# Nextomics/NextPolish2

Hardware: AMD Instinct MI355X
Metric: polished reference Mbp/s (whole node) at 30x HiFi + k21/k31; FASTA identical to oracle (higher is better)
Workload: dtype u8

## Files before the change

### nextpolish2_amd/csrc/np2_common.hpp

```cpp
#pragma once
#include <cstdint>
#include <hip/hip_runtime.h>

#define NP2_HD __host__ __device__ __forceinline__

namespace np2 {

struct AlignBase {
    uint32_t t_pos;
    uint16_t delta;
    uint8_t q;
    NP2_HD bool is_head() const { return q == 15; }
    NP2_HD bool eq(const AlignBase &o) const { return q == o.q && delta == o.delta && t_pos == o.t_pos; }
};
NP2_HD AlignBase ab_head(uint32_t t_pos, uint16_t delta) { return AlignBase{t_pos, delta, 15}; }

NP2_HD uint16_t node_bases(const AlignBase &b1, const AlignBase &b2, const AlignBase &b3) {
    unsigned f = 0;
    if (b2.t_pos == b1.t_pos) f |= 0x4000u;
    if (b2.t_pos == b3.t_pos) f |= 0x1000u;
    return (uint16_t)(f | ((unsigned)b1.q << 8) | ((unsigned)b2.q << 4) | (unsigned)b3.q);
}
NP2_HD void node_decode(uint16_t bases, uint16_t delta, uint32_t p, AlignBase &a, AlignBase &b, AlignBase &c) {
    a.q = (bases >> 8) & 0xF;
    b.q = (bases >> 4) & 0xF;
    c.q = bases & 0xF;
    if ((bases & 0x5000) == 0x5000) {
        a.t_pos = p, a.delta = delta;
        b.t_pos = p, b.delta = (uint16_t)(delta + 1);
        c.t_pos = p, c.delta = (uint16_t)(delta + 2);
    } else if (bases & 0x1000) {
        a.t_pos = p - 1, a.delta = delta;
        b.t_pos = p, b.delta = 0;
        c.t_pos = p, c.delta = 1;
    } else if (bases & 0x4000) {
        a.t_pos = p - 1, a.delta = delta;
        b.t_pos = p - 1, b.delta = (uint16_t)(delta + 1);
        c.t_pos = p, c.delta = 0;
    } else {
        a.t_pos = p - 2, a.delta = delta;
        b.t_pos = p - 1, b.delta = 0;
        c.t_pos = p, c.delta = 0;
    }
}
NP2_HD uint16_t node_delta3(uint16_t bases, uint16_t delta) {
    if ((bases & 0x5000) == 0x5000) return (uint16_t)(delta + 2);
    if (bases & 0x1000) return 1;
    return 0;
}

NP2_HD uint64_t yak_hash64(uint64_t key, uint64_t mask) {
    key = (~key + (key << 21)) & mask;
    key = key ^ key >> 24;
    key = ((key + (key << 3)) + (key << 8)) & mask;
    key = key ^ key >> 14;
    key = ((key + (key << 2)) + (key << 4)) & mask;
    key = key ^ key >> 28;
    key = (key + (key << 31)) & mask;
    return key;
}

NP2_HD uint8_t code_to_ascii(uint8_t c) {
    const uint64_t tab = 0x004D4E2D54474341ULL;
    return (uint8_t)(tab >> (8 * (c & 7)));
}
NP2_HD uint8_t ascii_to_code(uint8_t ch) {
    switch (ch & 0x7F) {
    case 'A': case 'a': return 0;
    case 'C': case 'c': return 1;
    case 'G': case 'g': return 2;
    case 'T': case 't': case 'U': case 'u': return 3;
    case 'N': case 'n': return 5;
    case 'M': case 'm': return 6;
    default: return 4;
    }
}

static constexpr uint64_t INVALID_KMER = ~0ULL;
static constexpr uint32_t LQSEQ_MAX_CAN_COUNT = 60;
static constexpr int64_t SCORE_NEG = INT64_MIN >> 1;

enum : uint8_t { CLS_HQ = 0, CLS_LQ = 1, CLS_RESET = 2 };
static constexpr uint32_t GROW_ERR = 0x1000u;
static constexpr uint32_t LQ_LIST_ERR = 0x800u;

static constexpr uint32_t CKPT_SHIFT = 5;
static constexpr uint32_t CKPT = 1u << CKPT_SHIFT;

NP2_HD uint8_t nib_at(const uint8_t *bytes, uint32_t c) {
    uint8_t t = bytes[c >> 1];
    return (c & 1) ? (t & 15) : (t >> 4);
}


#if defined(__HIPCC__)
__device__ __forceinline__ uint32_t xcd_order(uint32_t b, uint32_t n) {
    if (n < 64) return b;
    const uint32_t q = n >> 3, r = n & 7u, x = b & 7u;
    return x * q + (x < r ? x : r) + (b >> 3);
}
#endif

}
```

### nextpolish2_amd/csrc/np2_ctx.hpp

```cpp
#pragma once
#include "../../include/np2.h"
#include "np2_abi.hpp"
#include "np2_common.hpp"
#include "np2_kernels.hpp"
#include "np2_hostcpu.hpp"

#include <algorithm>
#include <atomic>
#include <chrono>
#include <cstdio>
#include <cstdlib>
#include <cstring>
#include <map>
#include <memory>
#include <exception>
#include <mutex>
#include <stdexcept>
#include <string>
#include <vector>

namespace np2h {

using namespace np2;

// ... 393 lines not shown
    return std::chrono::duration<double, std::milli>(std::chrono::steady_clock::now().time_since_epoch()).count();
}


}

using namespace np2h;

struct np2_contig {
    np2_contig() {
        reads.cached = nib.cached = refnib.cached = ck_off.cached = ckpt.cached = descs.cached = true;
        tile_rd_off.cached = tile_rd.cached = true;
    }
    uint32_t L = 0, R = 0;
    uint64_t nib_bytes = 0, n_cols = 0, n_ckpt = 0;
    DevBuf<np2_read_t> reads;
    DevBuf<uint8_t> nib;
    DevBuf<uint8_t> refnib;
    uint32_t ref_stride = 0;
    DevBuf<uint64_t> ck_off;
    DevBuf<uint32_t> ckpt;
    uint32_t n_chunks = 0;
    DevBuf<ChunkDesc> descs;
    uint32_t n_tiles = 0;
    DevBuf<uint32_t> tile_rd_off, tile_rd;
    uint32_t tile_cap = TILE_CAP;
};

struct np2_ctx {
    int device = 0;
    hipStream_t stream = nullptr;
    hipStream_t stream_out = nullptr;
    hipEvent_t ev_out = nullptr;
    uint8_t *out_host[2] = {nullptr, nullptr};
    size_t out_host_cap[2] = {0, 0};
    int out_slot = 0;
    bool out_pending = false;
    uint64_t out_len = 0;
    std::vector<YakTable> yaks;
    std::string err;
    bool trace = false;
    std::map<std::string, std::vector<uint8_t>> trace_items;
    Timing timing;
    std::vector<std::pair<std::string, std::pair<hipEvent_t, hipEvent_t>>> pending_events;

    PinnedBuf pin_d2h, pin_h2d;
    uint32_t *mbox_host = nullptr, *mbox_dev = nullptr;
    uint32_t mbox_seq = 0;
    bool borrowed_state = false;
    uint8_t *sink_dst = nullptr;
    uint64_t sink_cap = 0;
    uint32_t last_first_pos = 0, last_last_pos = 0;
    const uint8_t *last_dbase = nullptr;
    const uint32_t *last_dpos = nullptr;
    DevBuf<uint32_t> shard_bounds;
    uint64_t last_len = 0;
    bool reuse_identical_pass = true;
    bool h2d_inflight = false;
    bool stage_timing = false;
    DevBuf<uint8_t> tmp;
    DevBuf<uint64_t> keys_raw, keys;
    DevBuf<uint32_t> vals_raw, vals;
    DevBuf<uint32_t> npos, ncount, nminr, nbesti, node_off, run_start, run_end, n0_besti, emit, eoff;
    DevBuf<uint16_t> nbases, ndelta;
    DevBuf<int64_t> nscore;
    DevBuf<int32_t> cov, mval, smin;
    DevBuf<uint8_t> alive, cns_base, cns_cls, lq_kind, lq_nothead;
    DevBuf<uint32_t> cns_pos, lq_next, rflag, rstart, rend, ridx, raw_start, raw_end, headflag, hidx, lq_start,
        lq_end;
    DevBuf<uint32_t> pj, pcount, reg_ncand, reg_bytes, reg_soff, reg_maxlen, blk_sum, blk_coff, blk_soff, kept_read, kept_len, kept_col, cand_off, cand_order, cand_seq_off, kill_ids;
    DevBuf<uint64_t> cand_kmer;
    DevBuf<uint8_t> cand_seq;
    DevBuf<uint16_t> kscore;
    DevBuf<uint32_t> scal;
    DevBuf<uint64_t> lb_status;
    DevBuf<uint32_t> lb_ticket;
    uint32_t lb_ticket_total = 0, lb_epoch = 0;
    bool lb_dirty = false;
    static constexpr size_t LB_MAX_BLOCKS = 1u << 20;
    DevBuf<uint32_t> mlen;
    DevBuf<uint8_t> reg_lable, grp, cns_base2, rech_groups, rech_groups_tmp;
    DevBuf<uint8_t> votepack;
    DevBuf<uint8_t> votepack2;
    DevBuf<uint32_t> rech_headjobs;
    DevBuf<uint32_t> ecount, eval, eval_s, eflag, eidx, seed_cand, keep_n, keep_list, cns_pos2, sp_idx_s,
        sp_idx_e, ap_g, ap_s, ap_e, rech, rech_joboff, job_len,
        job_off32;
    DevBuf<int32_t> ew, ap_delta, ap_shift;
    DevBuf<uint64_t> ekey, ekey_s;
    DevBuf<uint16_t> keep_ks;
    DevBuf<uint32_t> long_list;
    DevBuf<uint64_t> bt_path;
    DevBuf<uint64_t> chunk_st;
    uint32_t chunk_epoch = 0;
    DevBuf<uint32_t> tile_cur, tile_n, tile_scan, tile_scanb, tile_nn, tile_nr, tile_noff, tile_roff;
    uint32_t tile_cap = TILE_CAP;
    uint32_t bucket_cap = 0;
    DevBuf<uint2> nrec;
    DevBuf<uint8_t> votebuf;
    DevBuf<uint32_t> band, band_n, band_off, row_cnt;
    DevBuf<int64_t> run_gain, tile_gain;
    DevBuf<uint8_t> out_snap;
    DevBuf<uint8_t> run_flag;
    uint32_t deep_min = 65536;
    DevBuf<uint32_t> lq_list, hbits;
    DevBuf<uint16_t> tile_pidx;
    bool pidx_valid = false;
    DevBuf<ReadInfo> rinfo;
    DevBuf<uint32_t> lqc, lqoff;
    DevBuf<uint8_t> pflag;
    DevBuf<uint32_t> dp_list;
    DevBuf<uint16_t> pf_slots;
    DevBuf<uint32_t> pf_bad, pf_bad2;
    DevBuf<uint64_t> pf_prof;
    bool front_fused = false;
    struct Hooks {
        bool front_unfused = false, pf_prof = false, edge_sort = false;
        bool test_misspeculate = false, shard_spec_log = false, phase_profile = false, exact_grow = false, no_speculate = false;
        bool has_grow_guess = false;
        uint32_t grow_guess = 0;
        bool has_pf_cap = false, has_pf_cap_big = false, has_pf_halo = false, has_pf_cov_max = false;
        uint32_t pf_cap = 0, pf_cap_big = 0, pf_halo = 0, pf_cov_max = 0;
        void read() {
            auto on = [](const char *n) { return getenv(n) != nullptr; };
            auto u32 = [](const char *n, bool &has, uint32_t &v) {
                if (const char *e = getenv(n)) has = true, v = (uint32_t)atol(e);
            };
            front_unfused = on("NP2_FRONT_UNFUSED"), pf_prof = on("NP2_PF_PROF"), edge_sort = on("NP2_EDGE_SORT");
            test_misspeculate = on("NP2_TEST_MISSPECULATE");
            shard_spec_log = on("NP2_SHARD_SPEC_LOG"), phase_profile = on("NP2_PHASE_PROFILE"), exact_grow = on("NP2_EXACT_GROW");
            no_speculate = on("NP2_NO_SPECULATE");
            u32("NP2_TEST_GROW_GUESS", has_grow_guess, grow_guess);
            u32("NP2_PF_CAP", has_pf_cap, pf_cap), u32("NP2_PF_CAP_BIG", has_pf_cap_big, pf_cap_big);
            u32("NP2_PF_HALO", has_pf_halo, pf_halo), u32("NP2_PF_COV_MAX", has_pf_cov_max, pf_cov_max);
        }
    } hooks;
    bool pf_big = getenv("NP2_PF_BIG") != nullptr;
    uint32_t front_redos = 0;
    DevBuf<uint16_t> kscore_saved;
    DevBuf<uint8_t> sstr;
    DevBuf<uint64_t> soff;
    DevBuf<uint16_t> sscore;
};


namespace np2h {


enum Scal { S_ERR = 0, S_NNODES, S_NRUNS, S_BEST, S_PATHBEGIN, S_NRAW, S_NREG, S_DUP, S_LAST0, S_LAST1, S_GAIN0,
            S_GAIN1, S_DEEP, S_NDPLIST, S_NRECH, S_NGROUPS, S_NLONG, S_NLQ, S_PF, S_M0, S_M1, S_M2, S_M3, S_NC, S_SB, S_GROW,
            S_NBAD, S_PFOUT, S_PFGAIN0, S_PFGAIN1, S_PFEND0, S_PFEND1, S_NBAD2, S_NOKEY, S_COUNT = 34 };
static_assert(S_M1 % 2 == 0 && S_LAST0 % 2 == 0 && S_GAIN0 % 2 == 0 && S_PFGAIN0 % 2 == 0 && S_PFEND0 % 2 == 0,
              "64-bit device counters live in these slot pairs");

static constexpr int NP2_MAX_YAK = 15;
static constexpr uint32_t SCAL_TOTAL = 96;
static_assert(S_COUNT + 2 * (NP2_MAX_YAK + 2) <= SCAL_TOTAL && S_COUNT < 64, "round counters behind the posted block; the mailbox holds 64 words");

inline double thread_cpu_ms() {
    timespec ts;
    clock_gettime(CLOCK_THREAD_CPUTIME_ID, &ts);
    return ts.tv_sec * 1e3 + ts.tv_nsec * 1e-6;
}
struct WallTimer {
    np2_ctx *cx;
    const char *name;
    double t0, c0 = 0;
    WallTimer(np2_ctx *c, const char *n);
    ~WallTimer();
};

struct EventTimer {
    np2_ctx *cx;
    hipEvent_t a = nullptr, b = nullptr;
    bool on;
    EventTimer(np2_ctx *c, const char *name, bool always = false)
        : cx(c), on((always || c->stage_timing) && !tl_recorder()) {
        if (!on) return;
        (void)hipEventCreate(&a);
        (void)hipEventCreate(&b);
        (void)hipEventRecord(a, cx->stream);
        cx->pending_events.push_back({name, {a, b}});
    }
    ~EventTimer() {
        if (on) (void)hipEventRecord(b, cx->stream);
    }
};

inline WallTimer::WallTimer(np2_ctx *c, const char *n) : cx(c), name(n), t0(c->stage_timing ? now_ms() : 0.0), c0(c->stage_timing ? thread_cpu_ms() : 0.0) {}
inline WallTimer::~WallTimer() {
    if (cx->stage_timing) {
        cx->timing.host.push_back({name, (float)(now_ms() - t0)});
        if (strncmp(name, "wall", 4) == 0) cx->timing.host.push_back({std::string("cpu") + (name + 4), (float)(thread_cpu_ms() - c0)});
    }
}

inline void flush_timings(np2_ctx *cx) {
    std::map<std::string, float> acc;
    std::vector<std::string> order;
    for (auto &e : cx->pending_events) {
        float ms = 0;
        (void)hipEventSynchronize(e.second.second);
        (void)hipEventElapsedTime(&ms, e.second.first, e.second.second);
        if (!acc.count(e.first)) order.push_back(e.first);
        acc[e.first] += ms;
        (void)hipEventDestroy(e.second.first);
        (void)hipEventDestroy(e.second.second);
    }
    cx->pending_events.clear();
    for (auto &h : cx->timing.host) {
        if (!acc.count(h.first)) order.push_back(h.first);
        acc[h.first] += h.second;
    }
    cx->timing.host.clear();
    cx->timing.names = order;
    cx->timing.ms.clear();
    cx->timing.joined.clear();
    for (auto &n : order) {
        cx->timing.ms.push_back(acc[n]);
        cx->timing.joined += n;
        cx->timing.joined.push_back('\0');
    }
    cx->timing.joined.push_back('\0');
}
inline auto ctx_sink(np2_ctx *cx, bool timings = false) {
    return [cx, timings](int, const std::string &msg) {
        (void)hipStreamSynchronize(cx->stream);
        if (timings) flush_timings(cx);
        cx->err = msg;
    };
}

inline void recorder_sync(Recorder *r) {
    r->sync_fn(r, true);
    for (auto &g : r->graveyard)
        dev_release_idle(g.first, (g.second >> 63) ? 0 : g.second, (g.second >> 63) ? (g.second & ~(1ull << 63)) : 0);
    r->graveyard.clear();
}
np2_ctx *ctx_create_slot(np2_ctx *parent, hipStream_t s, uint32_t *mbox_host, uint32_t *mbox_dev);
void ctx_slot_set_stream(np2_ctx *cx, hipStream_t s);
// ... 177 lines not shown
```

### nextpolish2_amd/csrc/np2_host.cpp

```cpp
#include "../../include/np2.h"
#include "np2_common.hpp"
#include "np2_kernels.hpp"
#include "np2_ctx.hpp"
#include "np2_phase_host.hpp"

#include <algorithm>
#include <atomic>
#include <thread>
#include <chrono>
#include <cstdio>
#include <cstdlib>
#include <cstring>
#include <map>
#include <mutex>
#include <stdexcept>
#include <string>
#include <unordered_map>
#include <unordered_set>
#include <future>
#include <functional>
#include <vector>

using namespace np2;

// ... 13 lines not shown
    std::vector<uint32_t> pos;
    std::vector<uint8_t> base;
    size_t size() const { return pos.size(); }
};
void trace_cns(np2_ctx *cx, int pass, const std::string &tag, const Cns &c) {
    trace_put(cx, pass, tag + ".pos", c.pos);
    trace_put(cx, pass, tag + ".base", c.base);
}

struct PassCounts {
    uint32_t n_reg = 0, NC = 0, SB = 0, M = 0;
    uint32_t grow = 0;
    bool known = false;
    uint32_t NC_cap = 0;
    uint32_t SB_cap = 0;
    void resolve(const std::vector<uint32_t> &sc) {
        NC = sc[S_NC], SB = sc[S_SB], grow = sc[S_GROW];
        known = true;
    }
};

RegionTables region_tables(np2_ctx *cx, uint32_t n_reg) {
    return RegionTables{cx->cand_off.p, cx->cand_order.p, cx->kscore.p, cx->cand_seq_off.p, cx->cand_seq.p, n_reg};
}

void trace_region_tables(np2_ctx *cx, int pass, const std::string &tag, const PassCounts &pc, bool kept_view) {
    if (!cx->trace) return;
    const uint32_t n_reg = pc.n_reg;
    auto start = d2h(cx, cx->lq_start.p, n_reg), end = d2h(cx, cx->lq_end.p, n_reg);
    auto coff = d2h(cx, cx->cand_off.p, (size_t)n_reg + 1);
    auto order = d2h(cx, cx->cand_order.p, pc.NC);
    auto ks = d2h(cx, cx->kscore.p, pc.NC);
    auto soff = d2h(cx, cx->cand_seq_off.p, (size_t)pc.NC + 1);
    auto pool = d2h(cx, cx->cand_seq.p, pc.SB);
    std::vector<uint8_t> lable(n_reg, 0);
    std::vector<uint32_t> seedc, keepn, keepl;
    std::vector<uint16_t> keepks;
    if (tag != "cand") lable = d2h(cx, cx->reg_lable.p, n_reg);
    if (kept_view) {
        seedc = d2h(cx, cx->seed_cand.p, n_reg);
        keepn = d2h(cx, cx->keep_n.p, n_reg);
        keepl = d2h(cx, cx->keep_list.p, pc.NC);
        keepks = d2h(cx, cx->keep_ks.p, pc.NC);
    }
    std::vector<uint32_t> o_coff(1, 0), o_order, o_soff(1, 0), sudo_off(1, 0);
    std::vector<uint16_t> o_ks;
    std::vector<uint8_t> o_seq, sudo;
    for (uint32_t g = 0; g < n_reg; ++g) {
        if (kept_view) {
            const uint32_t c = seedc[g];
            if (c != 0xFFFFFFFFu) sudo.insert(sudo.end(), pool.begin() + soff[c], pool.begin() + soff[c + 1]);
            for (uint32_t t = 0; t < keepn[g]; ++t) {
                const uint32_t ci = keepl[coff[g] + t];
                o_order.push_back(order[ci]);
                o_ks.push_back(keepks[coff[g] + t]);
                o_seq.insert(o_seq.end(), pool.begin() + soff[ci], pool.begin() + soff[ci + 1]);
                o_soff.push_back((uint32_t)o_seq.size());
            }
        } else {
            for (uint32_t ci = coff[g]; ci < coff[g + 1]; ++ci) {
                o_order.push_back(order[ci]);
                o_ks.push_back(ks[ci]);
                o_seq.insert(o_seq.end(), pool.begin() + soff[ci], pool.begin() + soff[ci + 1]);
                o_soff.push_back((uint32_t)o_seq.size());
            }
        }
        sudo_off.push_back((uint32_t)sudo.size());
        o_coff.push_back((uint32_t)o_order.size());
    }
    trace_put(cx, pass, tag + ".start", start);
    trace_put(cx, pass, tag + ".end", end);
    trace_put(cx, pass, tag + ".lable", lable);
    trace_put(cx, pass, tag + ".sudo_off", sudo_off);
    trace_put(cx, pass, tag + ".sudo", sudo);
    trace_put(cx, pass, tag + ".cand_off", o_coff);
    trace_put(cx, pass, tag + ".order", o_order);
    trace_put(cx, pass, tag + ".kscore", o_ks);
    trace_put(cx, pass, tag + ".seq_off", o_soff);
    trace_put(cx, pass, tag + ".seq", o_seq);
    if (tag == "cand") trace_put(cx, pass, "cand.kmer", d2h(cx, cx->cand_kmer.p, pc.NC));
}

struct GrowRetry : Np2Error {
    GrowRetry() : Np2Error(NP2_E_DEVICE, "internal: guessed growth allowance too small") {}
};
void check_region_err(np2_ctx *cx, uint32_t e) {
    (void)cx;
    if (e & 4u) throw Np2Error(NP2_E_REFPANIC, "reference would panic: seq2 order is equal to 0");
    if (e & 8u) throw Np2Error(NP2_E_REFPANIC, "reference would panic: index out of bounds: lqseq.seqs[max1_p]");
    if (e & 16u) throw Np2Error(NP2_E_REFPANIC, "reference would panic: the first lqseq is not ref.");
    if (e & 32u) throw Np2Error(NP2_E_REFPANIC, "reference would panic: lqseq.seqs[0] after retain_sort_seqs");
    if (e & 64u) throw Np2Error(NP2_E_REFPANIC, "reference would panic: consensus index out of bounds in reupdate");
    if (e & 128u) throw Np2Error(NP2_E_NOMEM, "cartesian product of chained LQ regions is too large");
    if (e & LB_ERR) throw Np2Error(NP2_E_DEVICE, "device-wide scan timed out waiting for a predecessor block");
    if (e & GROW_ERR) throw GrowRetry();
    if (e & LQ_LIST_ERR) throw Np2Error(NP2_E_DEVICE, "internal: more low-quality bases than their list was sized for");
}

struct VoteData {
    uint32_t R = 0;
    bool any = false;
    std::vector<uint64_t> pair_key;
    std::vector<uint32_t> pair_cnt;
    const uint64_t *view_key = nullptr;
    const uint32_t *view_cnt = nullptr;
    uint64_t view_n = 0;
    const uint32_t *off = nullptr;
    const phase::Graph::Edge *edges = nullptr;
    uint32_t n_nokey = 0;
    std::vector<uint32_t> off_own;
    std::vector<phase::Graph::Edge> edges_own;
    bool rows() const { return off != nullptr; }
    const uint64_t *keys() const { return view_key ? view_key : pair_key.data(); }
    const uint32_t *cnts() const { return view_key ? view_cnt : pair_cnt.data(); }
    uint64_t n_pairs() const { return view_key ? view_n : (uint64_t)pair_key.size(); }
    void own() {
        if (rows() && off_own.empty()) {
            off_own.assign(off, off + R + 1);
            edges_own.assign(edges, edges + off[R]);
            off = off_own.data(), edges = edges_own.data();
        }
        if (!view_key) return;
        pair_key.assign(view_key, view_key + view_n);
        pair_cnt.assign(view_cnt, view_cnt + view_n);
        view_key = nullptr, view_cnt = nullptr, view_n = 0;
    }
    std::vector<uint32_t> first_key;
    std::vector<int32_t> ref_w;
    std::vector<uint8_t> ref_seen, bad;
    const uint8_t *d_bad = nullptr;
    bool key_added = false;
};

bool vote_rows_from_pairs(VoteData &vd, bool use_all) {
    const uint32_t R = vd.R;
    const uint64_t *k = vd.keys();
    const uint32_t *cn = vd.cnts();
    const uint64_t np = vd.n_pairs();
    std::vector<uint32_t> n_lo(R, 0), n_up(R, 0);
    uint32_t nokey = 0;
    auto listed = [&](uint64_t i, uint32_t &a, uint32_t &b) {
        a = (uint32_t)(k[i] >> 32), b = (uint32_t)k[i];
        if (a >= R || b >= R || vd.first_key[a] == 0xFFFFFFFFu || vd.first_key[b] == 0xFFFFFFFFu) return false;
        return use_all || !(vd.bad[a] | vd.bad[b]);
    };
    for (uint64_t i = 0; i < np; ++i) {
        uint32_t a = (uint32_t)(k[i] >> 32), b = (uint32_t)k[i];
        if (b <= a || b - a - 1 >= EDGE_BAND || (i && k[i - 1] >= k[i])) return false;
        if (a >= R || b >= R || vd.first_key[a] == 0xFFFFFFFFu || vd.first_key[b] == 0xFFFFFFFFu) ++nokey;
        if (listed(i, a, b)) ++n_lo[b], ++n_up[a];
    }
    vd.off_own.assign((size_t)R + 1, 0);
    std::vector<uint32_t> cur_lo(R), cur_up(R);
    for (uint32_t v = 0; v < R; ++v) {
        cur_lo[v] = vd.off_own[v], cur_up[v] = vd.off_own[v] + n_lo[v];
        vd.off_own[v + 1] = cur_up[v] + n_up[v];
    }
    vd.edges_own.resize(vd.off_own[R]);
    for (uint64_t i = 0; i < np; ++i) {
        uint32_t a, b;
        if (!listed(i, a, b)) continue;
        const int32_t same = (int32_t)(cn[i] & 0xFFFFu), neg = (int32_t)(cn[i] >> 16);
        const float w = (float)(neg >= 3 ? -neg : same - neg);
        vd.edges_own[cur_lo[b]++] = phase::Graph::Edge(a, w);
        vd.edges_own[cur_up[a]++] = phase::Graph::Edge(b, w);
    }
    vd.off = vd.off_own.data(), vd.edges = vd.edges_own.data(), vd.n_nokey = nokey;
    return true;
}

void vote_collect(np2_ctx *cx, np2_contig *c, PassCounts &pc, bool asref, bool use_all, int pass, uint32_t own_lo,
                  uint32_t own_hi, VoteData &vd, bool wide = false, uint64_t key_add = 0) {
    hipStream_t s = cx->stream;
    const uint32_t R = c->R, n_reg = pc.n_reg;
    RegionTables rt = region_tables(cx, n_reg);
    uint32_t NE = 0, NU = 0;
    vd = VoteData();
    vd.R = R;
// ... 184 lines not shown
    const bool prof = getenv("NP2_PHASE_PROFILE") != nullptr;
    double t_mark = t_host0;
    auto mark = [&](const char *what) {
        if (prof) {
            const double t = now_ms();
            fprintf(stderr, "  vote host: %s %.2f ms\n", what, t - t_mark);
            t_mark = t;
        }
    };
    phase::Graph data;
    data.reserve_ids(R);
    mark("key order");
    for (auto &k : keys) data.add_key(k.second);
    mark("key table");
    auto weight = [&](uint64_t i) {
        const int32_t same = (int32_t)(pair_cnt[i] & 0xFFFFu), neg = (int32_t)(pair_cnt[i] >> 16);
        return (float)(neg >= 3 ? -neg : same - neg);
    };
    std::vector<uint32_t> bad;
    for (uint32_t r = 0; r < R; ++r)
        if (vd.bad[r]) bad.push_back(r);
    if (!use_all) data.keys.keep_if([&](uint32_t k, phase::Nil &) { return !vd.bad[k]; });
    mark("retain");
    std::future<phase::OrderSet> communities;
    if (data.keys.size() >= (1u << 15) && phase::host_threads() > 1)
        communities = std::async(std::launch::async, [&data] { return phase::SignedLouvain::first_communities(data.keys); });
    bool ok = false;
    try {
        if (vd.rows()) {
            ok = vd.n_nokey == 0;
            if (ok) data.adopt_rows(vd.off, vd.edges, R);
        } else {
            ok = data.add_edges_sorted(vd.keys(), NU, weight, use_all ? nullptr : vd.bad.data());
        }
    } catch (...) {
        if (communities.valid()) communities.wait();
        throw;
    }
    phase::OrderSet comm_pre;
    if (communities.valid()) comm_pre = communities.get();
    const bool have_pre = !comm_pre.empty();
    if (!ok) throw Np2Error(NP2_E_DEVICE, "internal: edge endpoint without a key");
    if (!use_all)
        for (uint32_t b : bad) data.is_key[b] = 0;
    mark("keys + edges");
    if (cx && cx->trace && pass >= 0) {
        trace_put(cx, pass, "vote.row_off", data.off);
        const phase::Graph::Edge *e0 = data.n_ids() ? data.adj(0).b : nullptr;
        trace_put(cx, pass, "vote.rows", std::vector<phase::Graph::Edge>(e0, e0 + (e0 ? data.n_edges() : 0)));
    }
    std::vector<float> ref_row(R, 0.f);
    std::vector<uint8_t> ref_have(R, 0);
    bool have_ref = false;
    for (uint32_t r = 0; r < R; ++r)
        if (vd.ref_seen[r]) {
            ref_row[r] = (float)vd.ref_w[r];
            ref_have[r] = 1;
            have_ref = true;
        }
    std::vector<uint32_t> losers;
    if (!phase::losing_reads(std::move(data), have_ref, ref_row, ref_have, losers, have_pre ? &comm_pre : nullptr))
        throw Np2Error(NP2_E_REFPANIC,
                       "reference would panic: the weight of two conflicting community is not less than 0");
    mark("louvain + ranking");
    if (cx) cx->timing.host.push_back({"wall_louvain", (float)(now_ms() - t_host0)});
    std::vector<uint8_t> lost(R, 0);
    for (uint32_t b : bad) lost[b] = 1;
    for (uint32_t l : losers)
        if (l < R) lost[l] = 1;
        else throw Np2Error(NP2_E_DEVICE, "internal: loser outside the contig's reads");
    losers.clear();
    for (uint32_t r = 0; r < R; ++r)
        if (lost[r]) losers.push_back(r);
    return losers;
}

struct CnsDev {
    uint32_t *pos;
    uint8_t *base;
    const uint32_t *M_p;
    uint32_t M_cap;
};

CnsDev splice_gpu(np2_ctx *cx, const CnsDev &in, uint32_t n_reg, uint8_t lable, uint32_t grow_bound, bool to_b,
                  uint32_t version) {
    hipStream_t s = cx->stream;
    EventTimer t(cx, "splice");
    cx->sp_idx_s.ensure(n_reg + 2);
    cx->sp_idx_e.ensure(n_reg + 2);
    cx->ap_g.ensure(n_reg + 2);
    cx->ap_s.ensure(n_reg + 2);
    cx->ap_e.ensure(n_reg + 2);
    cx->ap_delta.ensure(n_reg + 2);
    cx->ap_shift.ensure(n_reg + 2);
    cx->mlen.ensure(16);
    const uint32_t out_cap = in.M_cap + grow_bound;
    const size_t cap = (size_t)out_cap + 64;
    uint32_t *opos = to_b ? cx->cns_pos2.ensure(cap) : cx->cns_pos.ensure(cap);
    uint8_t *obase = to_b ? cx->cns_base2.ensure(cap) : cx->cns_base.ensure(cap);
    uint32_t *const stuck_p = cx->scal.p + S_COUNT + 2 * version, *const nap_p = stuck_p + 1;
    launch_splice_find(s, in.pos, in.M_p, cx->lq_start.p, cx->lq_end.p, cx->reg_lable.p, lable, n_reg, cx->sp_idx_s.p,
                       cx->sp_idx_e.p, stuck_p);
    launch_splice_plan(s, next_lookback(cx, region_lb_blocks(n_reg)), cx->reg_lable.p, lable, n_reg, stuck_p,
                       cx->sp_idx_s.p, cx->sp_idx_e.p, cx->seed_cand.p, cx->cand_seq_off.p, cx->ap_g.p, cx->ap_s.p,
                       cx->ap_e.p, cx->ap_delta.p, cx->ap_shift.p, nap_p, in.M_p, cx->mlen.p + version, out_cap,
                       cx->scal.p + S_ERR);
    launch_splice_write(s, in.pos, in.base, in.M_p, in.M_cap, cx->ap_g.p, cx->ap_s.p, cx->ap_e.p, cx->ap_delta.p,
                        cx->ap_shift.p, nap_p, n_reg, cx->lq_start.p, cx->seed_cand.p, cx->cand_seq_off.p,
                        cx->cand_seq.p, opos, obase);
    return CnsDev{opos, obase, cx->mlen.p + version, out_cap};
}

Cns fetch_cns_dev(np2_ctx *cx, const CnsDev &c) {
    Cns r;
    const uint32_t M = d2h(cx, c.M_p, 1)[0];
    r.pos = d2h(cx, c.pos, M);
    r.base = d2h(cx, c.base, M);
    return r;
}

CnsDev recheck_gpu(np2_ctx *cx, const CnsDev &in, const PassCounts &pc, int yak_idx, uint16_t min_kmer_count,
                   bool first_yak, bool to_b, uint32_t version) {
    hipStream_t s = cx->stream;
    const uint32_t n_reg = pc.n_reg, ksize = cx->yaks[yak_idx].k;
    uint32_t n_rech = 0, n_groups = 0, n_jobs = 0;
    uint64_t blob_bound = 0;
    {
        EventTimer t(cx, "recheck");
        cx->rech.ensure(n_reg + 2);
        cx->rech_groups.ensure((size_t)(n_reg + 2) * rech_group_bytes());
        cx->rech_joboff.ensure(n_reg + 2);
        cx->rech_groups_tmp.ensure((size_t)(n_reg + 2) * rech_group_bytes());
        cx->rech_headjobs.ensure(n_reg + 2);
        launch_rech_list(s, next_lookback(cx, region_lb_blocks(n_reg)), cx->reg_lable.p, n_reg, cx->rech.p, cx->scal.p + S_NRECH,
                         (unsigned long long *)(cx->scal.p + S_M1), cx->scal.p + S_ERR);
        launch_rech_groups(s, next_lookback(cx, region_lb_blocks(n_reg)), cx->rech.p, cx->scal.p + S_NRECH, n_reg, in.pos, in.M_p,
                           cx->lq_start.p, cx->lq_end.p, cx->keep_n.p, ksize, cx->reg_maxlen.p, cx->rech_groups_tmp.p,
                           cx->rech_headjobs.p, cx->rech_groups.p,
                           cx->rech_joboff.p, cx->scal.p + S_NGROUPS,
                           cx->scal.p + S_M0, (unsigned long long *)(cx->scal.p + S_M1), cx->scal.p + S_ERR);
        std::vector<uint32_t> sc = fetch_scal(cx);
        blob_bound = (uint64_t)sc[S_M1] | ((uint64_t)sc[S_M2] << 32);
        check_region_err(cx, sc[S_ERR]);
        n_rech = sc[S_NRECH];
        n_groups = sc[S_NGROUPS];
        n_jobs = sc[S_M0];
    }
    if (n_rech) {
        RechPtrs rp{cx->rech_groups.p, cx->rech_joboff.p, cx->rech.p, cx->cand_off.p, cx->keep_list.p,
                    cx->cand_seq_off.p, cx->cand_seq.p, in.base, n_groups};
        if (n_jobs) {
            EventTimer t(cx, "recheck");
            cx->job_len.ensure(n_jobs + 2);
            cx->job_off32.ensure(n_jobs + 2);
            cx->soff.ensure(n_jobs + 2);
            cx->sscore.ensure(n_jobs + 2);
            cx->tmp.ensure(prim_temp_bytes((size_t)n_jobs + 2));
            launch_rech_job_len(s, rp, n_jobs, cx->job_len.p);
            exclusive_total_n(cx, cx->job_len.p, cx->job_off32.p, n_jobs);
            if (blob_bound >= 0xFFFFFFF0ull)
                blob_bound = fetch_scal(cx, cx->scal.p + S_M0, cx->job_off32.p + n_jobs)[S_M0];
            cx->sstr.ensure((size_t)blob_bound + 64);
            launch_rech_job_build(s, rp, n_jobs, cx->job_off32.p, cx->soff.p, cx->sstr.p);
            launch_score_strings(s, cx->yaks[yak_idx].dev(), cx->sstr.p, cx->soff.p, n_jobs, min_kmer_count,
                                 cx->sscore.p, true);
            launch_rech_apply(s, rp, cx->sscore.p, cx->keep_ks.p);
        }
        EventTimer t(cx, "recheck");
        launch_rech_select(s, cx->rech.p, cx->scal.p + S_NRECH, n_rech, cx->cand_off.p, cx->keep_n.p, cx->keep_list.p,
                           cx->keep_ks.p, cx->cand_order.p, first_yak, cx->reg_lable.p, cx->seed_cand.p);
    }
    CnsDev out = splice_gpu(cx, in, n_reg, LB_RECH, pc.grow, to_b, version);
    launch_rech_relabel(s, cx->reg_lable.p, n_reg);
    return out;
}

void gpu_score_strings(np2_ctx *cx, int yak_idx, const std::vector<uint8_t> &blob, const std::vector<uint64_t> &off,
                       uint16_t min_kmer_count, std::vector<uint16_t> &scores) {
    const size_t n = off.size() - 1;
    scores.assign(n, 0);
    if (!n) return;
    cx->sstr.ensure(blob.size() + 16);
    cx->soff.ensure(off.size());
    cx->sscore.ensure(n);
    {
        op_sync(cx);
        uint8_t *pin = (uint8_t *)cx->pin_h2d.ensure(blob.size() + off.size() * 8 + 16);
        const size_t o2 = (blob.size() + 7) & ~(size_t)7;
        memcpy(pin, blob.data(), blob.size());
        memcpy(pin + o2, off.data(), off.size() * 8);
        op_h2d(cx, cx->sstr.p, pin, blob.size());
        op_h2d(cx, cx->soff.p, pin + o2, off.size() * 8);
        cx->h2d_inflight = true;
    }
    {
        EventTimer t(cx, "score_strings");
        launch_score_strings(cx->stream, cx->yaks[yak_idx].dev(), cx->sstr.p, cx->soff.p, n, min_kmer_count,
                             cx->sscore.p, false);
    }
    scores = d2h(cx, cx->sscore.p, n);
}

struct PassOut {
    bool has_regions = false;
    Cns cns;
};

void run_diff(np2_ctx *cx, np2_contig *c, uint32_t &T) {
    hipStream_t s = cx->stream;
    const uint32_t L = c->L, R = c->R, NCH = c->n_chunks;
    const uint32_t n_tiles = (L + TILE - 1) >> TILE_SHIFT;
    const uint32_t bcap = std::min(cx->tile_cap, c->tile_cap);
    const uint64_t buckets = (uint64_t)n_tiles * bcap;
    uint64_t ovf_cap = std::max<uint64_t>(c->n_cols / 256 + 65536, 1u << 18);
    cx->tmp.ensure(prim_temp_bytes(std::max<size_t>((size_t)NCH + 2, (size_t)L + 2)));
    cx->tile_n.ensure(n_tiles + 2);
    cx->tile_scan.ensure(n_tiles + 2);
    cx->tile_scanb.ensure(n_tiles + 2);
    cx->tile_nn.ensure(n_tiles + 2);
    cx->tile_nr.ensure(n_tiles + 2);
    cx->tile_noff.ensure(n_tiles + 2);
    cx->tile_roff.ensure(n_tiles + 2);
    cx->tile_gain.ensure(n_tiles + 2);
    if (cx->tile_cur.cap < (size_t)n_tiles + 2) {
        cx->tile_cur.ensure(n_tiles + 2);
        zero32(cx, cx->tile_cur.p, cx->tile_cur.cap);
    }
    if (cx->chunk_st.cap < (size_t)NCH + 2) {
        cx->chunk_st.ensure(NCH + 2);
// ... 500 lines not shown
    uint64_t key_add = 0;
    PassCounts pc;
    bool final_pass() const { return pass + 1 == o.iter_count; }
};

void run_begin(PolishRun &r) {
    np2_ctx *cx = r.cx;
    if (r.o.iter_count < 1) throw Np2Error(NP2_E_ARG, "iter_count must be >= 1");
    HIPCHK(hipSetDevice(cx->device));
    cx->trace_items.clear();
    cx->last_dbase = nullptr;
    cx->last_dpos = nullptr;
    cx->scal.ensure(SCAL_TOTAL);
    cx->alive.ensure(r.c->R + 2);
    {
        WallTimer w(cx, "wall_diff");
        run_diff(cx, r.c, r.T);
    }
    launch_init_alive(cx->stream, r.c->reads.p, r.c->R, cx->alive.p);
    r.pass = 0;
    r.reuse = false;
}

void run_pass_front(PolishRun &r) {
    np2_ctx *cx = r.cx;
    np2_contig *c = r.c;
    if (!r.reuse) {
        {
            WallTimer w(cx, "wall_cns_lq");
            if (!r.front_issued) pass_front_issue(cx, c, r.T, (int)r.pass);
            r.front_issued = false;
            consensus_and_regions_finish(cx, c, r.T, (int)r.pass, r.M, r.n_reg, !r.wide_votes);
        }
        if (cx->trace) {
            trace_cns(cx, (int)r.pass, "cns_raw", fetch_cns(cx, r.M));
            trace_put(cx, (int)r.pass, "lq.start", d2h(cx, cx->lq_start.p, r.n_reg));
            trace_put(cx, (int)r.pass, "lq.end", d2h(cx, cx->lq_end.p, r.n_reg));
        }
    }
    if (r.n_reg == 0) return;
    if (!r.reuse) {
        r.pc = PassCounts();
        r.pc.M = r.M;
        WallTimer w(cx, "wall_extract");
        extract_candidates(cx, c, r.n_reg, r.o.min_kmer_count, (int)r.pass, r.pc);
    } else if (r.pc.NC_cap) {
        op_copy_d2d(cx, cx->kscore.p, cx->kscore_saved.p, (size_t)(r.pc.known ? r.pc.NC : r.pc.NC_cap) * 2);
    }
}

void run_vote_pass(PolishRun &r, VoteData &vd, const std::function<void()> *after_front = nullptr) {
    np2_ctx *cx = r.cx;
    vd = VoteData();
    vd.R = r.c->R;
    run_pass_front(r);
    if (after_front) (*after_front)();
    if (r.n_reg == 0) return;
    WallTimer w(cx, "wall_vote");
    const bool may_reuse = cx->reuse_identical_pass && !cx->trace;
    if (may_reuse && r.pc.NC_cap) {
        cx->kscore_saved.ensure((size_t)r.pc.NC_cap + 2);
        op_copy_d2d(cx, cx->kscore_saved.p, cx->kscore.p, (size_t)(r.pc.known ? r.pc.NC : r.pc.NC_cap) * 2);
    }
    vote_collect(cx, r.c, r.pc, r.o.model_ref != 0, r.o.use_all_reads != 0, (int)r.pass, r.own_lo, r.own_hi, vd, r.wide_votes, r.key_add);
    if (r.pc.known) r.grow_prev = r.pc.grow;
}

void run_apply_losers(PolishRun &r, const std::vector<uint32_t> &losers) {
    np2_ctx *cx = r.cx;
    if (r.n_reg) trace_put(cx, (int)r.pass, "invalid_ids", losers);
    for (uint32_t id : losers) REFPANIC_IF(id >= r.c->R, "index out of bounds: alignseqs[id]");
    const bool may_reuse = cx->reuse_identical_pass && !cx->trace;
    r.reuse = false;
    if (!losers.empty()) {
        cx->kill_ids.ensure(losers.size());
        h2d_staged(cx, cx->kill_ids.p, losers.data(), losers.size() * 4);
        launch_kill_reads(cx->stream, cx->kill_ids.p, (uint32_t)losers.size(), cx->alive.p);
    } else if (may_reuse) {
        r.reuse = true;
    }
    ++r.pass;
}

void run_final_pass(PolishRun &r, ResultOut &result, bool exact_grow = false) {
    np2_ctx *cx = r.cx;
    np2_contig *c = r.c;
    hipStream_t s = cx->stream;
    const uint32_t n_reg_prev = r.n_reg;
    (void)n_reg_prev;
    run_pass_front(r);
    const uint32_t n_reg = r.n_reg;
    if (n_reg == 0) {
        fetch_result(cx, cx->cns_pos.p, cx->cns_base.p, cx->eoff.p + c->L, r.M, result);
        return;
    }
    PassCounts &pc = r.pc;
    WallTimer w(cx, "wall_final");
    RegionTables rt = region_tables(cx, n_reg);
    cx->reg_lable.ensure(n_reg + 2);
    cx->seed_cand.ensure(n_reg + 2);
    cx->keep_n.ensure(n_reg + 2);
    const bool no_guess = cx->hooks.exact_grow;
    bool guessed = false;
    if (!pc.known) {
        if (r.grow_prev != 0xFFFFFFFFu && !exact_grow && !no_guess && !cx->trace && (uint64_t)r.grow_prev * 2 + 4096 < 0x7FFFFFFFull) {
            pc.grow = r.grow_prev * 2 + 4096;
            if (cx->hooks.has_grow_guess) pc.grow = cx->hooks.grow_guess;
            guessed = true;
        } else {
            pc.resolve(fetch_scal(cx));
        }
    }
    try {
        cx->keep_list.ensure((size_t)pc.NC_cap + 2);
        cx->keep_ks.ensure((size_t)pc.NC_cap + 2);
        {
            EventTimer t(cx, "seed");
            launch_seed(s, rt, r.o.max_indel_len, cx->reg_lable.p, cx->seed_cand.p, cx->keep_n.p, cx->keep_list.p,
                        cx->keep_ks.p, cx->scal.p + S_ERR);
        }
        if (cx->trace) check_region_err(cx, d2h(cx, cx->scal.p + S_ERR, 1)[0]);
        trace_region_tables(cx, (int)r.pass, "seed", pc, true);
        CnsDev cur{cx->cns_pos.p, cx->cns_base.p, cx->eoff.p + c->L, r.M};
        bool to_b = true;
        uint32_t version = 0;
        cur = splice_gpu(cx, cur, n_reg, LB_SUCC, pc.grow, to_b, version++);
        to_b = !to_b;
        if (cx->trace) trace_cns(cx, (int)r.pass, "cns_succ", fetch_cns_dev(cx, cur));
        for (size_t y = 0; y < cx->yaks.size(); ++y) {
            cur = recheck_gpu(cx, cur, pc, (int)y, r.o.min_kmer_count, y == 0, to_b, version++);
            to_b = !to_b;
            trace_region_tables(cx, (int)r.pass, "rech" + std::to_string(y), pc, true);
            if (cx->trace) trace_cns(cx, (int)r.pass, "cns_rech" + std::to_string(y), fetch_cns_dev(cx, cur));
        }
        fetch_result(cx, cur.pos, cur.base, cur.M_p, cur.M_cap, result, guessed ? r.M + r.grow_prev : r.M + pc.grow);
    } catch (const GrowRetry &) {
        if (!guessed) throw;
        result.release();
        op_fill(cx, cx->scal.p + S_ERR, 0, 4);
        r.reuse = false;
        run_final_pass(r, result, true);
    }
}

void polish_impl(np2_ctx *cx, np2_contig *c, const np2_opts_t *o, ResultOut &result) {
    PolishRun r;
    r.cx = cx, r.c = c, r.o = *o;
    run_begin(r);
    const bool no_spec = cx->hooks.no_speculate;
    const bool use_all = o->use_all_reads != 0;
    struct Decision {
        std::vector<uint32_t> losers;
        double ms = 0;
    };
    struct Pending {
        std::future<Decision> fut;
        std::shared_ptr<VoteData> vd;
        size_t n_bad = 0;
        bool active = false;
    } pend;
    auto settle = [&]() -> bool {
        if (!pend.active) return true;
        pend.active = false;
        Decision d = pend.fut.get();
        cx->timing.host.push_back({"wall_louvain", (float)d.ms});
        std::vector<uint32_t> extra;
        for (uint32_t id : d.losers) {
            REFPANIC_IF(id >= c->R, "index out of bounds: alignseqs[id]");
            if (!pend.vd->bad[id]) extra.push_back(id);
        }
        if (extra.empty() && d.losers.size() == pend.n_bad && !cx->hooks.test_misspeculate) return true;
        if (!extra.empty()) {
            cx->kill_ids.ensure(extra.size() + 1);
            h2d_staged(cx, cx->kill_ids.p, extra.data(), extra.size() * 4);
            launch_kill_reads(cx->stream, cx->kill_ids.p, (uint32_t)extra.size(), cx->alive.p);
        }
        r.reuse = false;
        r.front_issued = false;
        return false;
    };
    const std::function<void()> settle_then_redo = [&]() {
        if (!settle()) run_pass_front(r);
    };
    while (!r.final_pass()) {
        auto vd = std::make_shared<VoteData>();
        run_vote_pass(r, *vd, &settle_then_redo);
        size_t n_bad = 0;
        if (vd->any && vd->d_bad && !use_all && !cx->trace && !no_spec)
            for (uint8_t b : vd->bad) n_bad += b;
        if (n_bad == 0) {
            run_apply_losers(r, vote_decide(cx, *vd, use_all, (int)r.pass));
            continue;
        }
        launch_kill_flagged(cx->stream, vd->d_bad, c->R, cx->alive.p);
        ++r.pass;
        r.reuse = false;
        if (cx->hooks.pf_prof) vd->own();
        pass_front_issue(cx, c, r.T, (int)r.pass);
        r.front_issued = true;
        op_submit(cx);
        pend.vd = vd;
        pend.n_bad = n_bad;
        pend.active = true;
        auto decide = [vd, use_all]() {
            Decision d;
            const double t0 = now_ms();
            d.losers = vote_decide(nullptr, *vd, use_all);
            d.ms = now_ms() - t0;
            return d;
        };
        if (tl_recorder() == nullptr) {
            vd->own();
            pend.fut = std::async(std::launch::async, decide);
        } else {
            std::promise<Decision> p;
            pend.fut = p.get_future();
            try {
                p.set_value(decide());
            } catch (...) {
                p.set_exception(std::current_exception());
            }
            (void)settle();
        }
    }
// ... 1021 lines not shown
```

### nextpolish2_amd/csrc/np2_kernels.hip

```cpp
#include "np2_common.hpp"
#include "np2_kernels.hpp"
#include "np2_blockscan.hpp"
#include "np2_nib128.hpp"
#include "../../include/np2.h"

namespace np2 {

__device__ __forceinline__ uint8_t ref_code(const uint8_t *__restrict__ refnib, uint32_t p) {
    return (refnib[p >> 1] >> (4 * (p & 1))) & 7;
}

__device__ __forceinline__ void k_encode_ref(const uint32_t np2_bid, const uint32_t np2_nb, const uint8_t *__restrict__ read0, uint32_t L, uint8_t *__restrict__ refnib,
                             uint32_t nbytes_total, uint32_t stride, uint32_t *__restrict__ err) {
    uint32_t i = np2_bid * blockDim.x + threadIdx.x;
    if (i >= nbytes_total) return;
    uint32_t c0 = 2 * i, c1 = 2 * i + 1;
    uint8_t b = c0 < L ? read0[i] : 0;
    uint8_t hi = c0 < L ? (b >> 4) : 0, lo = c1 < L ? (b & 15) : 0;
    if ((c0 < L && c0 != 0 && (hi & 8)) || (c1 < L && (lo & 8))) atomicOr(err, 1u);
    if (c0 < L && (hi & 7) == 7) atomicOr(err, 1u);
    if (c1 < L && (lo & 7) == 7) atomicOr(err, 1u);
    refnib[i] = (uint8_t)((hi & 7) | ((lo & 7) << 4));
    const uint8_t nx = c1 + 1 < L ? (uint8_t)((read0[i + 1] >> 4) & 7) : (uint8_t)0;
    refnib[stride + i] = (uint8_t)(((hi & 7) << 4) | (lo & 7));
// ... 1177 lines not shown
        while (atomicCAS((unsigned long long *)&tb[s], (unsigned long long)YAK_EMPTY, (unsigned long long)w) != YAK_EMPTY)
            s = (s + 1) & capm;
        ob[s] = (uint32_t)i;
    }
}

__device__ __forceinline__ void k_lookup(const uint32_t np2_bid, const uint32_t np2_nb, YakDev y, const uint64_t *__restrict__ hashes, uint64_t n, uint16_t min_count,
                         uint16_t *__restrict__ out) {
    uint64_t i = (uint64_t)np2_bid * blockDim.x + threadIdx.x;
    if (i < n) out[i] = yak_get(y, hashes[i], min_count);
}

__device__ __forceinline__ uint16_t wave_score_string_any(const YakDev &y, const uint8_t *__restrict__ s, uint32_t len,
                                                          uint16_t min_count) {
    const uint32_t lane = threadIdx.x & 63;
    const uint32_t k = y.k;
    const uint64_t mask = (1ULL << (2 * (uint64_t)k)) - 1, shift = 2 * ((uint64_t)k - 1);
    uint32_t mn = 0xFFFFFFFFu;
    if (len >= k) {
        for (uint32_t st = lane; st + k <= len; st += 64) {
            uint64_t fw = 0, rv = 0;
            bool ok = true;
            for (uint32_t j = 0; j < k; ++j) {
                const uint64_t c = ascii_to_code(s[st + j]);
                if (c >= 4) {
                    ok = false;
                    break;
                }
                fw = ((fw << 2) | c) & mask;
                rv = (rv >> 2) | ((3ULL ^ c) << shift);
            }
            if (ok) mn = min(mn, (uint32_t)yak_get(y, yak_hash64(fw < rv ? fw : rv, mask), min_count));
        }
    }
    for (int o = 32; o > 0; o >>= 1) mn = min(mn, (uint32_t)__shfl_xor(mn, o));
    return mn == 0xFFFFFFFFu ? (uint16_t)0 : (uint16_t)mn;
}
__device__ __forceinline__ uint16_t wave_score_string(const YakDev &y, const uint8_t *__restrict__ s, uint32_t len,
                                                      uint16_t min_count) {
    const uint32_t lane = threadIdx.x & 63;
    const uint32_t k = y.k;
    const uint64_t mask = (1ULL << (2 * (uint64_t)k)) - 1;
    uint32_t mn = 0xFFFFFFFFu;
    if (len >= k) {
        for (uint32_t st = lane; st + k <= len; st += 64) {
            uint64_t codes = 0, bad = 0;
#pragma unroll
            for (uint32_t wd = 0; wd < 4; ++wd) {
                uint64_t x;
                __builtin_memcpy(&x, s + st + 8 * wd, 8);
                uint64_t c = ((x >> 1) ^ (x >> 2)) & 0x0303030303030303ULL;
                c = (c | (c >> 6)) & 0x000F000F000F000FULL;
                c = (c | (c >> 12)) & 0x000000FF000000FFULL;
                c = (c | (c >> 24)) & 0xFFFFULL;
                codes |= c << (16 * wd);
                uint64_t b = (x >> 3) & 0x0101010101010101ULL;
                b = (b | (b >> 7)) & 0x0003000300030003ULL;
                b = (b | (b >> 14)) & 0x0000000F0000000FULL;
                b = (b | (b >> 28)) & 0xFFULL;
                bad |= b << (8 * wd);
            }
            if ((bad & ((1ULL << k) - 1ULL)) == 0) {
                codes &= mask;
                uint64_t rb = __builtin_bitreverse64(codes);
                rb = ((rb >> 1) & 0x5555555555555555ULL) | ((rb & 0x5555555555555555ULL) << 1);
                const uint64_t fw = rb >> (64 - 2 * k), rv = ~codes & mask;
                mn = min(mn, (uint32_t)yak_get(y, yak_hash64(fw < rv ? fw : rv, mask), min_count));
            }
        }
    }
    for (int o = 32; o > 0; o >>= 1) mn = min(mn, (uint32_t)__shfl_xor(mn, o));
    return mn == 0xFFFFFFFFu ? (uint16_t)0 : (uint16_t)mn;
}

__device__ __forceinline__ void k_score_strings(const uint32_t np2_bid, const uint32_t np2_nb, YakDev y, const uint8_t *__restrict__ strs, const uint64_t *__restrict__ off,
                                uint64_t n, uint16_t min_count, uint16_t *__restrict__ out, uint32_t own_strings) {
    const uint64_t w = ((uint64_t)np2_bid * (blockDim.x >> 6)) + (uint32_t)__builtin_amdgcn_readfirstlane((int)(threadIdx.x >> 6));
    if (w >= n) return;
    const uint16_t sc = own_strings ? wave_score_string(y, strs + off[w], (uint32_t)(off[w + 1] - off[w]), min_count)
                                    : wave_score_string_any(y, strs + off[w], (uint32_t)(off[w + 1] - off[w]), min_count);
    if ((threadIdx.x & 63) == 0) out[w] = sc;
}

__device__ __forceinline__ void k_cand_score(const uint32_t np2_bid, const uint32_t np2_nb, YakDev y, const uint32_t *__restrict__ cand_seq_off, const uint64_t *__restrict__ cand_kmer,
                             const uint32_t *__restrict__ n_cand_p, uint16_t min_count,
                             uint16_t *__restrict__ kscore, uint32_t *__restrict__ long_list,
                             uint32_t *__restrict__ n_long) {
    const uint32_t c = np2_bid * blockDim.x + threadIdx.x;
    const bool live = c < *n_cand_p;
    const uint32_t len = live ? cand_seq_off[c + 1] - cand_seq_off[c] : 0u;
    const bool is_long = live && len > y.k;
    const uint64_t m = __ballot(is_long);
    if (m) {
        const uint32_t lane = threadIdx.x & 63, lead = (uint32_t)__builtin_ctzll(m);
        uint32_t base = 0;
        if (lane == lead) base = atomicAdd(n_long, (uint32_t)__builtin_popcountll(m));
        base = __shfl(base, lead);
        if (is_long) long_list[base + (uint32_t)__builtin_popcountll(m & ((1ULL << lane) - 1ULL))] = c;
    }
    if (!live) return;
    uint16_t sc = 0;
    if (!is_long) {
        const uint64_t km = cand_kmer[c];
        if (km != INVALID_KMER) sc = yak_get(y, km, min_count);
    }
    kscore[c] = sc;
}
__device__ __forceinline__ void k_cand_score_long(const uint32_t np2_bid, const uint32_t np2_nb, YakDev y, const uint32_t *__restrict__ cand_seq_off,
                                  const uint8_t *__restrict__ cand_seq, const uint32_t *__restrict__ long_list,
                                  const uint32_t *__restrict__ n_long, uint16_t min_count,
                                  uint16_t *__restrict__ kscore) {
    const uint32_t nl = *n_long;
    for (uint32_t w = (uint32_t)__builtin_amdgcn_readfirstlane((int)((np2_bid * blockDim.x + threadIdx.x) >> 6)); w < nl; w += (np2_nb * blockDim.x) >> 6) {
        const uint32_t c = long_list[w];
        const uint16_t sc = wave_score_string(y, cand_seq + cand_seq_off[c], cand_seq_off[c + 1] - cand_seq_off[c],
                                              min_count);
        if ((threadIdx.x & 63) == 0) kscore[c] = sc;
    }
}

}

namespace np2 {
static inline dim3 grid1(uint64_t n, uint32_t bs = 256) { return dim3((unsigned)((n + bs - 1) / bs)); }

void launch_encode_ref(hipStream_t s, const uint8_t *read0, uint32_t L, uint8_t *refnib, uint32_t nbytes,
                       uint32_t stride, uint32_t *err) {
    NP2_LAUNCH(k_encode_ref, grid1(nbytes), 256, s, read0, L, refnib, nbytes, stride, err);
}
void launch_post(hipStream_t s, uint32_t *scal, uint32_t n_scal, uint32_t *mbox, uint32_t seq, uint32_t *d0,
                 const uint32_t *s0, uint32_t *d1, const uint32_t *s1, uint32_t *d2, const uint32_t *s2, uint32_t *d3,
                 const uint32_t *s3, const uint32_t *ends_of, uint32_t *ends_dst) {
    NP2_LAUNCH(k_post, dim3(1), 64, s, scal, n_scal, mbox, seq, d0, s0, d1, s1, d2, s2, d3, s3, ends_of, ends_dst);
}
void launch_fill(hipStream_t s, uint8_t *p, uint64_t bytes, uint8_t byte) {
    if (bytes) NP2_LAUNCH(k_fill, grid1((bytes + 15) / 16), 256, s, p, bytes, 0x01010101u * byte);
}
void launch_copy(hipStream_t s, uint8_t *dst, const uint8_t *src, uint64_t bytes) {
    if (bytes) NP2_LAUNCH(k_copy, grid1((bytes + 15) / 16), 256, s, dst, src, bytes);
}
void launch_copy_len(hipStream_t s, uint8_t *dst, const uint8_t *src, const uint32_t *n_dev, uint32_t elem, uint64_t cap_bytes) {
    if (cap_bytes) NP2_LAUNCH(k_copy_len, grid1((cap_bytes + 15) / 16), 256, s, dst, src, n_dev, elem, cap_bytes);
}
void launch_copy_counted(hipStream_t s, uint32_t *dst, const uint32_t *src, const uint32_t *n_dev, uint32_t cap, uint32_t words_per) {
    if (cap) NP2_LAUNCH(k_copy_counted, dim3(std::max<uint32_t>(1, std::min<uint32_t>((cap + 1023) / 1024, 2048))), 256, s, dst, src, n_dev, cap, words_per);
}
void launch_init_alive(hipStream_t s, const np2_read_t *reads, uint32_t R, uint8_t *alive) {
    NP2_LAUNCH(k_init_alive, grid1(R), 256, s, reads, R, alive);
}
void launch_kill_flagged(hipStream_t s, const uint8_t *flag, uint32_t n, uint8_t *alive) {
    if (n) NP2_LAUNCH(k_kill_flagged, grid1(n), 256, s, flag, n, alive);
}
void launch_kill_reads(hipStream_t s, const uint32_t *ids, uint32_t n, uint8_t *alive) {
    if (n) NP2_LAUNCH(k_kill_reads, grid1(n), 256, s, ids, n, alive);
}
void launch_revive_reads(hipStream_t s, const uint32_t *ids, uint32_t n, uint8_t *alive) {
    if (n) NP2_LAUNCH(k_revive_reads, grid1(n), 256, s, ids, n, alive);
}
static Graph mk_graph(const GraphPtrs &gp) { return Graph{gp.refnib, gp.node_off, gp.nd, gp.cov, gp.L, gp.nrec, gp.deep}; }

void launch_dp_short(hipStream_t s, const GraphPtrs &gp, const void *refw, const uint32_t *run_start,
                     const uint32_t *n_runs, uint32_t max_runs, uint32_t *run_end, int64_t *run_gain, uint32_t *emit,
                     uint32_t *path_begin, uint64_t *path, uint32_t *dp_list, uint32_t *n_dp_list) {
    if (max_runs)
        NP2_LAUNCH(k_dp_bt_short, dim3(std::min<uint32_t>((max_runs + 63) / 64, DP_GRID_CAP)), 64, s, run_start, n_runs, mk_graph(gp), (const uint32_t *)refw, run_end, run_gain, emit, path_begin, path, dp_list, n_dp_list);
}
// ... 3 lines not shown
                    const uint32_t *dp_list, const uint32_t *n_dp_list) {
    if (!max_runs) return;
    NP2_LAUNCH(k_dp_bt_oct, dim3(std::min<uint32_t>((max_runs + 7) / 8, 2048u)), 64, s, run_start, mk_graph(gp), nrec, nscore, nbesti, n0_besti, run_end, last_n0_score, run_gain, emit, path_begin, path, run_flag, dp_list, n_dp_list);
    NP2_LAUNCH(k_dp_bt_long, dim3(std::min<uint32_t>((max_runs + DP_BLOCK - 1) / DP_BLOCK, 512u)), DP_BLOCK, s, run_start, mk_graph(gp), nrec, nscore, nbesti, n0_besti, run_end, last_n0_score, run_gain, emit, path_begin, path, run_flag, dp_list, n_dp_list);
}
void launch_dp_finish(hipStream_t s, const GraphPtrs &gp, const uint32_t *run_start, const uint32_t *n_runs,
                      const int64_t *nscore, const uint32_t *nbesti, const uint32_t *n0_besti, const int64_t *last_n0_score,
                      unsigned long long *total_gain, uint32_t *blocks_done, uint32_t *best_idx, const int64_t *run_gain,
                      const long long *tile_gain, uint32_t n_tiles, uint32_t *emit, uint32_t *path_begin, uint64_t *path) {
    NP2_LAUNCH(k_dp_finish, dim3(64), 256, s, run_gain, n_runs, tile_gain, n_tiles, total_gain, blocks_done, mk_graph(gp), nscore, last_n0_score, run_start, nbesti, n0_besti, best_idx, emit, path_begin, path);
}
static inline dim3 run_grid(uint32_t bound) { return dim3(std::max<uint32_t>(1, std::min<uint32_t>((bound + 256) / 256, 4096))); }
void launch_bt_write(hipStream_t s, const GraphPtrs &gp, const uint32_t *run_start, const uint32_t *n_runs,
                     uint32_t run_bound, const uint32_t *emit, const uint32_t *eoff, const uint64_t *path,
                     uint32_t *cns_pos, uint8_t *cns_base, uint8_t *cns_cls, uint8_t *lq_nothead, uint32_t *lqc) {
    NP2_LAUNCH(k_cns_write, grid1(gp.L), 256, s, gp.refnib, gp.pflag, emit, eoff, gp.L, cns_pos, cns_base, cns_cls, lq_nothead);
    NP2_LAUNCH(k_cns_runs, run_grid(4 * (uint64_t)run_bound > 0xFFFFFFF0ull ? 0xFFFFFFF0u : 4 * run_bound), 256, s, run_start, n_runs, run_bound, gp.node_off, emit, eoff, path, cns_pos, cns_base, cns_cls, lq_nothead, lqc);
}
void launch_lq_list(hipStream_t s, const GraphPtrs &gp, const uint32_t *run_start, const uint32_t *n_runs,
                    uint32_t run_bound, const uint32_t *emit, const uint32_t *eoff, const uint64_t *path,
                    const uint32_t *lqoff, uint32_t cap, uint32_t *lq_list, uint32_t *err) {
    NP2_LAUNCH(k_lq_list, run_grid(run_bound), 256, s, run_start, n_runs, run_bound, gp.node_off, emit, eoff, path, lqoff, cap, lq_list, err);
}
void launch_default_tail(hipStream_t s, const GraphPtrs &gp, const uint32_t *best_idx, const uint32_t *M_p, uint8_t *cns_base,
                         uint8_t *cns_cls, uint32_t *lq_list, uint32_t *n_lq, uint32_t cap, uint32_t *err) {
    NP2_LAUNCH(k_default_tail, 1, 64, s, best_idx, gp.node_off, gp.pflag, gp.L, M_p, cns_base, cns_cls, lq_list, n_lq, cap, err);
}
static inline dim3 lq_grid(uint32_t cap) { return dim3(std::max<uint32_t>(1, std::min<uint32_t>((cap + 2047) / 2048, 2048))); }
void launch_lq_scan(hipStream_t s, const uint32_t *cns_pos, const uint8_t *cns_base, const uint8_t *cns_cls,
                    const uint32_t *M_p, const uint32_t *lq_list, const uint32_t *n_lq, uint32_t lq_cap, uint8_t *lq_kind,
                    uint32_t *lq_next, uint8_t *lq_nothead, uint32_t *hbits, uint32_t n_hwords, uint32_t *rstart, uint32_t *rend) {
    NP2_LAUNCH(k_lq_scan, lq_grid(std::max(lq_cap, n_hwords / 4)), 256, s, cns_pos, cns_base, cns_cls, M_p, lq_list, n_lq, lq_cap, lq_kind, lq_next, lq_nothead, hbits, n_hwords);
    NP2_LAUNCH(k_lq_region, lq_grid(lq_cap), 256, s, cns_pos, cns_base, M_p, lq_list, n_lq, lq_cap, lq_kind, lq_next, lq_nothead, hbits, rstart, rend);
}
void launch_lq_bits_count(hipStream_t s, const uint32_t *hbits, uint32_t n_words, uint32_t *wcnt) {
    NP2_LAUNCH(k_lq_bits_count, grid1((uint64_t)n_words + 1), 256, s, hbits, n_words, wcnt);
}
void launch_scatter_regions(hipStream_t s, const uint32_t *hbits, uint32_t n_words, const uint32_t *woff,
                            const uint32_t *rstart, const uint32_t *rend, uint32_t *raw_start, uint32_t *raw_end,
                            uint32_t *n_raw) {
    NP2_LAUNCH(k_scatter_regions, grid1(std::max<uint32_t>(n_words, 1)), 256, s, hbits, n_words, woff, rstart, rend, raw_start, raw_end, n_raw);
}
void launch_lq_merge_flag(hipStream_t s, const uint32_t *raw_start, const uint32_t *raw_end, const uint32_t *n_raw,
                          uint32_t *headflag) {
    NP2_LAUNCH(k_lq_merge_flag, dim3(256), 256, s, raw_start, raw_end, n_raw, headflag);
}
void launch_lq_merge_scan(hipStream_t s, const uint32_t *raw_start, const uint32_t *raw_end, const uint32_t *n_raw, uint32_t n_host,
                          uint32_t *headflag, uint32_t *hidx) {
    NP2_LAUNCH(k_lq_merge_scan, dim3(1), 1024, s, raw_start, raw_end, n_raw, n_host, headflag, hidx);
}
void launch_lq_merge_write(hipStream_t s, const uint32_t *raw_start, const uint32_t *raw_end, const uint32_t *n_raw,
                           const uint32_t *headflag, const uint32_t *hidx, uint32_t *lq_start, uint32_t *lq_end,
                           uint32_t *n_reg) {
    NP2_LAUNCH(k_lq_merge_write, dim3(256), 256, s, raw_start, raw_end, n_raw, headflag, hidx, lq_start, lq_end, n_reg);
}
void launch_read_m(hipStream_t s, const np2_read_t *reads, uint32_t R, const uint8_t *alive, const uint32_t *lq_start,
                   uint32_t n_reg, int32_t *mval) {
    NP2_LAUNCH(k_read_m, grid1(R), 256, s, reads, R, alive, lq_start, n_reg, mval);
}
void launch_pair_count(hipStream_t s, const np2_read_t *reads, uint32_t R, const uint8_t *alive,
                       const uint32_t *lq_start, const uint32_t *lq_end, uint32_t n_reg, const int32_t *smin,
                       uint32_t *pj, uint32_t *pcount, const uint64_t *ck_off, ReadInfo *rinfo) {
    NP2_LAUNCH(k_pair_count, grid1(R), 256, s, reads, R, alive, lq_start, lq_end, n_reg, smin, pj, pcount, ck_off, rinfo);
}
void launch_yak_insert(hipStream_t s, const uint64_t *words, const uint64_t *bucket_off, uint32_t n_buckets,
                       uint64_t max_bucket, uint64_t *table, uint32_t cap_log2, uint32_t *dup_flag, uint32_t gap) {
    uint32_t gx = (uint32_t)((max_bucket + 255) / 256);
    if (gx == 0) gx = 1;
    if (gx > 64) gx = 64;
    hipLaunchKernelGGL(k_yak_insert, dim3(gx, n_buckets), dim3(256), 0, s, words, bucket_off, n_buckets, table,
                       cap_log2, dup_flag, gap);
}
void launch_yak_insert_dup(hipStream_t s, const uint64_t *words, const uint64_t *bucket_off, uint32_t n_buckets,
                           uint64_t max_bucket, uint64_t *table, uint32_t cap_log2, uint32_t *ord, uint32_t gap) {
    uint32_t gx = (uint32_t)((max_bucket + 255) / 256);
    gx = std::min<uint32_t>(64, std::max<uint32_t>(1, gx));
    hipLaunchKernelGGL(k_yak_insert_dup, dim3(gx, n_buckets), dim3(256), 0, s, words, bucket_off, n_buckets, table,
                       cap_log2, ord, gap);
}
void launch_lookup(hipStream_t s, const YakDev &y, const uint64_t *hashes, uint64_t n, uint16_t min_count,
                   uint16_t *out) {
    if (n) NP2_LAUNCH(k_lookup, grid1(n), 256, s, y, hashes, n, min_count, out);
}
void launch_score_strings(hipStream_t s, const YakDev &y, const uint8_t *strs, const uint64_t *off, uint64_t n,
                          uint16_t min_count, uint16_t *out, bool own_strings) {
    if (n) NP2_LAUNCH(k_score_strings, grid1(n * 64), 256, s, y, strs, off, n, min_count, out, own_strings ? 1u : 0u);
}
void launch_cand_score(hipStream_t s, const YakDev &y, const uint32_t *cand_seq_off, const uint8_t *cand_seq,
                       const uint64_t *cand_kmer, const uint32_t *n_cand_p, uint32_t cand_cap, uint16_t min_count,
                       uint16_t *kscore, uint32_t *long_list, uint32_t *n_long) {
    if (!cand_cap) return;
    NP2_LAUNCH(k_cand_score, grid1(cand_cap), 256, s, y, cand_seq_off, cand_kmer, n_cand_p, min_count, kscore, long_list, n_long);
    NP2_LAUNCH(k_cand_score_long, dim3(std::max<uint32_t>(16, std::min<uint32_t>(1024, cand_cap / 4096))), 256, s, y, cand_seq_off, cand_seq, long_list, n_long, min_count, kscore);
}
}
```

### nextpolish2_amd/csrc/np2_kernels.hpp

```cpp
#pragma once
#include <cstddef>
#include <cstdint>
#include <hip/hip_runtime.h>
#include "../../include/np2.h"
#include "np2_lookback.hpp"
#include "np2_launch.hpp"

namespace np2 {

static constexpr uint32_t TILE_SHIFT = 10;
static constexpr uint32_t TILE = 1u << TILE_SHIFT;
static constexpr uint32_t TILE_CAP = 4096;

static constexpr uint32_t DENSE_COLS = 4096;
struct ChunkDesc {
    uint64_t nib_off;
    uint64_t ckbase;
    uint32_t read, ts;
    uint32_t c0, ncols;
    uint32_t first_chunk;
    uint32_t aln_t_e, nck;
    uint32_t pad0;
    uint32_t pad[4];
};
// ... 66 lines not shown
        for (;;) {
            const uint64_t w = tb[s];
            if (w == YAK_EMPTY) return c;
            if ((w >> 10) == key && (uint16_t)(w & 1023) >= min_count && (int64_t)ob[s] > at) at = ob[s], c = (uint16_t)(w & 1023);
            s = (s + 1) & capm;
        }
    }
    for (;;) {
        const uint64_t w = tb[s];
        if (w == YAK_EMPTY) return 0;
        if ((w >> 10) == key) {
            const uint16_t c = (uint16_t)(w & 1023);
            return c >= min_count ? c : 0;
        }
        s = (s + 1) & capm;
    }
}
#endif

void launch_encode_ref(hipStream_t s, const uint8_t *read0, uint32_t L, uint8_t *refnib, uint32_t nbytes, uint32_t stride, uint32_t *err);
void launch_chunk_counts(hipStream_t s, const ChunkDesc *descs, uint32_t n_chunks, const uint8_t *nib, uint64_t *chunk_st, uint32_t epoch);
void launch_diff_reads(hipStream_t s, const ChunkDesc *descs, uint32_t n_chunks, const uint8_t *nib, const uint64_t *refw,
                       const uint8_t *refnib, const uint8_t *refeo, uint32_t eo_stride, uint32_t L, uint64_t *keys, uint32_t *vals, uint32_t *tile_cur,
                       uint32_t n_tiles, uint32_t bucket_cap, uint64_t ovf_base, uint32_t ovf_cap, uint32_t *ovf_cnt,
                       uint32_t *ckpt, uint64_t *chunk_st, uint32_t epoch, uint32_t *err);
void launch_post(hipStream_t s, uint32_t *scal, uint32_t n_scal, uint32_t *mbox, uint32_t seq, uint32_t *d0 = nullptr,
                 const uint32_t *s0 = nullptr, uint32_t *d1 = nullptr, const uint32_t *s1 = nullptr, uint32_t *d2 = nullptr,
                 const uint32_t *s2 = nullptr, uint32_t *d3 = nullptr, const uint32_t *s3 = nullptr,
                 const uint32_t *ends_of = nullptr, uint32_t *ends_dst = nullptr);
void launch_fill(hipStream_t s, uint8_t *p, uint64_t bytes, uint8_t byte);
void launch_copy(hipStream_t s, uint8_t *dst, const uint8_t *src, uint64_t bytes);
void launch_copy_len(hipStream_t s, uint8_t *dst, const uint8_t *src, const uint32_t *n_dev, uint32_t elem, uint64_t cap_bytes);
void launch_copy_counted(hipStream_t s, uint32_t *dst, const uint32_t *src, const uint32_t *n_dev, uint32_t cap, uint32_t words_per = 1);
void launch_init_alive(hipStream_t s, const np2_read_t *reads, uint32_t R, uint8_t *alive);
void launch_kill_reads(hipStream_t s, const uint32_t *ids, uint32_t n, uint8_t *alive);
void launch_revive_reads(hipStream_t s, const uint32_t *ids, uint32_t n, uint8_t *alive);
void launch_kill_flagged(hipStream_t s, const uint8_t *flag, uint32_t n, uint8_t *alive);
void launch_dp_short(hipStream_t s, const GraphPtrs &gp, const void *refw, const uint32_t *run_start,
                     const uint32_t *n_runs, uint32_t max_runs, uint32_t *run_end, int64_t *run_gain, uint32_t *emit,
                     uint32_t *path_begin, uint64_t *path, uint32_t *dp_list, uint32_t *n_dp_list);
void launch_dp_long(hipStream_t s, const GraphPtrs &gp, const uint32_t *run_start, uint32_t max_runs, const uint2 *nrec,
                    int64_t *nscore, uint32_t *nbesti, uint32_t *n0_besti, uint32_t *run_end, int64_t *last_n0_score,
                    int64_t *run_gain, uint32_t *emit, uint32_t *path_begin, uint64_t *path, uint8_t *run_flag,
                    const uint32_t *dp_list, const uint32_t *n_dp_list);
void launch_dp_finish(hipStream_t s, const GraphPtrs &gp, const uint32_t *run_start, const uint32_t *n_runs,
                      const int64_t *nscore, const uint32_t *nbesti, const uint32_t *n0_besti, const int64_t *last_n0_score,
                      unsigned long long *total_gain, uint32_t *blocks_done, uint32_t *best_idx, const int64_t *run_gain,
                      const long long *tile_gain, uint32_t n_tiles, uint32_t *emit, uint32_t *path_begin, uint64_t *path);
void launch_bt_write(hipStream_t s, const GraphPtrs &gp, const uint32_t *run_start, const uint32_t *n_runs,
                     uint32_t run_bound, const uint32_t *emit, const uint32_t *eoff, const uint64_t *path,
                     uint32_t *cns_pos, uint8_t *cns_base, uint8_t *cns_cls, uint8_t *lq_nothead, uint32_t *lqc);
void launch_lq_list(hipStream_t s, const GraphPtrs &gp, const uint32_t *run_start, const uint32_t *n_runs,
                    uint32_t run_bound, const uint32_t *emit, const uint32_t *eoff, const uint64_t *path,
                    const uint32_t *lqoff, uint32_t cap, uint32_t *lq_list, uint32_t *err);
void launch_default_tail(hipStream_t s, const GraphPtrs &gp, const uint32_t *best_idx, const uint32_t *M_p, uint8_t *cns_base,
                         uint8_t *cns_cls, uint32_t *lq_list, uint32_t *n_lq, uint32_t cap, uint32_t *err);
void launch_lq_scan(hipStream_t s, const uint32_t *cns_pos, const uint8_t *cns_base, const uint8_t *cns_cls,
                    const uint32_t *M_p, const uint32_t *lq_list, const uint32_t *n_lq, uint32_t lq_cap, uint8_t *lq_kind,
                    uint32_t *lq_next, uint8_t *lq_nothead, uint32_t *hbits, uint32_t n_hwords, uint32_t *rstart, uint32_t *rend);
void launch_lq_merge_scan_lb(hipStream_t s, const Lookback &lb, const uint32_t *raw_start, const uint32_t *raw_end, const uint32_t *n_raw,
                             uint32_t n_host, uint32_t *headflag, uint32_t *hidx, uint32_t *err);
uint32_t lq_merge_lb_blocks();
void launch_lq_merge_scan(hipStream_t s, const uint32_t *raw_start, const uint32_t *raw_end, const uint32_t *n_raw, uint32_t n_host,
                          uint32_t *headflag, uint32_t *hidx);
void launch_scan_lb_popc(hipStream_t s, const Lookback &lb, const uint32_t *bits, uint32_t *out, uint32_t n_words, uint32_t *err);
void launch_lq_bits_count(hipStream_t s, const uint32_t *hbits, uint32_t n_words, uint32_t *wcnt);
void launch_scatter_regions(hipStream_t s, const uint32_t *hbits, uint32_t n_words, const uint32_t *woff,
                            const uint32_t *rstart, const uint32_t *rend, uint32_t *raw_start, uint32_t *raw_end,
                            uint32_t *n_raw);
void launch_lq_merge_flag(hipStream_t s, const uint32_t *raw_start, const uint32_t *raw_end, const uint32_t *n_raw,
                          uint32_t *headflag);
void launch_lq_merge_write(hipStream_t s, const uint32_t *raw_start, const uint32_t *raw_end, const uint32_t *n_raw,
                           const uint32_t *headflag, const uint32_t *hidx, uint32_t *lq_start, uint32_t *lq_end,
                           uint32_t *n_reg);
void launch_read_m(hipStream_t s, const np2_read_t *reads, uint32_t R, const uint8_t *alive, const uint32_t *lq_start,
                   uint32_t n_reg, int32_t *mval);
void launch_yak_insert(hipStream_t s, const uint64_t *words, const uint64_t *bucket_off, uint32_t n_buckets,
                       uint64_t max_bucket, uint64_t *table, uint32_t cap_log2, uint32_t *dup_flag, uint32_t gap = 0);
void launch_yak_insert_dup(hipStream_t s, const uint64_t *words, const uint64_t *bucket_off, uint32_t n_buckets,
                           uint64_t max_bucket, uint64_t *table, uint32_t cap_log2, uint32_t *ord, uint32_t gap = 0);
void launch_lookup(hipStream_t s, const YakDev &y, const uint64_t *hashes, uint64_t n, uint16_t min_count, uint16_t *out);
void launch_score_strings(hipStream_t s, const YakDev &y, const uint8_t *strs, const uint64_t *off, uint64_t n,
                          uint16_t min_count, uint16_t *out, bool own_strings);
void launch_cand_score(hipStream_t s, const YakDev &y, const uint32_t *cand_seq_off, const uint8_t *cand_seq,
                       const uint64_t *cand_kmer, const uint32_t *n_cand_p, uint32_t cand_cap, uint16_t min_count,
                       uint16_t *kscore, uint32_t *long_list, uint32_t *n_long);


void launch_pair_count(hipStream_t s, const np2_read_t *reads, uint32_t R, const uint8_t *alive,
                       const uint32_t *lq_start, const uint32_t *lq_end, uint32_t n_reg, const int32_t *smin,
                       uint32_t *pj, uint32_t *pcount, const uint64_t *ck_off, ReadInfo *rinfo);
void launch_scan_lb_excl(hipStream_t s, const Lookback &lb, const uint32_t *in, uint32_t *out, uint32_t n, bool write_end,
                          uint32_t *err);
uint32_t scan_lb_blocks(uint64_t n);
void launch_scan_small_excl(hipStream_t s, const uint32_t *in, uint32_t *out, uint32_t n, const uint32_t *n_dev,
                            uint32_t *total_out, bool write_end);
void launch_scan_small_incl(hipStream_t s, const int32_t *in, int32_t *out, uint32_t n, const uint32_t *n_dev);
void launch_scan_small_min(hipStream_t s, const int32_t *in, int32_t *out, uint32_t n, const uint32_t *n_dev);
void launch_region_measure(hipStream_t s, const CandPtrs &c, uint32_t n_reg, uint32_t *kept_read, uint32_t *kept_len,
                           uint32_t *kept_col, uint32_t *reg_ncand, uint32_t *reg_bytes, uint32_t *reg_maxlen,
                           uint32_t *blk_sum);
uint32_t cand_offsets_blocks(uint32_t n_reg);
void launch_cand_offsets(hipStream_t s, const uint32_t *blk_sum, uint32_t n_reg, uint32_t *blk_coff, uint32_t *blk_soff,
                         uint32_t *cand_off, uint32_t *reg_soff, uint32_t *n_cand, uint32_t *n_bytes, uint32_t *grow,
                         const Lookback *lb = nullptr, uint32_t *err = nullptr);
void launch_region_write(hipStream_t s, const CandPtrs &c, uint32_t n_reg, const uint32_t *kept_read,
                         const uint32_t *kept_len, const uint32_t *kept_col, const uint32_t *reg_ncand,
                         const uint32_t *reg_bytes, const uint32_t *blk_coff, const uint32_t *blk_soff, uint32_t *cand_off,
                         uint32_t *reg_soff, uint32_t cand_cap, uint32_t seq_cap, uint32_t *cand_order, uint64_t *cand_kmer,
                         uint32_t *cand_seq_off, uint8_t *cand_seq);

uint32_t tile_scan_blocks(uint32_t n_tiles);
void launch_tile_layout(hipStream_t s, uint32_t *tile_cur, uint32_t n_tiles, uint32_t bucket_cap, uint32_t *tile_n,
                        uint32_t *tile_scan, uint32_t *tile_scanb, const uint32_t *ovf_cnt, uint32_t *out,
                        const Lookback *lb = nullptr, uint32_t *err = nullptr);
void launch_tile_sort(hipStream_t s, uint16_t *pidx, const np2_read_t *reads, const uint8_t *nib, const uint32_t *tile_n,
                      uint32_t n_tiles, uint32_t bucket_cap, uint32_t max_tile, uint64_t *keys, uint32_t *vals,
                      uint32_t *err);
void launch_gather_buckets(hipStream_t s, const np2_read_t *reads, const uint8_t *nib, const uint32_t *tile_n,
                           const uint32_t *tile_scanb, uint32_t n_tiles, uint32_t bucket_cap, const uint64_t *bkeys,
                           const uint32_t *bvals, uint64_t *keys, uint32_t *vals);
void launch_gather_spill(hipStream_t s, const np2_read_t *reads, const uint8_t *nib, const uint64_t *okeys,
                         const uint32_t *ovals, uint32_t n, uint64_t *keys, uint32_t *vals);
void launch_tile_count(hipStream_t s, const uint64_t *keys, const uint32_t *vals, const uint32_t *tile_n,
                       const uint32_t *tile_scan, uint32_t bucket_cap, uint32_t n_tiles, const uint8_t *alive,
                       uint32_t *tile_nn, uint32_t *tile_nr);
void launch_tile_offsets(hipStream_t s, const uint32_t *tile_nn, const uint32_t *tile_nr, uint32_t n_tiles,
                         uint32_t *tile_noff, uint32_t *tile_roff, uint32_t *n_nodes, uint32_t *n_runs, uint32_t *reset,
                         uint32_t n_reset, const Lookback *lb = nullptr, uint32_t *err = nullptr,
                         const long long *tile_gain = nullptr, unsigned long long *gain_total = nullptr);
void launch_tile_write(hipStream_t s, const uint64_t *keys, const uint32_t *vals, const uint32_t *tile_n,
                       const uint32_t *tile_scan, uint32_t bucket_cap, const uint32_t *tile_noff, const uint32_t *tile_roff,
                       uint32_t n_tiles, const uint8_t *alive, uint32_t L, NodeArrays nd, uint2 *nrec, uint32_t *node_off,
                       uint32_t *run_start, const np2_read_t *reads, const uint32_t *tile_rd_off, const uint32_t *tile_rd,
                       int32_t *cov, const uint8_t *refnib, uint32_t *emit, long long *tile_gain, uint32_t *deep_flag, uint32_t deep_min,
                       uint8_t *pflag);

static constexpr uint32_t PF_CAP = 960;
static constexpr uint32_t PF_HALO = 64;
static constexpr uint32_t PF_CAP_MID = 2048;
static constexpr uint32_t PF_CAP_BIG = 3584;
static constexpr uint32_t PF_COV_MAX = 8192;
static constexpr uint32_t PF_REDO = 1u;
static constexpr uint32_t PF_NEED_BIG = 2u;
struct PfTile {
    const uint64_t *keys;
    const uint32_t *vals;
    const uint32_t *tile_n, *tile_scan;
    const uint16_t *pidx;
    const uint8_t *alive;
    const np2_read_t *reads;
    const uint32_t *tile_rd_off, *tile_rd;
    const uint8_t *refnib;
    uint16_t *slots;
    uint32_t *tile_cnt, *tile_lq;
    long long *tile_gain;
    uint32_t *flags, *n_bad, *bad_list, *n_bad2, *bad_list2;
    long long *end_rel;
    unsigned long long *gain_total;
    unsigned long long *prof;
    uint32_t L, n_tiles, bucket_cap;
    uint32_t cap_lim, cap_lim_big, halo_lim, cov_max;
    uint32_t big_enabled;
};
uint64_t pf_slot_entries(uint32_t n_tiles, uint64_t T);
void launch_pf_tile(hipStream_t s, const PfTile &a);
void launch_pf_compact(hipStream_t s, uint32_t n_tiles, const uint16_t *slots, const uint32_t *tile_scan, const uint32_t *tile_cnt,
                       const uint32_t *tile_coff, const uint32_t *tile_lqoff, uint32_t *cns_pos, uint8_t *cns_base,
                       uint8_t *cns_cls, uint8_t *lq_nothead, uint32_t *lq_list, uint32_t lq_cap, uint32_t *err, uint32_t *flags,
                       uint32_t *flags_out, uint32_t *n_bad, uint32_t *n_bad2);

struct RegionTables {
    const uint32_t *cand_off;
    const uint32_t *order;
    uint16_t *kscore;
    const uint32_t *seq_off;
    const uint8_t *seq;
    uint32_t n_reg;
};
struct RechPtrs {
    const void *groups;
    const uint32_t *job_off;
    const uint32_t *rech;
    const uint32_t *cand_off;
    const uint32_t *keep_list;
    const uint32_t *seq_off;
    const uint8_t *seq;
    const uint8_t *cns_base;
    uint32_t n_groups;
};
void launch_vote_phase(hipStream_t s, const RegionTables &rt, bool asref, bool use_all, const uint32_t *lq_start,
                       uint32_t own_lo, uint32_t own_hi, uint8_t *reg_lable, uint8_t *grp, uint32_t *ecount, int32_t *ref_w,
                       uint8_t *ref_seen, uint8_t *bad, uint32_t *first_reg, uint32_t *err);
void launch_vote_counts(hipStream_t s, const uint32_t *first_reg, const uint8_t *bad, uint32_t R, uint32_t *out);
void launch_edges_write(hipStream_t s, const RegionTables &rt, const uint8_t *reg_lable, const uint8_t *grp,
                        const uint32_t *ecount, const uint32_t *eoff, uint64_t *ekey, uint32_t *eval);
static constexpr uint32_t EDGE_BAND = 256;
void launch_edges_row(hipStream_t s, const RegionTables &rt, const uint8_t *grp, const uint32_t *ecount, const uint32_t *pj,
                      const uint32_t *pcount, const uint8_t *alive, uint32_t R, uint32_t *band, uint32_t *row_n, uint32_t *ovf);
void launch_band_emit(hipStream_t s, const uint32_t *band, uint32_t R, const uint32_t *row_off, uint64_t *ukey, uint32_t *uw,
                      uint32_t *n_out, uint64_t key_add = 0);
void launch_vote_rows_count(hipStream_t s, const uint32_t *band, const uint32_t *row_n, const uint8_t *bad, bool use_all, uint32_t R,
                            uint32_t *cnt, uint32_t *nokey);
void launch_vote_rows_emit(hipStream_t s, const uint32_t *band, const uint32_t *row_n, const uint8_t *bad, bool use_all,
                           const uint32_t *first_reg, uint32_t R, const uint32_t *off, void *edges, uint32_t *n_out, uint32_t *nokey);
void launch_edge_reduce(hipStream_t s, const uint64_t *ekey, const uint32_t *eval, uint32_t n, uint32_t *flag, uint32_t *wout);
void launch_edge_compact(hipStream_t s, const uint64_t *ekey, const uint32_t *flag, const uint32_t *idx, const uint32_t *wout,
                         uint32_t n, uint64_t *ukey, uint32_t *uw, uint32_t *n_out);
void launch_seed(hipStream_t s, const RegionTables &rt, int32_t max_indel_len, uint8_t *reg_lable, uint32_t *seed_cand,
                 uint32_t *keep_n, uint32_t *keep_list, uint16_t *keep_ks, uint32_t *err);
uint32_t region_lb_blocks(uint32_t n_reg);
void launch_splice_find(hipStream_t s, const uint32_t *cns_pos, const uint32_t *M_p, const uint32_t *lq_start,
                        const uint32_t *lq_end, const uint8_t *reg_lable, uint8_t lable, uint32_t n_reg, uint32_t *idx_s,
                        uint32_t *idx_e, uint32_t *stuck);
void launch_splice_plan(hipStream_t s, const Lookback &lb, const uint8_t *reg_lable, uint8_t lable, uint32_t n_reg,
                        const uint32_t *stuck, const uint32_t *idx_s, const uint32_t *idx_e, const uint32_t *seed_cand,
                        const uint32_t *seq_off, uint32_t *ap_g, uint32_t *ap_s, uint32_t *ap_e, int32_t *ap_delta,
                        int32_t *ap_shift_incl, uint32_t *n_ap, const uint32_t *M_in, uint32_t *M_out, uint32_t out_cap , uint32_t *err);
void launch_splice_write(hipStream_t s, const uint32_t *in_pos, const uint8_t *in_base, const uint32_t *M_p, uint32_t M_cap,
                         const uint32_t *ap_g, const uint32_t *ap_s, const uint32_t *ap_e, const int32_t *ap_delta,
                         const int32_t *ap_shift_incl, const uint32_t *n_ap, uint32_t max_ap, const uint32_t *lq_start,
                         const uint32_t *seed_cand, const uint32_t *seq_off, const uint8_t *seq, uint32_t *out_pos,
                         uint8_t *out_base);
void launch_shard_bounds(hipStream_t s, const uint32_t *cns_pos, const uint32_t *M_p, const uint32_t *t, uint32_t *out);
void launch_rech_list(hipStream_t s, const Lookback &lb, const uint8_t *reg_lable, uint32_t n_reg, uint32_t *rech,
                      uint32_t *n_rech, unsigned long long *blob_bound, uint32_t *err);
void launch_rech_groups(hipStream_t s, const Lookback &lb, const uint32_t *rech, const uint32_t *n_rech_p, uint32_t max_rech,
                        const uint32_t *cns_pos, const uint32_t *M_p, const uint32_t *lq_start, const uint32_t *lq_end,
                        const uint32_t *keep_n, uint32_t ksize, const uint32_t *reg_maxlen, void *tmp_groups,
                        uint32_t *head_jobs, void *groups, uint32_t *job_off, uint32_t *n_groups, uint32_t *n_jobs,
                        unsigned long long *blob_bound, uint32_t *err);
size_t rech_group_bytes();
void launch_rech_job_len(hipStream_t s, const RechPtrs &p, uint32_t n_jobs, uint32_t *len);
void launch_rech_job_build(hipStream_t s, const RechPtrs &p, uint32_t n_jobs, const uint32_t *soff32, uint64_t *soff64,
                           uint8_t *blob);
void launch_rech_apply(hipStream_t s, const RechPtrs &p, const uint16_t *score, uint16_t *keep_ks);
void launch_rech_select(hipStream_t s, const uint32_t *rech, const uint32_t *n_rech_p, uint32_t max_rech,
                        const uint32_t *cand_off, const uint32_t *keep_n, const uint32_t *keep_list, const uint16_t *keep_ks,
                        const uint32_t *order, bool first_yak, uint8_t *reg_lable, uint32_t *seed_cand);
void launch_rech_relabel(hipStream_t s, uint8_t *reg_lable, uint32_t n_reg);

struct FrontOp {
    uint32_t col0, q0, t0;
    uint32_t len_type;
};
struct FrontRec {
    uint32_t pos, n_ops;
    uint64_t op_off;
    uint64_t seq_off;
    uint64_t out_off;
    uint32_t n_cols;
    uint32_t pad;
};
struct FrontOut {
    uint32_t aln_t_s, aln_t_e, n_cols, pad;
};
void launch_columnarise(hipStream_t s, const FrontRec *recs, uint32_t n_recs, const FrontOp *ops, const uint8_t *ref,
                        const uint8_t *seq4, uint8_t *nib, FrontOut *out);
void launch_pack_ref(hipStream_t s, const uint8_t *ref, uint32_t L, uint8_t *dst);

size_t prim_temp_bytes(size_t n);
int prim_sort_pairs_u64_u32(hipStream_t s, void *tmp, size_t tmp_bytes, const uint64_t *kin, uint64_t *kout,
                            const uint32_t *vin, uint32_t *vout, size_t n, unsigned end_bit);
int prim_exclusive_sum_u32(hipStream_t s, void *tmp, size_t tmp_bytes, const uint32_t *in, uint32_t *out, size_t n);
int prim_inclusive_sum_i32(hipStream_t s, void *tmp, size_t tmp_bytes, const int32_t *in, int32_t *out, size_t n);
int prim_inclusive_min_i32(hipStream_t s, void *tmp, size_t tmp_bytes, const int32_t *in, int32_t *out, size_t n);

}
```

### nextpolish2_amd/csrc/np2_regions.hip

```cpp
#include "np2_common.hpp"
#include "np2_kernels.hpp"
#include "np2_blockscan.hpp"
#include "np2_lookback.hpp"

namespace np2 {

static constexpr uint8_t LB_TEMP = 0x01, LB_SUCC = 0x80, LB_HETE = 0x40, LB_RECH = 0x20;

__device__ __forceinline__ uint32_t min_support(uint32_t n) { return n >= 9 ? 3u : (n >= 6 ? 2u : 1u); }

struct SubWave {
    uint32_t base;
    bool half;
    __device__ __forceinline__ uint64_t ballot(bool p) const {
        const uint64_t b = __ballot(p);
        return half ? (b >> base) & 0xFFFFFFFFull : b;
    }
    template <class T> __device__ __forceinline__ T shfl(T v, uint32_t j) const { return __shfl(v, (int)(base + j)); }
};

struct WaveStats {
    uint64_t eqmask;
    uint32_t stat;
    uint32_t c;
// ... 366 lines not shown
        for (uint32_t k = 0; k < EDGE_BAND / 64; ++k) {
            const uint32_t d = k * 64 + lane;
            if (own) c += vote_row_above(band, bad, use_all, R, v, d) != 0;
            c += vote_row_below(band, row_n, bad, use_all, v, (int64_t)v - 1 - d) != 0;
        }
    }
    for (int o = 32; o > 0; o >>= 1) c += __shfl_xor(c, o);
    if (lane == 0) cnt[v] = c;
}
__device__ __forceinline__ void k_vote_rows_emit(const uint32_t np2_bid, const uint32_t np2_nb, const uint32_t *__restrict__ band,
                                                 const uint32_t *__restrict__ row_n, const uint8_t *__restrict__ bad, uint32_t use_all,
                                                 const uint32_t *__restrict__ first_reg, uint32_t R, const uint32_t *__restrict__ off,
                                                 uint2 *__restrict__ edges, uint32_t *__restrict__ n_out, uint32_t *__restrict__ nokey) {
    const uint32_t lane = threadIdx.x & 63;
    const uint32_t v = (uint32_t)__builtin_amdgcn_readfirstlane((int)((np2_bid * blockDim.x + threadIdx.x) >> 6));
    if (v >= R) return;
    if (v == R - 1 && lane == 0) *n_out = off[R];
    if (v == 0) return;
    const bool own = row_n[v] != 0, live = use_all || !bad[v];
    const uint64_t lt = (1ull << lane) - 1;
    uint32_t o = off[v];
    const uint32_t end = off[v + 1];
    if (live && end != o) {
#pragma unroll
        for (uint32_t k = 0; k < EDGE_BAND / 64; ++k) {
            const int64_t a = (int64_t)v - EDGE_BAND + k * 64 + lane;
            const uint32_t w = vote_row_below(band, row_n, bad, use_all, v, a);
            const uint64_t m = __ballot(w != 0);
            const uint32_t at = o + (uint32_t)__popcll(m & lt);
            if (w != 0 && at < end) edges[at] = make_uint2((uint32_t)a, __float_as_uint(vote_weight(w)));
            o += (uint32_t)__popcll(m);
        }
    }
    if (!own) return;
    const bool v_key = first_reg[v] != 0xFFFFFFFFu;
    uint32_t nk = 0;
#pragma unroll
    for (uint32_t k = 0; k < EDGE_BAND / 64; ++k) {
        const uint32_t d = k * 64 + lane, b = v + 1 + d;
        if (b < R && band[(uint64_t)v * EDGE_BAND + d] != 0 && !(v_key && first_reg[b] != 0xFFFFFFFFu)) ++nk;
        const uint32_t w = live ? vote_row_above(band, bad, use_all, R, v, d) : 0u;
        const uint64_t m = __ballot(w != 0);
        const uint32_t at = o + (uint32_t)__popcll(m & lt);
        if (w != 0 && at < end) edges[at] = make_uint2(b, __float_as_uint(vote_weight(w)));
        o += (uint32_t)__popcll(m);
    }
    for (int x = 32; x > 0; x >>= 1) nk += __shfl_xor(nk, x);
    if (nk && lane == 0) atomicAdd(nokey, nk);
}

__device__ __forceinline__ void k_edge_reduce(const uint32_t np2_bid, const uint32_t np2_nb, const uint64_t *__restrict__ ekey, const uint32_t *__restrict__ eval, uint32_t n,
                              uint32_t *__restrict__ flag, uint32_t *__restrict__ wout) {
    uint32_t i = np2_bid * blockDim.x + threadIdx.x;
    if (i >= n) return;
    const uint64_t k = ekey[i];
    if (i > 0 && ekey[i - 1] == k) {
        flag[i] = 0;
        return;
    }
    int32_t sum = 0, neg = 0;
    for (uint32_t j = i; j < n && ekey[j] == k; ++j) {
        const int32_t w = (int32_t)eval[j];
        sum += w;
        neg += w < 0;
    }
    flag[i] = 1;
    wout[i] = (uint32_t)(sum + neg) | ((uint32_t)neg << 16);
}
__device__ __forceinline__ void k_edge_compact(const uint32_t np2_bid, const uint32_t np2_nb, const uint64_t *__restrict__ ekey, const uint32_t *__restrict__ flag,
                               const uint32_t *__restrict__ idx, const uint32_t *__restrict__ wout, uint32_t n,
                               uint64_t *__restrict__ ukey, uint32_t *__restrict__ uw, uint32_t *__restrict__ n_out) {
    uint32_t i = np2_bid * blockDim.x + threadIdx.x;
    if (i >= n) return;
    if (flag[i]) {
        ukey[idx[i]] = ekey[i];
        uw[idx[i]] = wout[i];
    }
    if (i == n - 1) *n_out = idx[i] + flag[i];
}

__device__ __forceinline__ void k_seed(const uint32_t np2_bid0, const uint32_t np2_nb, RegionTables rt, int32_t max_indel_len,
                                              uint8_t *__restrict__ reg_lable, uint32_t *__restrict__ seed_cand,
                                              uint32_t *__restrict__ keep_n, uint32_t *__restrict__ keep_list,
                                              uint16_t *__restrict__ keep_ks, uint32_t *__restrict__ err) {
    const uint32_t np2_bid = xcd_order(np2_bid0, np2_nb);
    const uint32_t wl = threadIdx.x & 63;
    const uint32_t g0 = (uint32_t)__builtin_amdgcn_readfirstlane((int)((np2_bid * blockDim.x + threadIdx.x) >> 6)) * 2;
    if (g0 >= rt.n_reg) return;
    const bool has1 = g0 + 1 < rt.n_reg;
    const bool packed = has1 && rt.cand_off[g0 + 1] - rt.cand_off[g0] <= 32 && rt.cand_off[g0 + 2] - rt.cand_off[g0 + 1] <= 32;
    const uint32_t rounds = (has1 && !packed) ? 2u : 1u;
    for (uint32_t round = 0; round < rounds; ++round) {
        const SubWave sw{packed ? (wl & 32u) : 0u, packed};
        const uint32_t lane = packed ? (wl & 31u) : wl;
        const uint32_t g = packed ? g0 + (wl >> 5) : g0 + round;
        const uint32_t c0 = rt.cand_off[g], n = rt.cand_off[g + 1] - c0;
        if (n == 0) {
            if (lane == 0) {
                atomicOr(err, 8u);
                reg_lable[g] = 0;
                keep_n[g] = 0;
                seed_cand[g] = 0;
            }
            continue;
        }
        uint32_t so = 0, len = 0, order = 0xFFFFFFFFu;
        uint16_t ks = 0;
        if (lane < n) {
            so = rt.seq_off[c0 + lane];
            len = rt.seq_off[c0 + lane + 1] - so;
            order = rt.order[c0 + lane];
            ks = rt.kscore[c0 + lane];
        }
        WaveStats w = wave_group_stats(sw, lane, n, so, len, rt.seq, ks > 0, order);
        const uint32_t min_c = min_support(n);
        if (sw.shfl(order, 0) != 0) {
            if (lane == 0) atomicOr(err, 16u);
        }
        uint32_t key = w.head ? w.c : 0;
        {
            const bool has0 = sw.shfl((uint32_t)w.head, 0) != 0;
            uint32_t k0 = sw.shfl(key, 0);
            if (has0) {
                if (k0 > 1 && k0 < min_c) k0 = min_c;
            } else {
                const uint32_t cnt0 = __builtin_popcountll(sw.shfl((uint32_t)(w.eqmask & 0xFFFFFFFFu), 0)) +
                                      __builtin_popcountll(sw.shfl((uint32_t)(w.eqmask >> 32), 0));
                if (cnt0 > 1) k0 = min_c;
            }
            const bool dup = lane >= 1 && lane < n && lane < 63 && ((w.eqmask >> (lane + 1)) != 0);
            const bool nodup = sw.ballot(dup) == 0;
            if (w.max1_p != 0 && w.max1_c < min_c && (w.max1_c > 1 || nodup)) {
                if (lane == w.max1_p) key = min_c;
                k0 = min_c;
            } else if (w.max1_c < min_c) {
                k0 = min_c;
            }
            if (lane == 0) key = k0;
        }
        const bool kept = lane < n && key >= min_c;
        uint32_t rank = 0;
        for (uint64_t it = sw.ballot(kept); it; it &= it - 1) {
            const uint32_t j = (uint32_t)__builtin_ctzll(it);
            const uint32_t kj = sw.shfl(key, j);
            if (kept && (kj > key || (kj == key && j < lane))) ++rank;
        }
        uint32_t kn = __builtin_popcountll(sw.ballot(kept));
        if (kn == 0) {
            if (lane == 0) atomicOr(err, 32u);
            kn = 0;
        }
        const uint64_t r0mask = sw.ballot(kept && rank == 0);
        const uint32_t first = r0mask ? __builtin_ctzll(r0mask) : 0;
        uint32_t seed = w.max1_p;
        const int32_t d = (int32_t)sw.shfl(len, w.max1_p) - (int32_t)sw.shfl(len, first);
        const bool too_long = (d < 0 ? -d : d) > max_indel_len;
        uint8_t lable = LB_SUCC | LB_RECH;
        if (kn <= 1 || too_long) {
            seed = first;
            lable = LB_SUCC;
            kn = 0;
        }
        if (kept && kn) {
            keep_list[c0 + rank] = c0 + lane;
            keep_ks[c0 + rank] = ks;
        }
        if (lane == 0) {
            reg_lable[g] = lable;
            seed_cand[g] = c0 + seed;
            keep_n[g] = kn;
        }
    }
}

template <bool UPPER>
__device__ __forceinline__ uint32_t bound16_u32(const uint32_t *__restrict__ a, uint32_t n, uint32_t v, uint32_t lo0 = 0) {
    uint32_t lo = lo0, hi = n;
    while (lo < hi) {
        const uint32_t step = (hi - lo + 15) >> 4;
        uint32_t x[16];
#pragma unroll
        for (uint32_t k = 0; k < 16; ++k) x[k] = a[min(lo + k * step, hi - 1)];
        uint32_t c = 0;
#pragma unroll
        for (uint32_t k = 0; k < 16; ++k) c += (lo + k * step < hi && (UPPER ? x[k] <= v : x[k] < v)) ? 1u : 0u;
        const uint32_t n_probe = (hi - lo + step - 1) / step;
        const uint32_t nlo = c ? lo + (c - 1) * step + 1 : lo;
        const uint32_t nhi = c < n_probe ? lo + c * step : hi;
        lo = nlo, hi = nhi;
    }
    return lo;
}
__device__ __forceinline__ uint32_t lower_bound_u32(const uint32_t *a, uint32_t n, uint32_t v) {
    return bound16_u32<false>(a, n, v);
}
__device__ __forceinline__ uint32_t upper_bound_u32(const uint32_t *a, uint32_t n, uint32_t v) {
    return bound16_u32<true>(a, n, v);
}

__device__ __forceinline__ void k_splice_find(const uint32_t np2_bid, const uint32_t np2_nb, const uint32_t *__restrict__ cns_pos, const uint32_t *__restrict__ M_p,
                              const uint32_t *__restrict__ lq_start,
                              const uint32_t *__restrict__ lq_end, const uint8_t *__restrict__ reg_lable,
                              uint8_t lable, uint32_t n_reg, uint32_t *__restrict__ idx_s, uint32_t *__restrict__ idx_e,
                              uint32_t *__restrict__ stuck) {
    uint32_t g = np2_bid * blockDim.x + threadIdx.x;
    if (g >= n_reg || !(reg_lable[g] & lable)) return;
    const uint32_t M = *M_p;
    const uint32_t s = lower_bound_u32(cns_pos, M, lq_start[g]);
    const bool found = s < M && cns_pos[s] == lq_start[g];
    idx_s[g] = s;
    uint32_t e = s;
    if (found) {
        const uint32_t en = lq_end[g];
        const uint32_t near = (uint32_t)min((uint64_t)M, (uint64_t)s + (en - lq_start[g]) + 65u);
        e = (near == M || cns_pos[near - 1] > en) ? bound16_u32<true>(cns_pos, near, en, s) : upper_bound_u32(cns_pos, M, en);
        e = max(s, e);
    }
    idx_e[g] = e;
    if (!found) atomicMax(stuck, g + 1);
}
static constexpr uint32_t LB_REG_ITEMS = 4;
__device__ __forceinline__ void k_splice_plan(const uint32_t np2_bid, const uint32_t np2_nb, Lookback lb, uint32_t n_blocks, const uint8_t *__restrict__ reg_lable,
                                                     uint8_t lable, uint32_t n_reg, const uint32_t *__restrict__ stuck,
                                                     const uint32_t *__restrict__ idx_s, const uint32_t *__restrict__ idx_e,
                                                     const uint32_t *__restrict__ seed_cand,
                                                     const uint32_t *__restrict__ seq_off, uint32_t *__restrict__ ap_g,
                                                     uint32_t *__restrict__ ap_s, uint32_t *__restrict__ ap_e,
                                                     int32_t *__restrict__ ap_delta, int32_t *__restrict__ ap_shift_incl,
                                                     uint32_t *__restrict__ n_ap, const uint32_t *__restrict__ M_in,
                                                     uint32_t *__restrict__ M_out, uint32_t out_cap, uint32_t *__restrict__ err) {
    __shared__ uint32_t sh[8];
    const uint32_t bid = lb_block_id(lb, sh);
    uint32_t flag[LB_REG_ITEMS], g[LB_REG_ITEMS], s[LB_REG_ITEMS], e[LB_REG_ITEMS];
    int32_t delta[LB_REG_ITEMS];
    uint32_t fsum = 0;
    int32_t dsum_t = 0;
#pragma unroll
    for (uint32_t k = 0; k < LB_REG_ITEMS; ++k) {
        const uint32_t rr = (bid * 256 + threadIdx.x) * LB_REG_ITEMS + k;
        flag[k] = 0, g[k] = 0, s[k] = 0, e[k] = 0, delta[k] = 0;
        if (rr < n_reg) {
            g[k] = n_reg - 1 - rr;
            flag[k] = ((reg_lable[g[k]] & lable) && g[k] + 1 > *stuck) ? 1u : 0u;
            if (flag[k]) {
                const uint32_t c = seed_cand[g[k]];
                s[k] = idx_s[g[k]], e[k] = idx_e[g[k]];
                delta[k] = (int32_t)(seq_off[c + 1] - seq_off[c]) - (int32_t)(e[k] - s[k]);
            }
        }
        fsum += flag[k];
        dsum_t += delta[k];
    }
    uint32_t cnt, dsum;
    uint32_t lo = block_excl_scan<OpAdd, 4>(fsum, sh, cnt);
    uint32_t ld = block_excl_scan<OpAdd, 4>((uint32_t)dsum_t, sh, dsum);
    uint32_t pre_c, pre_d;
    lb_exclusive2(lb, bid, cnt, dsum, sh, err, pre_c, pre_d);
#pragma unroll
    for (uint32_t k = 0; k < LB_REG_ITEMS; ++k) {
        if (flag[k]) {
            const uint32_t o = pre_c + lo;
            ap_g[o] = g[k];
            ap_s[o] = s[k];
            ap_e[o] = e[k];
            ap_delta[o] = delta[k];
            ap_shift_incl[o] = (int32_t)(pre_d + ld) + delta[k];
        }
        lo += flag[k];
        ld += (uint32_t)delta[k];
    }
    if (bid == n_blocks - 1 && threadIdx.x == 0) {
        const uint32_t m_out = *M_in + pre_d + dsum;
        if (m_out > out_cap) {
            atomicOr(err, GROW_ERR);
            *n_ap = 0;
            *M_out = *M_in;
        } else {
            *n_ap = pre_c + cnt;
            *M_out = m_out;
        }
    }
}
static constexpr uint32_t SPLICE_SPAN = 2048;
static constexpr uint32_t SPLICE_LDS_SLOTS = 256;
__device__ __forceinline__ void k_splice_bases(const uint32_t np2_bid, const uint32_t np2_nb, const uint32_t *__restrict__ in_pos,
                                                      const uint8_t *__restrict__ in_base,
                                                      const uint32_t *__restrict__ M_p,
                                                      const uint32_t *__restrict__ ap_s, const uint32_t *__restrict__ ap_e,
                                                      const int32_t *__restrict__ ap_shift_incl,
                                                      const uint32_t *__restrict__ n_ap_p, uint32_t *__restrict__ out_pos,
                                                      uint8_t *__restrict__ out_base) {
    __shared__ uint32_t s_lo[2];
    __shared__ uint32_t s_s[SPLICE_LDS_SLOTS], s_e[SPLICE_LDS_SLOTS];
    __shared__ int32_t s_sh[SPLICE_LDS_SLOTS];
    const uint32_t i0 = np2_bid * SPLICE_SPAN;
    const uint32_t n_ap = *n_ap_p, M = *M_p;
    if (i0 >= M) return;
    uint32_t pv[SPLICE_SPAN / 256];
    uint8_t bv[SPLICE_SPAN / 256];
#pragma unroll
    for (uint32_t k = 0; k < SPLICE_SPAN / 256; ++k) {
        const uint32_t i = min(i0 + k * 256 + threadIdx.x, M - 1);
        pv[k] = in_pos[i], bv[k] = in_base[i];
    }
    if (threadIdx.x < 2)
        s_lo[threadIdx.x] = upper_bound_u32(ap_s, n_ap, threadIdx.x == 0 ? i0 : min(M - 1, i0 + SPLICE_SPAN - 1));
    __syncthreads();
    const uint32_t blo = s_lo[0], bhi = s_lo[1], b0 = blo ? blo - 1 : 0u;
    const bool staged = bhi - b0 <= SPLICE_LDS_SLOTS;
    if (staged && b0 + threadIdx.x < bhi) {
        s_s[threadIdx.x] = ap_s[b0 + threadIdx.x];
        s_e[threadIdx.x] = ap_e[b0 + threadIdx.x];
        s_sh[threadIdx.x] = ap_shift_incl[b0 + threadIdx.x];
    }
    __syncthreads();
#pragma unroll
    for (uint32_t k = 0; k < SPLICE_SPAN / 256; ++k) {
        const uint32_t i = i0 + k * 256 + threadIdx.x;
        if (i >= M) break;
        uint32_t lo = blo, hi = bhi;
        int64_t o = i;
        if (staged) {
            while (lo < hi) {
                const uint32_t mid = (lo + hi) >> 1;
                if (s_s[mid - b0] <= i) lo = mid + 1; else hi = mid;
            }
            if (lo > 0) {
                if (i < s_e[lo - 1 - b0]) continue;
                o += s_sh[lo - 1 - b0];
            }
        } else {
            while (lo < hi) {
                const uint32_t mid = (lo + hi) >> 1;
                if (ap_s[mid] <= i) lo = mid + 1; else hi = mid;
            }
            if (lo > 0) {
                const uint32_t sl = lo - 1;
                if (i < ap_e[sl]) continue;
                o += ap_shift_incl[sl];
            }
        }
        out_pos[o] = pv[k];
        out_base[o] = bv[k];
    }
}
__device__ __forceinline__ void k_splice_seeds(const uint32_t np2_bid, const uint32_t np2_nb, const uint32_t *__restrict__ ap_g, const uint32_t *__restrict__ ap_s,
                               const int32_t *__restrict__ ap_delta, const int32_t *__restrict__ ap_shift_incl,
                               const uint32_t *__restrict__ n_ap_p, const uint32_t *__restrict__ lq_start,
                               const uint32_t *__restrict__ seed_cand, const uint32_t *__restrict__ seq_off,
                               const uint8_t *__restrict__ seq, uint32_t *__restrict__ out_pos,
                               uint8_t *__restrict__ out_base) {
    const uint32_t sl = (np2_bid * blockDim.x + threadIdx.x) >> 3, q = threadIdx.x & 7u;
    if (sl >= *n_ap_p) return;
    const uint32_t g = ap_g[sl], c = seed_cand[g];
    const uint32_t so = seq_off[c], len = seq_off[c + 1] - so;
    const int64_t o = (int64_t)ap_s[sl] + (ap_shift_incl[sl] - ap_delta[sl]);
    const uint32_t p = lq_start[g];
    for (uint32_t t = q; t < len; t += 8) {
        out_pos[o + t] = p;
        out_base[o + t] = seq[so + t];
    }
}

__device__ __forceinline__ void k_shard_bounds(const uint32_t np2_bid, const uint32_t np2_nb, const uint32_t *__restrict__ cns_pos, const uint32_t *__restrict__ M_p,
                                               uint32_t t0, uint32_t t1, uint32_t t2, uint32_t t3, uint32_t t4, uint32_t t5,
                                               uint32_t *__restrict__ out) {
    __shared__ uint32_t s_i[6];
    const uint32_t M = *M_p;
    const uint32_t t[6] = {t0, t1, t2, t3, t4, t5};
    if (threadIdx.x < 6) {
        uint32_t tv = t[0];
#pragma unroll
        for (uint32_t k = 1; k < 6; ++k) tv = threadIdx.x == k ? t[k] : tv;
        const uint32_t i = lower_bound_u32(cns_pos, M, tv);
        out[threadIdx.x] = i;
        s_i[threadIdx.x] = i;
    }
    __syncthreads();
    if (threadIdx.x == 0) {
        const uint32_t a = s_i[1], b = s_i[4];
        out[6] = b > a ? cns_pos[a] : 0u;
        out[7] = b > a ? cns_pos[b - 1] : 0u;
    }
}

__device__ __forceinline__ void k_rech_list(const uint32_t np2_bid, const uint32_t np2_nb, Lookback lb, uint32_t n_blocks, const uint8_t *__restrict__ reg_lable,
                                                   uint32_t n_reg, uint32_t *__restrict__ rech, uint32_t *__restrict__ n_rech,
                                                   unsigned long long *__restrict__ blob_bound, uint32_t *__restrict__ err) {
    __shared__ uint32_t sh[8];
    if (np2_bid == 0 && threadIdx.x == 0) *blob_bound = 0;
    const uint32_t bid = lb_block_id(lb, sh);
    uint32_t flag[LB_REG_ITEMS], fsum = 0;
#pragma unroll
    for (uint32_t k = 0; k < LB_REG_ITEMS; ++k) {
        const uint32_t rr = (bid * 256 + threadIdx.x) * LB_REG_ITEMS + k;
        flag[k] = (rr < n_reg && (reg_lable[n_reg - 1 - rr] & LB_RECH)) ? 1u : 0u;
        fsum += flag[k];
    }
    uint32_t cnt, pre, dummy;
    uint32_t lo = block_excl_scan<OpAdd, 4>(fsum, sh, cnt);
    lb_exclusive2(lb, bid, cnt, 0u, sh, err, pre, dummy);
#pragma unroll
    for (uint32_t k = 0; k < LB_REG_ITEMS; ++k) {
        if (flag[k]) rech[pre + lo] = n_reg - 1 - ((bid * 256 + threadIdx.x) * LB_REG_ITEMS + k);
        lo += flag[k];
    }
    if (bid == n_blocks - 1 && threadIdx.x == 0) *n_rech = pre + cnt;
}

struct RechGroup {
    uint32_t first, n;
    uint32_t sl, el, sr, er;
    uint32_t bs[5], be[5];
    uint32_t lens[6];
    uint32_t njobs;
};

__device__ __forceinline__ void k_rech_groups(const uint32_t np2_bid, const uint32_t np2_nb, const uint32_t *__restrict__ rech,
                                                     const uint32_t *__restrict__ n_rech_p,
                                                     const uint32_t *__restrict__ cns_pos, const uint32_t *__restrict__ M_p,
                                                     const uint32_t *__restrict__ lq_start,
                                                     const uint32_t *__restrict__ lq_end,
                                                     const uint32_t *__restrict__ keep_n, uint32_t ksize,
                                                     const uint32_t *__restrict__ reg_maxlen,
                                                     RechGroup *__restrict__ tmp_groups, uint32_t *__restrict__ head_jobs,
                                                     unsigned long long *__restrict__ blob_bound,
                                                     uint32_t *__restrict__ err) {
    __shared__ unsigned long long s_bound[4];
    unsigned long long bound = 0;
    const uint32_t e = np2_bid * 256 + threadIdx.x;
    const uint32_t n_rech = *n_rech_p, M = *M_p;
    auto chained = [&](uint32_t x) { return lq_start[rech[x]] < lq_end[rech[x - 1]] + ksize; };
    bool head = false;
    RechGroup G = {};
    uint32_t jobs32 = 0;
    if (e < n_rech) {
        uint32_t back = 0, x = e;
        while (x > 0 && chained(x)) {
            --x;
            ++back;
        }
        head = back % 6 == 0;
    }
    if (head) {
        G.first = e;
        uint32_t n = 1;
        while (n < 6 && e + n < n_rech && chained(e + n)) ++n;
        G.n = n;
        const uint32_t l = ksize - 1;
        const uint32_t p0 = lq_start[rech[e]];
        const uint32_t i0 = lower_bound_u32(cns_pos, M, p0);
        if (i0 == 0 || i0 >= M) atomicOr(err, 64u);
        G.el = i0;
        G.sl = i0 > l ? i0 - l : 0;
        const uint32_t p1 = lq_end[rech[e + n - 1]];
        const uint32_t i1u = upper_bound_u32(cns_pos, M, p1);
        if (i1u == 0 || i1u >= M) atomicOr(err, 64u);
        const uint32_t i1 = i1u ? i1u - 1 : 0;
        G.sr = i1 + 1;
        G.er = (i1 + l < M) ? i1 + l + 1 : M;
        uint64_t jobs = 1;
#pragma unroll
        for (uint32_t x = 0; x < 6; ++x) {
            if (x >= n) break;
            G.lens[x] = keep_n[rech[e + x]];
            jobs *= G.lens[x];
            if (jobs > 0x7FFFFFFFull) {
                atomicOr(err, 128u);
                jobs = 0;
            }
            if (x + 1 < n) {
                const uint32_t s = lq_end[rech[e + x]], en = lq_start[rech[e + x + 1]];
                if (s + 1 == en) {
                    G.bs[x] = G.be[x] = 0;
                } else {
                    G.bs[x] = upper_bound_u32(cns_pos, M, s);
                    G.be[x] = lower_bound_u32(cns_pos, M, en);
                    if (G.be[x] < G.bs[x]) G.be[x] = G.bs[x];
                }
            }
        }
        jobs32 = (uint32_t)jobs;
        G.njobs = jobs32;
        uint64_t len = (uint64_t)(G.el - G.sl) + (G.er - G.sr);
#pragma unroll
        for (uint32_t x = 0; x < 6; ++x) {
            if (x >= n) break;
            len += reg_maxlen[rech[e + x]];
            if (x + 1 < n) len += G.be[x] - G.bs[x];
        }
        bound = (unsigned long long)jobs32 * len;
        tmp_groups[e] = G;
    }
    if (e < n_rech) head_jobs[e] = head ? jobs32 + 1u : 0u;
    for (int o = 32; o > 0; o >>= 1) bound += __shfl_xor(bound, o);
    if ((threadIdx.x & 63) == 0) s_bound[threadIdx.x >> 6] = bound;
    __syncthreads();
    if (threadIdx.x == 0) {
        const unsigned long long b = s_bound[0] + s_bound[1] + s_bound[2] + s_bound[3];
        if (b) atomicAdd(blob_bound, b);
    }
}
__device__ __forceinline__ void k_rech_compact(const uint32_t np2_bid, const uint32_t np2_nb, Lookback lb, uint32_t n_blocks,
                                                      const uint32_t *__restrict__ n_rech_p,
                                                      const uint32_t *__restrict__ head_jobs,
                                                      const RechGroup *__restrict__ tmp_groups,
                                                      RechGroup *__restrict__ groups, uint32_t *__restrict__ job_off,
                                                      uint32_t *__restrict__ n_groups, uint32_t *__restrict__ n_jobs,
                                                      uint32_t *__restrict__ err) {
    __shared__ uint32_t sh[8];
    const uint32_t bid = lb_block_id(lb, sh);
    const uint32_t n_rech = *n_rech_p;
    uint32_t hj[LB_REG_ITEMS], hs = 0, js = 0;
#pragma unroll
    for (uint32_t k = 0; k < LB_REG_ITEMS; ++k) {
        const uint32_t e = (bid * 256 + threadIdx.x) * LB_REG_ITEMS + k;
        hj[k] = e < n_rech ? head_jobs[e] : 0u;
        hs += hj[k] ? 1u : 0u;
        js += hj[k] ? hj[k] - 1u : 0u;
    }
    uint32_t nh, nj, pre_h, pre_j;
    uint32_t lh = block_excl_scan<OpAdd, 4>(hs, sh, nh);
    uint32_t lj = block_excl_scan<OpAdd, 4>(js, sh, nj);
    lb_exclusive2(lb, bid, nh, nj, sh, err, pre_h, pre_j);
    if (pre_j + nj < pre_j) atomicOr(err, 128u);
#pragma unroll
    for (uint32_t k = 0; k < LB_REG_ITEMS; ++k) {
        if (!hj[k]) continue;
        const uint32_t e = (bid * 256 + threadIdx.x) * LB_REG_ITEMS + k;
        groups[pre_h + lh] = tmp_groups[e];
        job_off[pre_h + lh] = pre_j + lj;
        ++lh;
        lj += hj[k] - 1u;
    }
    if (bid == n_blocks - 1 && threadIdx.x == 0) {
        *n_groups = pre_h + nh;
        *n_jobs = pre_j + nj;
        job_off[pre_h + nh] = pre_j + nj;
    }
}

struct RechCtx {
    const RechGroup *groups;
    const uint32_t *job_off;
    const uint32_t *rech;
    const uint32_t *cand_off;
    const uint32_t *keep_list;
    const uint32_t *seq_off;
    const uint8_t *seq;
    const uint8_t *cns_base;
    uint32_t n_groups;
};
__device__ __forceinline__ uint32_t job_group(const RechCtx &cx, uint32_t job) {
    uint32_t lo = 0, hi = cx.n_groups;
    while (lo < hi) {
        const uint32_t mid = (lo + hi) >> 1;
        if (cx.job_off[mid] <= job) lo = mid + 1; else hi = mid;
    }
    return lo - 1;
}
template <bool WRITE> __device__ uint32_t rech_string(const RechCtx &cx, uint32_t job, uint8_t *__restrict__ out) {
    const uint32_t gi = job_group(cx, job);
    const RechGroup &G = cx.groups[gi];
    uint32_t rem = job - cx.job_off[gi];
    uint32_t pick[6];
    for (uint32_t x = G.n; x-- > 0;) {
        pick[x] = rem % G.lens[x];
        rem /= G.lens[x];
    }
    uint32_t o = 0;
    for (uint32_t i = G.sl; i < G.el; ++i, ++o)
        if (WRITE) out[o] = cx.cns_base[i];
    for (uint32_t x = 0; x < G.n; ++x) {
        const uint32_t g = cx.rech[G.first + x];
        const uint32_t c = cx.keep_list[cx.cand_off[g] + pick[x]];
        const uint32_t so = cx.seq_off[c], len = cx.seq_off[c + 1] - so;
        for (uint32_t t = 0; t < len; ++t, ++o)
            if (WRITE) out[o] = cx.seq[so + t];
        if (x + 1 < G.n)
            for (uint32_t i = G.bs[x]; i < G.be[x]; ++i, ++o)
                if (WRITE) out[o] = cx.cns_base[i];
    }
    for (uint32_t i = G.sr; i < G.er; ++i, ++o)
        if (WRITE) out[o] = cx.cns_base[i];
    return o;
}
__device__ __forceinline__ void k_rech_job_len(const uint32_t np2_bid, const uint32_t np2_nb, RechCtx cx, uint32_t n_jobs, uint32_t *__restrict__ len) {
    uint32_t j = np2_bid * blockDim.x + threadIdx.x;
    if (j < n_jobs) len[j] = rech_string<false>(cx, j, nullptr);
}
__device__ __forceinline__ void k_rech_job_build(const uint32_t np2_bid, const uint32_t np2_nb, RechCtx cx, uint32_t n_jobs, const uint64_t *__restrict__ soff,
                                 uint8_t *__restrict__ blob) {
    uint32_t j = np2_bid * blockDim.x + threadIdx.x;
    if (j < n_jobs) rech_string<true>(cx, j, blob + soff[j]);
}
__device__ __forceinline__ void k_u32_to_u64_off(const uint32_t np2_bid, const uint32_t np2_nb, const uint32_t *__restrict__ in, uint32_t n, uint64_t *__restrict__ out) {
    uint32_t i = np2_bid * blockDim.x + threadIdx.x;
    if (i < n) out[i] = in[i];
}

__device__ __forceinline__ void k_rech_apply(const uint32_t np2_bid, const uint32_t np2_nb, RechCtx cx, const uint16_t *__restrict__ score, uint16_t *__restrict__ keep_ks) {
    uint32_t gi = np2_bid * blockDim.x + threadIdx.x;
    if (gi >= cx.n_groups) return;
    const RechGroup &G = cx.groups[gi];
    const uint32_t j0 = cx.job_off[gi];
    if (G.n == 1) {
        const uint32_t g = cx.rech[G.first];
        for (uint32_t t = 0; t < G.lens[0]; ++t) keep_ks[cx.cand_off[g] + t] = score[j0 + t];
        return;
    }
    for (uint32_t x = 0; x < G.n; ++x) {
        const uint32_t g = cx.rech[G.first + x];
        for (uint32_t t = 0; t < G.lens[x]; ++t) keep_ks[cx.cand_off[g] + t] = 0;
    }
    for (uint32_t j = 0; j < G.njobs; ++j) {
        const uint16_t ks = score[j0 + j];
        if (!ks) continue;
        uint32_t rem = j;
        for (uint32_t x = G.n; x-- > 0;) {
            const uint32_t p = rem % G.lens[x];
            rem /= G.lens[x];
            keep_ks[cx.cand_off[cx.rech[G.first + x]] + p] = ks;
        }
    }
}

__device__ __forceinline__ void k_rech_select(const uint32_t np2_bid, const uint32_t np2_nb, const uint32_t *__restrict__ rech, const uint32_t *__restrict__ n_rech_p,
                              const uint32_t *__restrict__ cand_off, const uint32_t *__restrict__ keep_n,
                              const uint32_t *__restrict__ keep_list, const uint16_t *__restrict__ keep_ks,
                              const uint32_t *__restrict__ order, uint32_t first_yak, uint8_t *__restrict__ reg_lable,
                              uint32_t *__restrict__ seed_cand) {
    uint32_t e = np2_bid * blockDim.x + threadIdx.x;
    if (e >= *n_rech_p) return;
    const uint32_t g = rech[e], c0 = cand_off[g], n = keep_n[g];
    uint32_t c = 0, valid = 0;
    for (uint32_t p = 0; p < n; ++p)
        if (keep_ks[c0 + p] != 0) {
            if (c == 0 || order[keep_list[c0 + p]] == 0) c = p + 1;
            ++valid;
        }
    if (valid > 1) reg_lable[g] |= LB_TEMP;
    if (c != 0) {
        seed_cand[g] = keep_list[c0 + c - 1];
    } else if (first_yak) {
        uint32_t i = 0;
        for (uint32_t p = 0; p < n; ++p)
            if (order[keep_list[c0 + p]] == 0) {
                i = p;
                break;
            }
        seed_cand[g] = keep_list[c0 + i];
    }
}
__device__ __forceinline__ void k_rech_relabel(const uint32_t np2_bid, const uint32_t np2_nb, uint8_t *__restrict__ reg_lable, uint32_t n_reg) {
    uint32_t g = np2_bid * blockDim.x + threadIdx.x;
    if (g >= n_reg) return;
    const uint8_t l = reg_lable[g];
    if (!(l & LB_RECH)) return;
    reg_lable[g] = (l & LB_TEMP) ? (uint8_t)(l ^ LB_TEMP) : (uint8_t)(l ^ LB_RECH);
}

__device__ __forceinline__ void k_vote_counts(const uint32_t np2_bid, const uint32_t np2_nb, const uint32_t *__restrict__ first_reg, const uint8_t *__restrict__ bad,
                                                      uint32_t R, uint32_t *__restrict__ out) {
    __shared__ uint32_t sk[16], sb[16];
    uint32_t nk = 0, nb = 0;
    for (uint32_t r = threadIdx.x; r < R; r += 1024) {
        nk += first_reg[r] != 0xFFFFFFFFu ? 1u : 0u;
        nb += bad[r] ? 1u : 0u;
    }
    for (int o = 32; o > 0; o >>= 1) {
        nk += __shfl_xor(nk, o);
        nb += __shfl_xor(nb, o);
    }
    if ((threadIdx.x & 63) == 0) {
        sk[threadIdx.x >> 6] = nk;
        sb[threadIdx.x >> 6] = nb;
    }
    __syncthreads();
    if (threadIdx.x == 0) {
        uint32_t a = 0, b = 0;
        for (int i = 0; i < 16; ++i) {
            a += sk[i];
            b += sb[i];
        }
        out[0] = a;
        out[1] = b;
    }
}

static inline dim3 g1(uint64_t n, uint32_t bs = 256) { return dim3((unsigned)((n + bs - 1) / bs)); }

void launch_vote_phase(hipStream_t s, const RegionTables &rt, bool asref, bool use_all, const uint32_t *lq_start,
                       uint32_t own_lo, uint32_t own_hi, uint8_t *reg_lable, uint8_t *grp, uint32_t *ecount, int32_t *ref_w,
                       uint8_t *ref_seen, uint8_t *bad, uint32_t *first_reg, uint32_t *err) {
    if (rt.n_reg)
        NP2_LAUNCH(k_vote_phase, g1((uint64_t)((rt.n_reg + 1) / 2) * 64), 256, s, rt, asref ? 1u : 0u, use_all ? 1u : 0u, lq_start, own_lo, own_hi, reg_lable, grp, ecount, ref_w, ref_seen, bad, first_reg, err);
}
void launch_vote_counts(hipStream_t s, const uint32_t *first_reg, const uint8_t *bad, uint32_t R, uint32_t *out) {
    NP2_LAUNCH(k_vote_counts, dim3(1), 1024, s, first_reg, bad, R, out);
}
void launch_edges_write(hipStream_t s, const RegionTables &rt, const uint8_t *reg_lable, const uint8_t *grp,
                        const uint32_t *ecount, const uint32_t *eoff, uint64_t *ekey, uint32_t *eval) {
    if (rt.n_reg)
        NP2_LAUNCH(k_edges_write, g1((uint64_t)rt.n_reg * 64), 256, s, rt, reg_lable, grp, ecount, eoff, ekey, eval);
}
void launch_edges_row(hipStream_t s, const RegionTables &rt, const uint8_t *grp, const uint32_t *ecount, const uint32_t *pj,
                      const uint32_t *pcount, const uint8_t *alive, uint32_t R, uint32_t *band, uint32_t *row_n, uint32_t *ovf) {
    if (R) NP2_LAUNCH(k_edges_row, g1((uint64_t)R * 64), 256, s, rt, grp, ecount, pj, pcount, alive, R, band, row_n, ovf);
}
void launch_vote_rows_count(hipStream_t s, const uint32_t *band, const uint32_t *row_n, const uint8_t *bad, bool use_all, uint32_t R,
                            uint32_t *cnt, uint32_t *nokey) {
    if (R) NP2_LAUNCH(k_vote_rows_count, g1((uint64_t)R * 64), 256, s, band, row_n, bad, use_all ? 1u : 0u, R, cnt, nokey);
}
void launch_vote_rows_emit(hipStream_t s, const uint32_t *band, const uint32_t *row_n, const uint8_t *bad, bool use_all,
                           const uint32_t *first_reg, uint32_t R, const uint32_t *off, void *edges, uint32_t *n_out, uint32_t *nokey) {
    if (R) NP2_LAUNCH(k_vote_rows_emit, g1((uint64_t)R * 64), 256, s, band, row_n, bad, use_all ? 1u : 0u, first_reg, R, off, (uint2 *)edges, n_out, nokey);
}
void launch_band_emit(hipStream_t s, const uint32_t *band, uint32_t R, const uint32_t *row_off, uint64_t *ukey, uint32_t *uw,
                      uint32_t *n_out, uint64_t key_add) {
    if (R) NP2_LAUNCH(k_band_emit, g1((uint64_t)R * 64), 256, s, band, R, row_off, ukey, uw, n_out, key_add);
}
void launch_edge_reduce(hipStream_t s, const uint64_t *ekey, const uint32_t *eval, uint32_t n, uint32_t *flag,
                        uint32_t *wout) {
    if (n) NP2_LAUNCH(k_edge_reduce, g1(n), 256, s, ekey, eval, n, flag, wout);
}
void launch_edge_compact(hipStream_t s, const uint64_t *ekey, const uint32_t *flag, const uint32_t *idx,
                         const uint32_t *wout, uint32_t n, uint64_t *ukey, uint32_t *uw, uint32_t *n_out) {
    if (n) NP2_LAUNCH(k_edge_compact, g1(n), 256, s, ekey, flag, idx, wout, n, ukey, uw, n_out);
}
void launch_seed(hipStream_t s, const RegionTables &rt, int32_t max_indel_len, uint8_t *reg_lable, uint32_t *seed_cand,
                 uint32_t *keep_n, uint32_t *keep_list, uint16_t *keep_ks, uint32_t *err) {
    if (rt.n_reg)
        NP2_LAUNCH(k_seed, g1((uint64_t)((rt.n_reg + 1) / 2) * 64), 256, s, rt, max_indel_len, reg_lable, seed_cand, keep_n, keep_list, keep_ks, err);
}
uint32_t region_lb_blocks(uint32_t n_reg) { return (n_reg + 256 * LB_REG_ITEMS - 1) / (256 * LB_REG_ITEMS); }
void launch_splice_find(hipStream_t s, const uint32_t *cns_pos, const uint32_t *M_p, const uint32_t *lq_start,
                        const uint32_t *lq_end, const uint8_t *reg_lable, uint8_t lable, uint32_t n_reg,
                        uint32_t *idx_s, uint32_t *idx_e, uint32_t *stuck) {
    NP2_LAUNCH(k_splice_find, g1(n_reg), 256, s, cns_pos, M_p, lq_start, lq_end, reg_lable, lable, n_reg, idx_s, idx_e, stuck);
}
void launch_splice_plan(hipStream_t s, const Lookback &lb, const uint8_t *reg_lable, uint8_t lable, uint32_t n_reg,
                        const uint32_t *stuck, const uint32_t *idx_s, const uint32_t *idx_e, const uint32_t *seed_cand,
                        const uint32_t *seq_off, uint32_t *ap_g, uint32_t *ap_s, uint32_t *ap_e, int32_t *ap_delta,
                        int32_t *ap_shift_incl, uint32_t *n_ap, const uint32_t *M_in, uint32_t *M_out, uint32_t out_cap, uint32_t *err) {
    const uint32_t nb = region_lb_blocks(n_reg);
    NP2_LAUNCH(k_splice_plan, dim3(nb), 256, s, lb, nb, reg_lable, lable, n_reg, stuck, idx_s, idx_e, seed_cand, seq_off, ap_g, ap_s, ap_e, ap_delta, ap_shift_incl, n_ap, M_in, M_out, out_cap, err);
}
void launch_splice_write(hipStream_t s, const uint32_t *in_pos, const uint8_t *in_base, const uint32_t *M_p, uint32_t M_cap,
                         const uint32_t *ap_g, const uint32_t *ap_s, const uint32_t *ap_e, const int32_t *ap_delta,
                         const int32_t *ap_shift_incl, const uint32_t *n_ap, uint32_t max_ap, const uint32_t *lq_start,
                         const uint32_t *seed_cand, const uint32_t *seq_off, const uint8_t *seq, uint32_t *out_pos,
                         uint8_t *out_base) {
    NP2_LAUNCH(k_splice_bases, dim3((M_cap + SPLICE_SPAN - 1) / SPLICE_SPAN), 256, s, in_pos, in_base, M_p, ap_s, ap_e, ap_shift_incl, n_ap, out_pos, out_base);
    if (max_ap)
        NP2_LAUNCH(k_splice_seeds, g1((uint64_t)max_ap * 8, 256), 256, s, ap_g, ap_s, ap_delta, ap_shift_incl, n_ap, lq_start, seed_cand, seq_off, seq, out_pos, out_base);
}
void launch_shard_bounds(hipStream_t s, const uint32_t *cns_pos, const uint32_t *M_p, const uint32_t *t, uint32_t *out) {
    NP2_LAUNCH(k_shard_bounds, dim3(1), 64, s, cns_pos, M_p, t[0], t[1], t[2], t[3], t[4], t[5], out);
}
void launch_rech_list(hipStream_t s, const Lookback &lb, const uint8_t *reg_lable, uint32_t n_reg, uint32_t *rech,
                      uint32_t *n_rech, unsigned long long *blob_bound, uint32_t *err) {
    const uint32_t nb = region_lb_blocks(n_reg);
    NP2_LAUNCH(k_rech_list, dim3(nb), 256, s, lb, nb, reg_lable, n_reg, rech, n_rech, blob_bound, err);
}
void launch_rech_groups(hipStream_t s, const Lookback &lb, const uint32_t *rech, const uint32_t *n_rech_p, uint32_t max_rech,
                        const uint32_t *cns_pos, const uint32_t *M_p, const uint32_t *lq_start, const uint32_t *lq_end,
                        const uint32_t *keep_n, uint32_t ksize, const uint32_t *reg_maxlen, void *tmp_groups,
                        uint32_t *head_jobs, void *groups, uint32_t *job_off, uint32_t *n_groups, uint32_t *n_jobs,
                        unsigned long long *blob_bound, uint32_t *err) {
    NP2_LAUNCH(k_rech_groups, dim3((max_rech + 255) / 256), 256, s, rech, n_rech_p, cns_pos, M_p, lq_start, lq_end, keep_n, ksize, reg_maxlen, (RechGroup *)tmp_groups, head_jobs, blob_bound, err);
    const uint32_t nb = region_lb_blocks(max_rech);
    NP2_LAUNCH(k_rech_compact, dim3(nb), 256, s, lb, nb, n_rech_p, head_jobs, (const RechGroup *)tmp_groups, (RechGroup *)groups, job_off, n_groups, n_jobs, err);
}
size_t rech_group_bytes() { return sizeof(RechGroup); }
static RechCtx mk_rech(const RechPtrs &p) {
    return RechCtx{(const RechGroup *)p.groups, p.job_off, p.rech, p.cand_off, p.keep_list, p.seq_off, p.seq,
                   p.cns_base, p.n_groups};
}
void launch_rech_job_len(hipStream_t s, const RechPtrs &p, uint32_t n_jobs, uint32_t *len) {
    if (n_jobs) NP2_LAUNCH(k_rech_job_len, g1(n_jobs, 64), 64, s, mk_rech(p), n_jobs, len);
}
void launch_rech_job_build(hipStream_t s, const RechPtrs &p, uint32_t n_jobs, const uint32_t *soff32, uint64_t *soff64,
                           uint8_t *blob) {
    if (!n_jobs) return;
    NP2_LAUNCH(k_u32_to_u64_off, g1(n_jobs + 1), 256, s, soff32, n_jobs + 1, soff64);
    NP2_LAUNCH(k_rech_job_build, g1(n_jobs, 64), 64, s, mk_rech(p), n_jobs, soff64, blob);
}
void launch_rech_apply(hipStream_t s, const RechPtrs &p, const uint16_t *score, uint16_t *keep_ks) {
    if (p.n_groups) NP2_LAUNCH(k_rech_apply, g1(p.n_groups, 64), 64, s, mk_rech(p), score, keep_ks);
}
void launch_rech_select(hipStream_t s, const uint32_t *rech, const uint32_t *n_rech_p, uint32_t max_rech,
                        const uint32_t *cand_off, const uint32_t *keep_n, const uint32_t *keep_list,
                        const uint16_t *keep_ks, const uint32_t *order, bool first_yak, uint8_t *reg_lable,
                        uint32_t *seed_cand) {
    if (max_rech)
        NP2_LAUNCH(k_rech_select, g1(max_rech, 64), 64, s, rech, n_rech_p, cand_off, keep_n, keep_list, keep_ks, order, first_yak ? 1u : 0u, reg_lable, seed_cand);
}
void launch_rech_relabel(hipStream_t s, uint8_t *reg_lable, uint32_t n_reg) {
    NP2_LAUNCH(k_rech_relabel, g1(n_reg), 256, s, reg_lable, n_reg);
}

}
```

Baseline: 4318.

## Drive recheck rounds from a device-built region list without host readbacks

The seed kernel now emits a compact list of RECH regions. Each k-mer table's recheck runs as a fixed chain of launches: a single-block prepare, a job-scoring kernel and a single-block finish that splices and forwards the surviving list. This avoids the per-table host readback of counts and the full-region passes that were sized by the total region count. The risk is that fixed capacities can overflow; an overflow raises a new error flag, and the pass is then redone on the general path. Small single-block kernels may also limit parallelism when lists are large.

```diff
diff --git a/nextpolish2_amd/csrc/np2_common.hpp b/nextpolish2_amd/csrc/np2_common.hpp
--- a/nextpolish2_amd/csrc/np2_common.hpp
+++ b/nextpolish2_amd/csrc/np2_common.hpp
@@ -82,6 +82,7 @@
 
 enum : uint8_t { CLS_HQ = 0, CLS_LQ = 1, CLS_RESET = 2 };
 static constexpr uint32_t GROW_ERR = 0x1000u;
+static constexpr uint32_t RECH_CAP_ERR = 0x2000u;
 static constexpr uint32_t LQ_LIST_ERR = 0x800u;
 
 static constexpr uint32_t CKPT_SHIFT = 5;
diff --git a/nextpolish2_amd/csrc/np2_ctx.hpp b/nextpolish2_amd/csrc/np2_ctx.hpp
--- a/nextpolish2_amd/csrc/np2_ctx.hpp
+++ b/nextpolish2_amd/csrc/np2_ctx.hpp
@@ -499,6 +499,8 @@
     DevBuf<uint8_t> reg_lable, grp, cns_base2, rech_groups, rech_groups_tmp;
     DevBuf<uint8_t> votepack;
     DevBuf<uint8_t> votepack2;
+    DevBuf<uint32_t> rl_list, rl_blob_off, rl_glen;
+    DevBuf<uint2> rl_job_ol;
     DevBuf<uint32_t> rech_headjobs;
     DevBuf<uint32_t> ecount, eval, eval_s, eflag, eidx, seed_cand, keep_n, keep_list, cns_pos2, sp_idx_s,
         sp_idx_e, ap_g, ap_s, ap_e, rech, rech_joboff, job_len,
@@ -534,8 +536,9 @@
     struct Hooks {
         bool front_unfused = false, pf_prof = false, edge_sort = false;
         bool test_misspeculate = false, shard_spec_log = false, phase_profile = false, exact_grow = false, no_speculate = false;
-        bool has_grow_guess = false;
+        bool has_grow_guess = false, rech_general = false, rech_log = false;
         uint32_t grow_guess = 0;
+        uint32_t rech_cap_list = 0xFFFFFFFFu, rech_cap_jobs = 0xFFFFFFFFu, rech_cap_blob = 0xFFFFFFFFu;
         bool has_pf_cap = false, has_pf_cap_big = false, has_pf_halo = false, has_pf_cov_max = false;
         uint32_t pf_cap = 0, pf_cap_big = 0, pf_halo = 0, pf_cov_max = 0;
         void read() {
@@ -547,6 +550,14 @@
             test_misspeculate = on("NP2_TEST_MISSPECULATE");
             shard_spec_log = on("NP2_SHARD_SPEC_LOG"), phase_profile = on("NP2_PHASE_PROFILE"), exact_grow = on("NP2_EXACT_GROW");
             no_speculate = on("NP2_NO_SPECULATE");
+            rech_general = on("NP2_RECH_GENERAL");
+            rech_log = on("NP2_RECH_LOG");
+            if (const char *e = getenv("NP2_TEST_RECH_CAP")) {
+                char *end = nullptr;
+                rech_cap_list = (uint32_t)strtoul(e, &end, 10);
+                if (end && *end == ',') rech_cap_jobs = (uint32_t)strtoul(end + 1, &end, 10);
+                if (end && *end == ',') rech_cap_blob = (uint32_t)strtoul(end + 1, &end, 10);
+            }
             u32("NP2_TEST_GROW_GUESS", has_grow_guess, grow_guess);
             u32("NP2_PF_CAP", has_pf_cap, pf_cap), u32("NP2_PF_CAP_BIG", has_pf_cap_big, pf_cap_big);
             u32("NP2_PF_HALO", has_pf_halo, pf_halo), u32("NP2_PF_COV_MAX", has_pf_cov_max, pf_cov_max);
@@ -573,6 +584,8 @@
 static constexpr int NP2_MAX_YAK = 15;
 static constexpr uint32_t SCAL_TOTAL = 96;
 static_assert(S_COUNT + 2 * (NP2_MAX_YAK + 2) <= SCAL_TOTAL && S_COUNT < 64, "round counters behind the posted block; the mailbox holds 64 words");
+static constexpr uint32_t S_RL = S_COUNT + 2 * (NP2_MAX_YAK + 2);
+static_assert(S_RL + 2 + np2::RL_STATE_WORDS <= SCAL_TOTAL, "the region lists' counters fit behind the round counters");
 
 inline double thread_cpu_ms() {
     timespec ts;
diff --git a/nextpolish2_amd/csrc/np2_host.cpp b/nextpolish2_amd/csrc/np2_host.cpp
--- a/nextpolish2_amd/csrc/np2_host.cpp
+++ b/nextpolish2_amd/csrc/np2_host.cpp
@@ -119,7 +119,8 @@
 }
 
 struct GrowRetry : Np2Error {
-    GrowRetry() : Np2Error(NP2_E_DEVICE, "internal: guessed growth allowance too small") {}
+    bool grow, rech_cap;
+    GrowRetry(bool g, bool r) : Np2Error(NP2_E_DEVICE, g ? "internal: guessed growth allowance too small" : "internal: recheck region list too small"), grow(g), rech_cap(r) {}
 };
 void check_region_err(np2_ctx *cx, uint32_t e) {
     (void)cx;
@@ -130,7 +131,7 @@
     if (e & 64u) throw Np2Error(NP2_E_REFPANIC, "reference would panic: consensus index out of bounds in reupdate");
     if (e & 128u) throw Np2Error(NP2_E_NOMEM, "cartesian product of chained LQ regions is too large");
     if (e & LB_ERR) throw Np2Error(NP2_E_DEVICE, "device-wide scan timed out waiting for a predecessor block");
-    if (e & GROW_ERR) throw GrowRetry();
+    if (e & (GROW_ERR | RECH_CAP_ERR)) throw GrowRetry((e & GROW_ERR) != 0, (e & RECH_CAP_ERR) != 0);
     if (e & LQ_LIST_ERR) throw Np2Error(NP2_E_DEVICE, "internal: more low-quality bases than their list was sized for");
 }
 
@@ -481,22 +482,29 @@
     uint32_t M_cap;
 };
 
-CnsDev splice_gpu(np2_ctx *cx, const CnsDev &in, uint32_t n_reg, uint8_t lable, uint32_t grow_bound, bool to_b,
-                  uint32_t version) {
-    hipStream_t s = cx->stream;
-    EventTimer t(cx, "splice");
-    cx->sp_idx_s.ensure(n_reg + 2);
-    cx->sp_idx_e.ensure(n_reg + 2);
-    cx->ap_g.ensure(n_reg + 2);
-    cx->ap_s.ensure(n_reg + 2);
-    cx->ap_e.ensure(n_reg + 2);
-    cx->ap_delta.ensure(n_reg + 2);
-    cx->ap_shift.ensure(n_reg + 2);
+CnsDev splice_buffers(np2_ctx *cx, const CnsDev &in, uint32_t n_slots, uint32_t grow_bound, bool to_b, uint32_t version) {
+    cx->sp_idx_s.ensure(n_slots + 2);
+    cx->sp_idx_e.ensure(n_slots + 2);
+    cx->ap_g.ensure(n_slots + 2);
+    cx->ap_s.ensure(n_slots + 2);
+    cx->ap_e.ensure(n_slots + 2);
+    cx->ap_delta.ensure(n_slots + 2);
+    cx->ap_shift.ensure(n_slots + 2);
     cx->mlen.ensure(16);
     const uint32_t out_cap = in.M_cap + grow_bound;
     const size_t cap = (size_t)out_cap + 64;
     uint32_t *opos = to_b ? cx->cns_pos2.ensure(cap) : cx->cns_pos.ensure(cap);
     uint8_t *obase = to_b ? cx->cns_base2.ensure(cap) : cx->cns_base.ensure(cap);
+    return CnsDev{opos, obase, cx->mlen.p + version, out_cap};
+}
+CnsDev splice_gpu(np2_ctx *cx, const CnsDev &in, uint32_t n_reg, uint8_t lable, uint32_t grow_bound, bool to_b,
+                  uint32_t version) {
+    hipStream_t s = cx->stream;
+    EventTimer t(cx, "splice");
+    const CnsDev out = splice_buffers(cx, in, n_reg, grow_bound, to_b, version);
+    uint32_t *const opos = out.pos;
+    uint8_t *const obase = out.base;
+    const uint32_t out_cap = out.M_cap;
     uint32_t *const stuck_p = cx->scal.p + S_COUNT + 2 * version, *const nap_p = stuck_p + 1;
     launch_splice_find(s, in.pos, in.M_p, cx->lq_start.p, cx->lq_end.p, cx->reg_lable.p, lable, n_reg, cx->sp_idx_s.p,
                        cx->sp_idx_e.p, stuck_p);
@@ -507,7 +515,7 @@
     launch_splice_write(s, in.pos, in.base, in.M_p, in.M_cap, cx->ap_g.p, cx->ap_s.p, cx->ap_e.p, cx->ap_delta.p,
                         cx->ap_shift.p, nap_p, n_reg, cx->lq_start.p, cx->seed_cand.p, cx->cand_seq_off.p,
                         cx->cand_seq.p, opos, obase);
-    return CnsDev{opos, obase, cx->mlen.p + version, out_cap};
+    return out;
 }
 
 Cns fetch_cns_dev(np2_ctx *cx, const CnsDev &c) {
@@ -516,6 +524,49 @@
     r.pos = d2h(cx, c.pos, M);
     r.base = d2h(cx, c.base, M);
     return r;
+}
+
+bool rech_by_list(const np2_ctx *cx, uint32_t n_reg) {
+    return !cx->trace && !cx->hooks.rech_general && n_reg <= RL_NREG_MAX;
+}
+uint32_t rech_list_cap(const np2_ctx *cx) { return std::min(cx->hooks.rech_cap_list, RL_CAP_LIST); }
+uint32_t *rech_list_of(np2_ctx *cx, size_t y) { return cx->rl_list.p + (y & 1) * RL_CAP_LIST; }
+uint32_t *rech_list_cnt(np2_ctx *cx, size_t y) { return cx->scal.p + S_RL + (y & 1); }
+
+CnsDev recheck_list_gpu(np2_ctx *cx, const CnsDev &in, const PassCounts &pc, int yak_idx, uint16_t min_kmer_count,
+                        bool first_yak, bool last_yak, bool to_b, uint32_t version) {
+    hipStream_t s = cx->stream;
+    EventTimer t(cx, "recheck");
+    const uint32_t ksize = cx->yaks[yak_idx].k;
+    const uint32_t cap_jobs = std::min(cx->hooks.rech_cap_jobs, RL_CAP_JOBS), cap_blob = std::min(cx->hooks.rech_cap_blob, RL_CAP_BLOB);
+    cx->rech.ensure(RL_CAP_LIST + 2);
+    cx->rech_groups.ensure((size_t)(RL_CAP_LIST + 2) * rech_group_bytes());
+    cx->rech_groups_tmp.ensure((size_t)(RL_CAP_LIST + 2) * rech_group_bytes());
+    cx->rech_joboff.ensure(RL_CAP_LIST + 2);
+    cx->rl_blob_off.ensure(RL_CAP_LIST + 2);
+    cx->rl_glen.ensure(RL_CAP_LIST + 2);
+    cx->rl_job_ol.ensure(RL_CAP_JOBS + 2);
+    cx->sstr.ensure((size_t)RL_CAP_BLOB + 64);
+    cx->sscore.ensure(RL_CAP_JOBS + 2);
+    const CnsDev out = splice_buffers(cx, in, std::max(pc.n_reg, RL_CAP_LIST), pc.grow, to_b, version);
+    uint32_t *const st = cx->scal.p + S_RL + 2, *const nap_p = cx->scal.p + S_COUNT + 2 * version + 1;
+    const RechList rl{rech_list_of(cx, (size_t)yak_idx), rech_list_cnt(cx, (size_t)yak_idx), rech_list_of(cx, (size_t)yak_idx + 1),
+                      rech_list_cnt(cx, (size_t)yak_idx + 1), st, cx->rech.p, cx->sp_idx_s.p, cx->sp_idx_e.p, cx->rech_groups.p, cx->rech_groups_tmp.p,
+                      cx->rech_joboff.p, cx->rl_blob_off.p, cx->rl_glen.p, cx->rl_job_ol.p, cx->sstr.p,
+                      rech_list_cap(cx), cap_jobs, cap_blob};
+    launch_rech_prepare(s, rl, in.pos, in.base, in.M_p, cx->lq_start.p, cx->lq_end.p, cx->keep_n.p, ksize, cx->reg_maxlen.p,
+                        cx->cand_off.p, cx->keep_list.p, cx->cand_seq_off.p, cx->cand_seq.p, cx->scal.p + S_ERR);
+    launch_score_jobs(s, cx->yaks[yak_idx].dev(), cx->sstr.p, cx->rl_job_ol.p, st + RL_NJOBS, min_kmer_count,
+                      cx->sscore.p);
+    launch_rech_finish(s, rl, cx->sscore.p, cx->keep_ks.p, cx->cand_off.p, cx->keep_n.p, cx->keep_list.p, cx->cand_order.p,
+                       first_yak, last_yak, cx->reg_lable.p, cx->seed_cand.p, in.pos, in.M_p, cx->lq_start.p,
+                       cx->cand_seq_off.p, cx->ap_g.p, cx->ap_s.p, cx->ap_e.p, cx->ap_delta.p, cx->ap_shift.p, nap_p, cx->mlen.p + version,
+                       out.M_cap, cx->scal.p + S_ERR);
+    launch_splice_write(s, in.pos, in.base, in.M_p, in.M_cap, cx->ap_g.p, cx->ap_s.p, cx->ap_e.p, cx->ap_delta.p,
+                        cx->ap_shift.p, nap_p, RL_CAP_LIST, cx->lq_start.p, cx->seed_cand.p, cx->cand_seq_off.p,
+                        cx->cand_seq.p, out.pos, out.base);
+    cx->timing.host.push_back({"rech_list", 1.0f});
+    return out;
 }
 
 CnsDev recheck_gpu(np2_ctx *cx, const CnsDev &in, const PassCounts &pc, int yak_idx, uint16_t min_kmer_count,
@@ -544,6 +595,9 @@
         n_rech = sc[S_NRECH];
         n_groups = sc[S_NGROUPS];
         n_jobs = sc[S_M0];
+        if (cx->hooks.rech_log)
+            fprintf(stderr, "np2 recheck, table %d: %u regions, %u RECH, %u groups, %u jobs, %llu string bytes at most\n", yak_idx, n_reg,
+                    n_rech, n_groups, n_jobs, (unsigned long long)blob_bound);
     }
     if (n_rech) {
         RechPtrs rp{cx->rech_groups.p, cx->rech_joboff.p, cx->rech.p, cx->cand_off.p, cx->keep_list.p,
@@ -1210,7 +1264,7 @@
     ++r.pass;
 }
 
-void run_final_pass(PolishRun &r, ResultOut &result, bool exact_grow = false) {
+void run_final_pass(PolishRun &r, ResultOut &result, bool exact_grow = false, bool rech_general = false) {
     np2_ctx *cx = r.cx;
     np2_contig *c = r.c;
     hipStream_t s = cx->stream;
@@ -1239,13 +1293,16 @@
             pc.resolve(fetch_scal(cx));
         }
     }
+    const bool by_list = !rech_general && !cx->yaks.empty() && rech_by_list(cx, n_reg);
     try {
         cx->keep_list.ensure((size_t)pc.NC_cap + 2);
         cx->keep_ks.ensure((size_t)pc.NC_cap + 2);
+        if (by_list) cx->rl_list.ensure(2 * (size_t)RL_CAP_LIST);
         {
             EventTimer t(cx, "seed");
             launch_seed(s, rt, r.o.max_indel_len, cx->reg_lable.p, cx->seed_cand.p, cx->keep_n.p, cx->keep_list.p,
-                        cx->keep_ks.p, cx->scal.p + S_ERR);
+                        cx->keep_ks.p, cx->scal.p + S_ERR, by_list ? rech_list_of(cx, 0) : nullptr,
+                        by_list ? rech_list_cnt(cx, 0) : nullptr, rech_list_cap(cx));
         }
         if (cx->trace) check_region_err(cx, d2h(cx, cx->scal.p + S_ERR, 1)[0]);
         trace_region_tables(cx, (int)r.pass, "seed", pc, true);
@@ -1256,18 +1313,21 @@
         to_b = !to_b;
         if (cx->trace) trace_cns(cx, (int)r.pass, "cns_succ", fetch_cns_dev(cx, cur));
         for (size_t y = 0; y < cx->yaks.size(); ++y) {
-            cur = recheck_gpu(cx, cur, pc, (int)y, r.o.min_kmer_count, y == 0, to_b, version++);
+            cur = by_list ? recheck_list_gpu(cx, cur, pc, (int)y, r.o.min_kmer_count, y == 0, y + 1 == cx->yaks.size(), to_b, version++)
+                          : recheck_gpu(cx, cur, pc, (int)y, r.o.min_kmer_count, y == 0, to_b, version++);
             to_b = !to_b;
             trace_region_tables(cx, (int)r.pass, "rech" + std::to_string(y), pc, true);
             if (cx->trace) trace_cns(cx, (int)r.pass, "cns_rech" + std::to_string(y), fetch_cns_dev(cx, cur));
         }
         fetch_result(cx, cur.pos, cur.base, cur.M_p, cur.M_cap, result, guessed ? r.M + r.grow_prev : r.M + pc.grow);
-    } catch (const GrowRetry &) {
-        if (!guessed) throw;
+    } catch (const GrowRetry &g) {
+        if ((g.grow && !guessed) || (g.rech_cap && !by_list)) throw;
         result.release();
         op_fill(cx, cx->scal.p + S_ERR, 0, 4);
+        op_fill(cx, cx->scal.p + S_COUNT, 0, (size_t)(SCAL_TOTAL - S_COUNT) * 4);
+        if (g.rech_cap) cx->timing.host.push_back({"rech_redo", 1.0f});
         r.reuse = false;
-        run_final_pass(r, result, true);
+        run_final_pass(r, result, exact_grow || g.grow, rech_general || g.rech_cap);
     }
 }
 
diff --git a/nextpolish2_amd/csrc/np2_kernels.hip b/nextpolish2_amd/csrc/np2_kernels.hip
--- a/nextpolish2_amd/csrc/np2_kernels.hip
+++ b/nextpolish2_amd/csrc/np2_kernels.hip
@@ -1283,6 +1283,16 @@
     if ((threadIdx.x & 63) == 0) out[w] = sc;
 }
 
+__device__ __forceinline__ void k_score_jobs(const uint32_t np2_bid, const uint32_t np2_nb, YakDev y, const uint8_t *__restrict__ strs, const uint2 *__restrict__ job_ol,
+                                             const uint32_t *__restrict__ n_jobs_p, uint16_t min_count, uint16_t *__restrict__ out) {
+    const uint32_t n = *n_jobs_p, n_waves = np2_nb * (blockDim.x >> 6);
+    for (uint32_t w = np2_bid * (blockDim.x >> 6) + (uint32_t)__builtin_amdgcn_readfirstlane((int)(threadIdx.x >> 6)); w < n; w += n_waves) {
+        const uint2 ol = job_ol[w];
+        const uint16_t sc = wave_score_string(y, strs + ol.x, ol.y, min_count);
+        if ((threadIdx.x & 63) == 0) out[w] = sc;
+    }
+}
+
 __device__ __forceinline__ void k_cand_score(const uint32_t np2_bid, const uint32_t np2_nb, YakDev y, const uint32_t *__restrict__ cand_seq_off, const uint64_t *__restrict__ cand_kmer,
                              const uint32_t *__restrict__ n_cand_p, uint16_t min_count,
                              uint16_t *__restrict__ kscore, uint32_t *__restrict__ long_list,
@@ -1452,6 +1462,10 @@
                    uint16_t *out) {
     if (n) NP2_LAUNCH(k_lookup, grid1(n), 256, s, y, hashes, n, min_count, out);
 }
+void launch_score_jobs(hipStream_t s, const YakDev &y, const uint8_t *strs, const uint2 *job_ol, const uint32_t *n_jobs_p,
+                       uint16_t min_count, uint16_t *out) {
+    NP2_LAUNCH(k_score_jobs, dim3(16), 256, s, y, strs, job_ol, n_jobs_p, min_count, out);
+}
 void launch_score_strings(hipStream_t s, const YakDev &y, const uint8_t *strs, const uint64_t *off, uint64_t n,
                           uint16_t min_count, uint16_t *out, bool own_strings) {
     if (n) NP2_LAUNCH(k_score_strings, grid1(n * 64), 256, s, y, strs, off, n, min_count, out, own_strings ? 1u : 0u);
diff --git a/nextpolish2_amd/csrc/np2_kernels.hpp b/nextpolish2_amd/csrc/np2_kernels.hpp
--- a/nextpolish2_amd/csrc/np2_kernels.hpp
+++ b/nextpolish2_amd/csrc/np2_kernels.hpp
@@ -172,6 +172,8 @@
 void launch_lookup(hipStream_t s, const YakDev &y, const uint64_t *hashes, uint64_t n, uint16_t min_count, uint16_t *out);
 void launch_score_strings(hipStream_t s, const YakDev &y, const uint8_t *strs, const uint64_t *off, uint64_t n,
                           uint16_t min_count, uint16_t *out, bool own_strings);
+void launch_score_jobs(hipStream_t s, const YakDev &y, const uint8_t *strs, const uint2 *job_ol, const uint32_t *n_jobs_p,
+                       uint16_t min_count, uint16_t *out);
 void launch_cand_score(hipStream_t s, const YakDev &y, const uint32_t *cand_seq_off, const uint8_t *cand_seq,
                        const uint64_t *cand_kmer, const uint32_t *n_cand_p, uint32_t cand_cap, uint16_t min_count,
                        uint16_t *kscore, uint32_t *long_list, uint32_t *n_long);
@@ -298,7 +300,8 @@
 void launch_edge_compact(hipStream_t s, const uint64_t *ekey, const uint32_t *flag, const uint32_t *idx, const uint32_t *wout,
                          uint32_t n, uint64_t *ukey, uint32_t *uw, uint32_t *n_out);
 void launch_seed(hipStream_t s, const RegionTables &rt, int32_t max_indel_len, uint8_t *reg_lable, uint32_t *seed_cand,
-                 uint32_t *keep_n, uint32_t *keep_list, uint16_t *keep_ks, uint32_t *err);
+                 uint32_t *keep_n, uint32_t *keep_list, uint16_t *keep_ks, uint32_t *err, uint32_t *rl_list = nullptr,
+                 uint32_t *rl_cnt = nullptr, uint32_t rl_cap = 0);
 uint32_t region_lb_blocks(uint32_t n_reg);
 void launch_splice_find(hipStream_t s, const uint32_t *cns_pos, const uint32_t *M_p, const uint32_t *lq_start,
                         const uint32_t *lq_end, const uint8_t *reg_lable, uint8_t lable, uint32_t n_reg, uint32_t *idx_s,
@@ -329,6 +332,34 @@
                         const uint32_t *cand_off, const uint32_t *keep_n, const uint32_t *keep_list, const uint16_t *keep_ks,
                         const uint32_t *order, bool first_yak, uint8_t *reg_lable, uint32_t *seed_cand);
 void launch_rech_relabel(hipStream_t s, uint8_t *reg_lable, uint32_t n_reg);
+static constexpr uint32_t RL_CAP_LIST = 1024;
+static constexpr uint32_t RL_CAP_JOBS = 2048;
+static constexpr uint32_t RL_CAP_BLOB = 1u << 20;
+static constexpr uint32_t RL_NREG_MAX = 400000;
+enum : uint32_t { RL_N = 0, RL_NGROUPS, RL_NJOBS, RL_OFF, RL_STATE_WORDS };
+struct RechList {
+    const uint32_t *list_in;
+    uint32_t *cnt_in;
+    uint32_t *list_out, *cnt_out;
+    uint32_t *st;
+    uint32_t *rech;
+    uint32_t *pos_lo, *pos_ub;
+    void *groups, *tmp_groups;
+    uint32_t *job_off, *blob_off, *glen;
+    uint2 *job_ol;
+    uint8_t *blob;
+    uint32_t cap_list, cap_jobs, cap_blob;
+};
+void launch_rech_prepare(hipStream_t s, const RechList &a, const uint32_t *cns_pos, const uint8_t *cns_base, const uint32_t *M_p,
+                         const uint32_t *lq_start, const uint32_t *lq_end, const uint32_t *keep_n, uint32_t ksize,
+                         const uint32_t *reg_maxlen, const uint32_t *cand_off, const uint32_t *keep_list,
+                         const uint32_t *seq_off, const uint8_t *seq, uint32_t *err);
+void launch_rech_finish(hipStream_t s, const RechList &a, const uint16_t *score, uint16_t *keep_ks, const uint32_t *cand_off,
+                        const uint32_t *keep_n, const uint32_t *keep_list, const uint32_t *order, bool first_yak,
+                        bool last_round, uint8_t *reg_lable, uint32_t *seed_cand, const uint32_t *cns_pos,
+                        const uint32_t *M_in, const uint32_t *lq_start, const uint32_t *seq_off,
+                        uint32_t *ap_g, uint32_t *ap_s, uint32_t *ap_e, int32_t *ap_delta, int32_t *ap_shift_incl,
+                        uint32_t *n_ap, uint32_t *M_out, uint32_t out_cap, uint32_t *err);
 
 struct FrontOp {
     uint32_t col0, q0, t0;
diff --git a/nextpolish2_amd/csrc/np2_regions.hip b/nextpolish2_amd/csrc/np2_regions.hip
--- a/nextpolish2_amd/csrc/np2_regions.hip
+++ b/nextpolish2_amd/csrc/np2_regions.hip
@@ -472,7 +472,8 @@
 __device__ __forceinline__ void k_seed(const uint32_t np2_bid0, const uint32_t np2_nb, RegionTables rt, int32_t max_indel_len,
                                               uint8_t *__restrict__ reg_lable, uint32_t *__restrict__ seed_cand,
                                               uint32_t *__restrict__ keep_n, uint32_t *__restrict__ keep_list,
-                                              uint16_t *__restrict__ keep_ks, uint32_t *__restrict__ err) {
+                                              uint16_t *__restrict__ keep_ks, uint32_t *__restrict__ err,
+                                              uint32_t *__restrict__ rl_list, uint32_t *__restrict__ rl_cnt, uint32_t rl_cap) {
     const uint32_t np2_bid = xcd_order(np2_bid0, np2_nb);
     const uint32_t wl = threadIdx.x & 63;
     const uint32_t g0 = (uint32_t)__builtin_amdgcn_readfirstlane((int)((np2_bid * blockDim.x + threadIdx.x) >> 6)) * 2;
@@ -559,6 +560,10 @@
             reg_lable[g] = lable;
             seed_cand[g] = c0 + seed;
             keep_n[g] = kn;
+            if (rl_cnt && (lable & LB_RECH)) {
+                const uint32_t i = atomicAdd(rl_cnt, 1u);
+                if (i < rl_cap) rl_list[i] = g;
+            }
         }
     }
 }
@@ -588,6 +593,38 @@
     return bound16_u32<true>(a, n, v);
 }
 
+__device__ __forceinline__ void cns_span(const uint32_t *__restrict__ cns_pos, uint32_t M, uint32_t st, uint32_t en,
+                                         uint32_t &lo, uint32_t &ub) {
+    lo = lower_bound_u32(cns_pos, M, st);
+    const uint32_t near = (uint32_t)min((uint64_t)M, (uint64_t)lo + (en - st) + 65u);
+    ub = (near == M || cns_pos[near - 1] > en) ? bound16_u32<true>(cns_pos, near, en, lo) : upper_bound_u32(cns_pos, M, en);
+}
+__device__ __forceinline__ bool splice_range(const uint32_t *__restrict__ cns_pos, uint32_t M, uint32_t st, uint32_t lo,
+                                             uint32_t ub, uint32_t &s, uint32_t &e) {
+    const bool found = lo < M && cns_pos[lo] == st;
+    s = lo;
+    e = found ? max(lo, ub) : lo;
+    return found;
+}
+__device__ __forceinline__ bool splice_find_region(const uint32_t *__restrict__ cns_pos, uint32_t M, uint32_t st, uint32_t en,
+                                                   uint32_t &s, uint32_t &e) {
+    uint32_t lo, ub;
+    cns_span(cns_pos, M, st, en, lo, ub);
+    return splice_range(cns_pos, M, st, lo, ub, s, e);
+}
+__device__ __forceinline__ void splice_plan_total(uint32_t m_in, uint32_t dsum, uint32_t cnt, uint32_t out_cap,
+                                                  uint32_t *__restrict__ n_ap, uint32_t *__restrict__ M_out,
+                                                  uint32_t *__restrict__ err) {
+    const uint32_t m_out = m_in + dsum;
+    if (m_out > out_cap) {
+        atomicOr(err, GROW_ERR);
+        *n_ap = 0;
+        *M_out = m_in;
+    } else {
+        *n_ap = cnt;
+        *M_out = m_out;
+    }
+}
 __device__ __forceinline__ void k_splice_find(const uint32_t np2_bid, const uint32_t np2_nb, const uint32_t *__restrict__ cns_pos, const uint32_t *__restrict__ M_p,
                               const uint32_t *__restrict__ lq_start,
                               const uint32_t *__restrict__ lq_end, const uint8_t *__restrict__ reg_lable,
@@ -595,17 +632,9 @@
                               uint32_t *__restrict__ stuck) {
     uint32_t g = np2_bid * blockDim.x + threadIdx.x;
     if (g >= n_reg || !(reg_lable[g] & lable)) return;
-    const uint32_t M = *M_p;
-    const uint32_t s = lower_bound_u32(cns_pos, M, lq_start[g]);
-    const bool found = s < M && cns_pos[s] == lq_start[g];
+    uint32_t s, e;
+    const bool found = splice_find_region(cns_pos, *M_p, lq_start[g], lq_end[g], s, e);
     idx_s[g] = s;
-    uint32_t e = s;
-    if (found) {
-        const uint32_t en = lq_end[g];
-        const uint32_t near = (uint32_t)min((uint64_t)M, (uint64_t)s + (en - lq_start[g]) + 65u);
-        e = (near == M || cns_pos[near - 1] > en) ? bound16_u32<true>(cns_pos, near, en, s) : upper_bound_u32(cns_pos, M, en);
-        e = max(s, e);
-    }
     idx_e[g] = e;
     if (!found) atomicMax(stuck, g + 1);
 }
@@ -659,17 +688,7 @@
         lo += flag[k];
         ld += (uint32_t)delta[k];
     }
-    if (bid == n_blocks - 1 && threadIdx.x == 0) {
-        const uint32_t m_out = *M_in + pre_d + dsum;
-        if (m_out > out_cap) {
-            atomicOr(err, GROW_ERR);
-            *n_ap = 0;
-            *M_out = *M_in;
-        } else {
-            *n_ap = pre_c + cnt;
-            *M_out = m_out;
-        }
-    }
+    if (bid == n_blocks - 1 && threadIdx.x == 0) splice_plan_total(*M_in, pre_d + dsum, pre_c + cnt, out_cap, n_ap, M_out, err);
 }
 static constexpr uint32_t SPLICE_SPAN = 2048;
 static constexpr uint32_t SPLICE_LDS_SLOTS = 256;
@@ -806,6 +825,84 @@
     uint32_t njobs;
 };
 
+__device__ __forceinline__ bool rech_chained(const uint32_t *rech, const uint32_t *__restrict__ lq_start,
+                                             const uint32_t *__restrict__ lq_end, uint32_t ksize, uint32_t x) {
+    return lq_start[rech[x]] < lq_end[rech[x - 1]] + ksize;
+}
+__device__ __forceinline__ bool rech_is_head(const uint32_t *rech, const uint32_t *__restrict__ lq_start,
+                                             const uint32_t *__restrict__ lq_end, uint32_t ksize, uint32_t e) {
+    uint32_t back = 0, x = e;
+    while (x > 0 && rech_chained(rech, lq_start, lq_end, ksize, x)) {
+        --x;
+        ++back;
+    }
+    return back % 6 == 0;
+}
+struct RechSearch {
+    const uint32_t *rech, *cns_pos, *lq_start, *lq_end;
+    uint32_t M;
+    __device__ __forceinline__ uint32_t lo(uint32_t x) const { return lower_bound_u32(cns_pos, M, lq_start[rech[x]]); }
+    __device__ __forceinline__ uint32_t ub(uint32_t x) const { return upper_bound_u32(cns_pos, M, lq_end[rech[x]]); }
+};
+struct RechFound {
+    const uint32_t *s_lo, *s_ub;
+    __device__ __forceinline__ uint32_t lo(uint32_t x) const { return s_lo[x]; }
+    __device__ __forceinline__ uint32_t ub(uint32_t x) const { return s_ub[x]; }
+};
+template <class Where>
+__device__ __forceinline__ RechGroup rech_group_build(uint32_t e, uint32_t n_rech, const uint32_t *rech, const Where &where,
+                                                      uint32_t M, const uint32_t *__restrict__ lq_start,
+                                                      const uint32_t *__restrict__ lq_end,
+                                                      const uint32_t *__restrict__ keep_n, uint32_t ksize,
+                                                      const uint32_t *__restrict__ reg_maxlen, uint32_t *__restrict__ err,
+                                                      uint64_t &len_bound) {
+    RechGroup G = {};
+    G.first = e;
+    uint32_t n = 1;
+    while (n < 6 && e + n < n_rech && rech_chained(rech, lq_start, lq_end, ksize, e + n)) ++n;
+    G.n = n;
+    const uint32_t l = ksize - 1;
+    const uint32_t i0 = where.lo(e);
+    if (i0 == 0 || i0 >= M) atomicOr(err, 64u);
+    G.el = i0;
+    G.sl = i0 > l ? i0 - l : 0;
+    const uint32_t i1u = where.ub(e + n - 1);
+    if (i1u == 0 || i1u >= M) atomicOr(err, 64u);
+    const uint32_t i1 = i1u ? i1u - 1 : 0;
+    G.sr = i1 + 1;
+    G.er = (i1 + l < M) ? i1 + l + 1 : M;
+    uint64_t jobs = 1;
+#pragma unroll
+    for (uint32_t x = 0; x < 6; ++x) {
+        if (x >= n) break;
+        G.lens[x] = keep_n[rech[e + x]];
+        jobs *= G.lens[x];
+        if (jobs > 0x7FFFFFFFull) {
+            atomicOr(err, 128u);
+            jobs = 0;
+        }
+        if (x + 1 < n) {
+            const uint32_t s = lq_end[rech[e + x]], en = lq_start[rech[e + x + 1]];
+            if (s + 1 == en) {
+                G.bs[x] = G.be[x] = 0;
+            } else {
+                G.bs[x] = where.ub(e + x);
+                G.be[x] = where.lo(e + x + 1);
+                if (G.be[x] < G.bs[x]) G.be[x] = G.bs[x];
+            }
+        }
+    }
+    G.njobs = (uint32_t)jobs;
+    uint64_t len = (uint64_t)(G.el - G.sl) + (G.er - G.sr);
+#pragma unroll
+    for (uint32_t x = 0; x < 6; ++x) {
+        if (x >= n) break;
+        len += reg_maxlen[rech[e + x]];
+        if (x + 1 < n) len += G.be[x] - G.bs[x];
+    }
+    len_bound = len;
+    return G;
+}
 __device__ __forceinline__ void k_rech_groups(const uint32_t np2_bid, const uint32_t np2_nb, const uint32_t *__restrict__ rech,
                                                      const uint32_t *__restrict__ n_rech_p,
                                                      const uint32_t *__restrict__ cns_pos, const uint32_t *__restrict__ M_p,
@@ -820,65 +917,13 @@
     unsigned long long bound = 0;
     const uint32_t e = np2_bid * 256 + threadIdx.x;
     const uint32_t n_rech = *n_rech_p, M = *M_p;
-    auto chained = [&](uint32_t x) { return lq_start[rech[x]] < lq_end[rech[x - 1]] + ksize; };
-    bool head = false;
-    RechGroup G = {};
+    const bool head = e < n_rech && rech_is_head(rech, lq_start, lq_end, ksize, e);
     uint32_t jobs32 = 0;
-    if (e < n_rech) {
-        uint32_t back = 0, x = e;
-        while (x > 0 && chained(x)) {
-            --x;
-            ++back;
-        }
-        head = back % 6 == 0;
-    }
     if (head) {
-        G.first = e;
-        uint32_t n = 1;
-        while (n < 6 && e + n < n_rech && chained(e + n)) ++n;
-        G.n = n;
-        const uint32_t l = ksize - 1;
-        const uint32_t p0 = lq_start[rech[e]];
-        const uint32_t i0 = lower_bound_u32(cns_pos, M, p0);
-        if (i0 == 0 || i0 >= M) atomicOr(err, 64u);
-        G.el = i0;
-        G.sl = i0 > l ? i0 - l : 0;
-        const uint32_t p1 = lq_end[rech[e + n - 1]];
-        const uint32_t i1u = upper_bound_u32(cns_pos, M, p1);
-        if (i1u == 0 || i1u >= M) atomicOr(err, 64u);
-        const uint32_t i1 = i1u ? i1u - 1 : 0;
-        G.sr = i1 + 1;
-        G.er = (i1 + l < M) ? i1 + l + 1 : M;
-        uint64_t jobs = 1;
-#pragma unroll
-        for (uint32_t x = 0; x < 6; ++x) {
-            if (x >= n) break;
-            G.lens[x] = keep_n[rech[e + x]];
-            jobs *= G.lens[x];
-            if (jobs > 0x7FFFFFFFull) {
-                atomicOr(err, 128u);
-                jobs = 0;
-            }
-            if (x + 1 < n) {
-                const uint32_t s = lq_end[rech[e + x]], en = lq_start[rech[e + x + 1]];
-                if (s + 1 == en) {
-                    G.bs[x] = G.be[x] = 0;
-                } else {
-                    G.bs[x] = upper_bound_u32(cns_pos, M, s);
-                    G.be[x] = lower_bound_u32(cns_pos, M, en);
-                    if (G.be[x] < G.bs[x]) G.be[x] = G.bs[x];
-                }
-            }
-        }
-        jobs32 = (uint32_t)jobs;
-        G.njobs = jobs32;
-        uint64_t len = (uint64_t)(G.el - G.sl) + (G.er - G.sr);
-#pragma unroll
-        for (uint32_t x = 0; x < 6; ++x) {
-            if (x >= n) break;
-            len += reg_maxlen[rech[e + x]];
-            if (x + 1 < n) len += G.be[x] - G.bs[x];
-        }
+        uint64_t len;
+        const RechGroup G = rech_group_build(e, n_rech, rech, RechSearch{rech, cns_pos, lq_start, lq_end, M}, M, lq_start, lq_end,
+                                             keep_n, ksize, reg_maxlen, err, len);
+        jobs32 = G.njobs;
         bound = (unsigned long long)jobs32 * len;
         tmp_groups[e] = G;
     }
@@ -949,31 +994,35 @@
     }
     return lo - 1;
 }
-template <bool WRITE> __device__ uint32_t rech_string(const RechCtx &cx, uint32_t job, uint8_t *__restrict__ out) {
-    const uint32_t gi = job_group(cx, job);
+template <bool WRITE>
+__device__ uint32_t rech_group_string(const RechCtx &cx, uint32_t gi, uint32_t rem, uint8_t *__restrict__ out, uint32_t lane = 0,
+                                      uint32_t nl = 1) {
     const RechGroup &G = cx.groups[gi];
-    uint32_t rem = job - cx.job_off[gi];
     uint32_t pick[6];
     for (uint32_t x = G.n; x-- > 0;) {
         pick[x] = rem % G.lens[x];
         rem /= G.lens[x];
     }
     uint32_t o = 0;
-    for (uint32_t i = G.sl; i < G.el; ++i, ++o)
-        if (WRITE) out[o] = cx.cns_base[i];
+    auto piece = [&](const uint8_t *__restrict__ src, uint32_t n) {
+        if (WRITE)
+            for (uint32_t t = lane; t < n; t += nl) out[o + t] = src[t];
+        o += n;
+    };
+    piece(cx.cns_base + G.sl, G.el - G.sl);
     for (uint32_t x = 0; x < G.n; ++x) {
         const uint32_t g = cx.rech[G.first + x];
         const uint32_t c = cx.keep_list[cx.cand_off[g] + pick[x]];
-        const uint32_t so = cx.seq_off[c], len = cx.seq_off[c + 1] - so;
-        for (uint32_t t = 0; t < len; ++t, ++o)
-            if (WRITE) out[o] = cx.seq[so + t];
-        if (x + 1 < G.n)
-            for (uint32_t i = G.bs[x]; i < G.be[x]; ++i, ++o)
-                if (WRITE) out[o] = cx.cns_base[i];
-    }
-    for (uint32_t i = G.sr; i < G.er; ++i, ++o)
-        if (WRITE) out[o] = cx.cns_base[i];
+        const uint32_t so = cx.seq_off[c];
+        piece(cx.seq + so, cx.seq_off[c + 1] - so);
+        if (x + 1 < G.n) piece(cx.cns_base + G.bs[x], G.be[x] - G.bs[x]);
+    }
+    piece(cx.cns_base + G.sr, G.er - G.sr);
     return o;
+}
+template <bool WRITE> __device__ uint32_t rech_string(const RechCtx &cx, uint32_t job, uint8_t *__restrict__ out) {
+    const uint32_t gi = job_group(cx, job);
+    return rech_group_string<WRITE>(cx, gi, job - cx.job_off[gi], out);
 }
 __device__ __forceinline__ void k_rech_job_len(const uint32_t np2_bid, const uint32_t np2_nb, RechCtx cx, uint32_t n_jobs, uint32_t *__restrict__ len) {
     uint32_t j = np2_bid * blockDim.x + threadIdx.x;
@@ -989,9 +1038,8 @@
     if (i < n) out[i] = in[i];
 }
 
-__device__ __forceinline__ void k_rech_apply(const uint32_t np2_bid, const uint32_t np2_nb, RechCtx cx, const uint16_t *__restrict__ score, uint16_t *__restrict__ keep_ks) {
-    uint32_t gi = np2_bid * blockDim.x + threadIdx.x;
-    if (gi >= cx.n_groups) return;
+__device__ __forceinline__ void rech_apply_group(const RechCtx &cx, uint32_t gi, const uint16_t *__restrict__ score,
+                                                 uint16_t *__restrict__ keep_ks) {
     const RechGroup &G = cx.groups[gi];
     const uint32_t j0 = cx.job_off[gi];
     if (G.n == 1) {
@@ -1014,15 +1062,17 @@
         }
     }
 }
-
-__device__ __forceinline__ void k_rech_select(const uint32_t np2_bid, const uint32_t np2_nb, const uint32_t *__restrict__ rech, const uint32_t *__restrict__ n_rech_p,
-                              const uint32_t *__restrict__ cand_off, const uint32_t *__restrict__ keep_n,
-                              const uint32_t *__restrict__ keep_list, const uint16_t *__restrict__ keep_ks,
-                              const uint32_t *__restrict__ order, uint32_t first_yak, uint8_t *__restrict__ reg_lable,
-                              uint32_t *__restrict__ seed_cand) {
-    uint32_t e = np2_bid * blockDim.x + threadIdx.x;
-    if (e >= *n_rech_p) return;
-    const uint32_t g = rech[e], c0 = cand_off[g], n = keep_n[g];
+__device__ __forceinline__ void k_rech_apply(const uint32_t np2_bid, const uint32_t np2_nb, RechCtx cx, const uint16_t *__restrict__ score, uint16_t *__restrict__ keep_ks) {
+    uint32_t gi = np2_bid * blockDim.x + threadIdx.x;
+    if (gi < cx.n_groups) rech_apply_group(cx, gi, score, keep_ks);
+}
+
+__device__ __forceinline__ void rech_select_region(uint32_t g, const uint32_t *__restrict__ cand_off,
+                                                   const uint32_t *__restrict__ keep_n, const uint32_t *__restrict__ keep_list,
+                                                   const uint16_t *__restrict__ keep_ks, const uint32_t *__restrict__ order,
+                                                   uint32_t first_yak, uint8_t *__restrict__ reg_lable,
+                                                   uint32_t *__restrict__ seed_cand) {
+    const uint32_t c0 = cand_off[g], n = keep_n[g];
     uint32_t c = 0, valid = 0;
     for (uint32_t p = 0; p < n; ++p)
         if (keep_ks[c0 + p] != 0) {
@@ -1042,12 +1092,215 @@
         seed_cand[g] = keep_list[c0 + i];
     }
 }
+__device__ __forceinline__ void k_rech_select(const uint32_t np2_bid, const uint32_t np2_nb, const uint32_t *__restrict__ rech, const uint32_t *__restrict__ n_rech_p,
+                              const uint32_t *__restrict__ cand_off, const uint32_t *__restrict__ keep_n,
+                              const uint32_t *__restrict__ keep_list, const uint16_t *__restrict__ keep_ks,
+                              const uint32_t *__restrict__ order, uint32_t first_yak, uint8_t *__restrict__ reg_lable,
+                              uint32_t *__restrict__ seed_cand) {
+    uint32_t e = np2_bid * blockDim.x + threadIdx.x;
+    if (e >= *n_rech_p) return;
+    rech_select_region(rech[e], cand_off, keep_n, keep_list, keep_ks, order, first_yak, reg_lable, seed_cand);
+}
+__device__ __forceinline__ uint8_t rech_relabel(uint8_t l) {
+    return (l & LB_TEMP) ? (uint8_t)(l ^ LB_TEMP) : (uint8_t)(l ^ LB_RECH);
+}
 __device__ __forceinline__ void k_rech_relabel(const uint32_t np2_bid, const uint32_t np2_nb, uint8_t *__restrict__ reg_lable, uint32_t n_reg) {
     uint32_t g = np2_bid * blockDim.x + threadIdx.x;
     if (g >= n_reg) return;
     const uint8_t l = reg_lable[g];
-    if (!(l & LB_RECH)) return;
-    reg_lable[g] = (l & LB_TEMP) ? (uint8_t)(l ^ LB_TEMP) : (uint8_t)(l ^ LB_RECH);
+    if (l & LB_RECH) reg_lable[g] = rech_relabel(l);
+}
+
+static constexpr uint32_t RL_ITEMS = 4;
+static_assert(RL_CAP_LIST == 256 * RL_ITEMS, "a thread of the list kernels owns RL_ITEMS consecutive entries");
+static_assert((uint64_t)RL_CAP_LIST * (RL_CAP_JOBS + 1) < (1ull << 32) && (uint64_t)RL_CAP_LIST * (RL_CAP_BLOB + 1) < (1ull << 32),
+              "clamped per-group sums stay inside 32 bits");
+
+__device__ __forceinline__ RechCtx rl_ctx(const RechList &a, const uint32_t *rech, const uint32_t *__restrict__ cand_off,
+                                          const uint32_t *__restrict__ keep_list, const uint32_t *__restrict__ seq_off,
+                                          const uint8_t *__restrict__ seq, const uint8_t *__restrict__ cns_base, uint32_t n_groups) {
+    return RechCtx{(const RechGroup *)a.groups, a.job_off, rech, cand_off, keep_list, seq_off, seq, cns_base, n_groups};
+}
+__device__ __forceinline__ void rl_round_off(const RechList &a, uint32_t cap_err, uint32_t *__restrict__ err) {
+    a.st[RL_N] = 0, a.st[RL_NGROUPS] = 0, a.st[RL_NJOBS] = 0, a.st[RL_OFF] = 1;
+    if (cap_err) atomicOr(err, RECH_CAP_ERR);
+}
+
+__device__ __forceinline__ void k_rech_prepare(const uint32_t np2_bid, const uint32_t np2_nb, RechList a,
+                                               const uint32_t *__restrict__ cns_pos, const uint8_t *__restrict__ cns_base,
+                                               const uint32_t *__restrict__ M_p, const uint32_t *__restrict__ lq_start,
+                                               const uint32_t *__restrict__ lq_end, const uint32_t *__restrict__ keep_n,
+                                               uint32_t ksize, const uint32_t *__restrict__ reg_maxlen,
+                                               const uint32_t *__restrict__ cand_off, const uint32_t *__restrict__ keep_list,
+                                               const uint32_t *__restrict__ seq_off, const uint8_t *__restrict__ seq,
+                                               uint32_t *__restrict__ err) {
+    __shared__ uint32_t s_raw[RL_CAP_LIST], s_rech[RL_CAP_LIST], s_lo[RL_CAP_LIST], s_ub[RL_CAP_LIST], sh[8], s_hdr[2];
+    const uint32_t tid = threadIdx.x;
+    if (tid == 0) s_hdr[0] = *err, s_hdr[1] = *a.cnt_in;
+    __syncthreads();
+    const uint32_t n = s_hdr[1], cap_list = min(a.cap_list, RL_CAP_LIST);
+    if (s_hdr[0] != 0 || n > cap_list) {
+        if (tid == 0) rl_round_off(a, s_hdr[0] == 0, err);
+        return;
+    }
+    for (uint32_t i = tid; i < n; i += 256) s_raw[i] = a.list_in[i];
+    __syncthreads();
+    for (uint32_t i = tid; i < n; i += 256) {
+        const uint32_t v = s_raw[i];
+        uint32_t rank = 0;
+        for (uint32_t j = 0; j < n; ++j) rank += s_raw[j] > v ? 1u : 0u;
+        s_rech[rank] = v;
+        a.rech[rank] = v;
+    }
+    __syncthreads();
+    const uint32_t M = *M_p;
+    for (uint32_t i = tid; i < n; i += 256) {
+        const uint32_t g = s_rech[i];
+        uint32_t lo, ub;
+        cns_span(cns_pos, M, lq_start[g], lq_end[g], lo, ub);
+        s_lo[i] = lo, s_ub[i] = ub;
+        a.pos_lo[i] = lo, a.pos_ub[i] = ub;
+    }
+    __syncthreads();
+    RechGroup *const groups = (RechGroup *)a.groups, *const tmp_groups = (RechGroup *)a.tmp_groups;
+    uint32_t head[RL_ITEMS], jobs[RL_ITEMS], bytes[RL_ITEMS], glen[RL_ITEMS], hs = 0, js = 0, bsum = 0;
+#pragma unroll
+    for (uint32_t k = 0; k < RL_ITEMS; ++k) {
+        const uint32_t e = tid * RL_ITEMS + k;
+        head[k] = (e < n && rech_is_head(s_rech, lq_start, lq_end, ksize, e)) ? 1u : 0u;
+        jobs[k] = 0, bytes[k] = 0, glen[k] = 0;
+        if (head[k]) {
+            uint64_t len;
+            const RechGroup G = rech_group_build(e, n, s_rech, RechFound{s_lo, s_ub}, M, lq_start, lq_end, keep_n, ksize, reg_maxlen, err, len);
+            tmp_groups[e] = G;
+            jobs[k] = min(G.njobs, a.cap_jobs + 1u);
+            glen[k] = (uint32_t)min(len, (uint64_t)a.cap_blob + 1u);
+            bytes[k] = (uint32_t)min((uint64_t)G.njobs * len, (uint64_t)a.cap_blob + 1u);
+        }
+        hs += head[k], js += jobs[k], bsum += bytes[k];
+    }
+    uint32_t nh, nj, nb;
+    uint32_t lh = block_excl_scan<OpAdd, 4>(hs, sh, nh);
+    uint32_t lj = block_excl_scan<OpAdd, 4>(js, sh, nj);
+    uint32_t lbt = block_excl_scan<OpAdd, 4>(bsum, sh, nb);
+    if (nj > min(a.cap_jobs, RL_CAP_JOBS) || nb > min(a.cap_blob, RL_CAP_BLOB)) {
+        if (tid == 0) rl_round_off(a, 1u, err);
+        return;
+    }
+#pragma unroll
+    for (uint32_t k = 0; k < RL_ITEMS; ++k) {
+        if (!head[k]) continue;
+        groups[lh] = tmp_groups[tid * RL_ITEMS + k];
+        a.job_off[lh] = lj;
+        a.blob_off[lh] = lbt;
+        a.glen[lh] = glen[k];
+        ++lh, lj += jobs[k], lbt += bytes[k];
+    }
+    if (tid == 0) {
+        a.job_off[nh] = nj;
+        a.st[RL_N] = n, a.st[RL_NGROUPS] = nh, a.st[RL_NJOBS] = nj, a.st[RL_OFF] = 0;
+    }
+    __threadfence_block();
+    __syncthreads();
+    const RechCtx cx = rl_ctx(a, s_rech, cand_off, keep_list, seq_off, seq, cns_base, nh);
+    for (uint32_t j = tid >> 4; j < nj; j += 16) {
+        const uint32_t gi = job_group(cx, j), rem = j - a.job_off[gi];
+        const uint32_t off = a.blob_off[gi] + rem * a.glen[gi];
+        uint32_t len = rech_group_string<false>(cx, gi, rem, nullptr);
+        if (len <= a.glen[gi]) {
+            rech_group_string<true>(cx, gi, rem, a.blob + off, tid & 15u, 16u);
+        } else {
+            if ((tid & 15u) == 0) atomicOr(err, RECH_CAP_ERR);
+            len = 0;
+        }
+        if ((tid & 15u) == 0) a.job_ol[j] = make_uint2(off, len);
+    }
+}
+
+__device__ __forceinline__ void k_rech_finish(const uint32_t np2_bid, const uint32_t np2_nb, RechList a,
+                                              const uint16_t *__restrict__ score, uint16_t *__restrict__ keep_ks,
+                                              const uint32_t *__restrict__ cand_off, const uint32_t *__restrict__ keep_n,
+                                              const uint32_t *__restrict__ keep_list, const uint32_t *__restrict__ order,
+                                              uint32_t first_yak, uint32_t last_round, uint8_t *__restrict__ reg_lable,
+                                              uint32_t *__restrict__ seed_cand, const uint32_t *__restrict__ cns_pos,
+                                              const uint32_t *__restrict__ M_in, const uint32_t *__restrict__ lq_start,
+                                              const uint32_t *__restrict__ seq_off,
+                                              uint32_t *__restrict__ ap_g, uint32_t *__restrict__ ap_s,
+                                              uint32_t *__restrict__ ap_e, int32_t *__restrict__ ap_delta,
+                                              int32_t *__restrict__ ap_shift_incl, uint32_t *__restrict__ n_ap,
+                                              uint32_t *__restrict__ M_out, uint32_t out_cap, uint32_t *__restrict__ err) {
+    __shared__ uint32_t sh[8], s_hdr[4], s_stuck;
+    const uint32_t tid = threadIdx.x;
+    if (tid == 0) s_hdr[0] = *err, s_hdr[1] = a.st[RL_N], s_hdr[2] = a.st[RL_NGROUPS], s_hdr[3] = a.st[RL_OFF], s_stuck = 0;
+    __syncthreads();
+    if (s_hdr[0] != 0 || s_hdr[3] != 0) {
+        if (tid == 0) *n_ap = 0, *M_out = *M_in, *a.cnt_in = 0, *a.cnt_out = 0;
+        return;
+    }
+    const uint32_t n = s_hdr[1], n_groups = s_hdr[2], M = *M_in;
+    const RechCtx cx = rl_ctx(a, a.rech, cand_off, keep_list, seq_off, nullptr, nullptr, n_groups);
+    for (uint32_t gi = tid; gi < n_groups; gi += 256) rech_apply_group(cx, gi, score, keep_ks);
+    __threadfence_block();
+    __syncthreads();
+    uint32_t g[RL_ITEMS], s[RL_ITEMS], e[RL_ITEMS];
+#pragma unroll
+    for (uint32_t k = 0; k < RL_ITEMS; ++k) {
+        const uint32_t x = tid * RL_ITEMS + k;
+        g[k] = 0, s[k] = 0, e[k] = 0;
+        if (x >= n) continue;
+        g[k] = a.rech[x];
+        rech_select_region(g[k], cand_off, keep_n, keep_list, keep_ks, order, first_yak, reg_lable, seed_cand);
+        if (!splice_range(cns_pos, M, lq_start[g[k]], a.pos_lo[x], a.pos_ub[x], s[k], e[k])) atomicMax(&s_stuck, g[k] + 1);
+    }
+    __syncthreads();
+    const uint32_t stuck = s_stuck;
+    uint32_t flag[RL_ITEMS], fsum = 0;
+    int32_t delta[RL_ITEMS], dsum_t = 0;
+#pragma unroll
+    for (uint32_t k = 0; k < RL_ITEMS; ++k) {
+        flag[k] = (tid * RL_ITEMS + k < n && g[k] + 1 > stuck) ? 1u : 0u;
+        delta[k] = 0;
+        if (flag[k]) {
+            const uint32_t c = seed_cand[g[k]];
+            delta[k] = (int32_t)(seq_off[c + 1] - seq_off[c]) - (int32_t)(e[k] - s[k]);
+        }
+        fsum += flag[k], dsum_t += delta[k];
+    }
+    uint32_t cnt, dsum;
+    uint32_t lo = block_excl_scan<OpAdd, 4>(fsum, sh, cnt);
+    uint32_t ld = block_excl_scan<OpAdd, 4>((uint32_t)dsum_t, sh, dsum);
+#pragma unroll
+    for (uint32_t k = 0; k < RL_ITEMS; ++k) {
+        if (flag[k]) {
+            ap_g[lo] = g[k];
+            ap_s[lo] = s[k];
+            ap_e[lo] = e[k];
+            ap_delta[lo] = delta[k];
+            ap_shift_incl[lo] = (int32_t)ld + delta[k];
+        }
+        lo += flag[k];
+        ld += (uint32_t)delta[k];
+    }
+    if (tid == 0) splice_plan_total(M, dsum, cnt, out_cap, n_ap, M_out, err);
+    uint32_t keep[RL_ITEMS], ksum = 0;
+#pragma unroll
+    for (uint32_t k = 0; k < RL_ITEMS; ++k) {
+        keep[k] = 0;
+        if (tid * RL_ITEMS + k < n) {
+            const uint8_t l = rech_relabel(reg_lable[g[k]]);
+            reg_lable[g[k]] = l;
+            keep[k] = (l & LB_RECH) ? 1u : 0u;
+        }
+        ksum += keep[k];
+    }
+    uint32_t n_keep;
+    uint32_t lk = block_excl_scan<OpAdd, 4>(ksum, sh, n_keep);
+#pragma unroll
+    for (uint32_t k = 0; k < RL_ITEMS; ++k) {
+        if (keep[k]) a.list_out[lk] = g[k];
+        lk += keep[k];
+    }
+    if (tid == 0) *a.cnt_in = 0, *a.cnt_out = last_round ? 0u : n_keep;
 }
 
 __device__ __forceinline__ void k_vote_counts(const uint32_t np2_bid, const uint32_t np2_nb, const uint32_t *__restrict__ first_reg, const uint8_t *__restrict__ bad,
@@ -1119,9 +1372,10 @@
     if (n) NP2_LAUNCH(k_edge_compact, g1(n), 256, s, ekey, flag, idx, wout, n, ukey, uw, n_out);
 }
 void launch_seed(hipStream_t s, const RegionTables &rt, int32_t max_indel_len, uint8_t *reg_lable, uint32_t *seed_cand,
-                 uint32_t *keep_n, uint32_t *keep_list, uint16_t *keep_ks, uint32_t *err) {
+                 uint32_t *keep_n, uint32_t *keep_list, uint16_t *keep_ks, uint32_t *err, uint32_t *rl_list, uint32_t *rl_cnt,
+                 uint32_t rl_cap) {
     if (rt.n_reg)
-        NP2_LAUNCH(k_seed, g1((uint64_t)((rt.n_reg + 1) / 2) * 64), 256, s, rt, max_indel_len, reg_lable, seed_cand, keep_n, keep_list, keep_ks, err);
+        NP2_LAUNCH(k_seed, g1((uint64_t)((rt.n_reg + 1) / 2) * 64), 256, s, rt, max_indel_len, reg_lable, seed_cand, keep_n, keep_list, keep_ks, err, rl_list, rl_cnt, rl_cap);
 }
 uint32_t region_lb_blocks(uint32_t n_reg) { return (n_reg + 256 * LB_REG_ITEMS - 1) / (256 * LB_REG_ITEMS); }
 void launch_splice_find(hipStream_t s, const uint32_t *cns_pos, const uint32_t *M_p, const uint32_t *lq_start,
@@ -1189,5 +1443,19 @@
 void launch_rech_relabel(hipStream_t s, uint8_t *reg_lable, uint32_t n_reg) {
     NP2_LAUNCH(k_rech_relabel, g1(n_reg), 256, s, reg_lable, n_reg);
 }
-
-}
+void launch_rech_prepare(hipStream_t s, const RechList &a, const uint32_t *cns_pos, const uint8_t *cns_base, const uint32_t *M_p,
+                         const uint32_t *lq_start, const uint32_t *lq_end, const uint32_t *keep_n, uint32_t ksize,
+                         const uint32_t *reg_maxlen, const uint32_t *cand_off, const uint32_t *keep_list,
+                         const uint32_t *seq_off, const uint8_t *seq, uint32_t *err) {
+    NP2_LAUNCH(k_rech_prepare, dim3(1), 256, s, a, cns_pos, cns_base, M_p, lq_start, lq_end, keep_n, ksize, reg_maxlen, cand_off, keep_list, seq_off, seq, err);
+}
+void launch_rech_finish(hipStream_t s, const RechList &a, const uint16_t *score, uint16_t *keep_ks, const uint32_t *cand_off,
+                        const uint32_t *keep_n, const uint32_t *keep_list, const uint32_t *order, bool first_yak,
+                        bool last_round, uint8_t *reg_lable, uint32_t *seed_cand, const uint32_t *cns_pos,
+                        const uint32_t *M_in, const uint32_t *lq_start, const uint32_t *seq_off,
+                        uint32_t *ap_g, uint32_t *ap_s, uint32_t *ap_e, int32_t *ap_delta, int32_t *ap_shift_incl,
+                        uint32_t *n_ap, uint32_t *M_out, uint32_t out_cap, uint32_t *err) {
+    NP2_LAUNCH(k_rech_finish, dim3(1), 256, s, a, score, keep_ks, cand_off, keep_n, keep_list, order, first_yak ? 1u : 0u, last_round ? 1u : 0u, reg_lable, seed_cand, cns_pos, M_in, lq_start, seq_off, ap_g, ap_s, ap_e, ap_delta, ap_shift_incl, n_ap, M_out, out_cap, err);
+}
+
+}
```

Result: faster. 4497, median of 6 (+4.2%).
